# OSU-NLP-Group/saev

Hardware: AMD Instinct MI355X
Metric: activations/sec (train step), d_in=1024 x32 k=32 (higher is better)
Workload: dtype f32 (encoder: fp16 MFMA first pass with a rigorous error margin, survivors recomputed exactly in fp32; all else fp32)

## Files before the change

saev_amd/csrc/ctx.h:

```cpp
#pragma once
#include <hip/hip_runtime.h>

#include <algorithm>
#include <cmath>
#include <cstdio>
#include <cstdlib>
#include <cstring>
#include <string>
#include <vector>

#include "kernels.h"

constexpr int AUX_KSPLIT_MAX = 16;
constexpr int CAND_CAP = 4096;
constexpr int CAND_STRIDE = CAND_CAP + 256;
constexpr int TIMING_RING = 512;
constexpr int DEAD_LAG = 4;
constexpr int DEAD_RING = 16;
enum { AUX_NONE = 0, AUX_SMALL_DEVICE = 1, AUX_SMALL_HOST = 2, AUX_DENSE = 3 };

struct saev_ctx {
    saev_cfg cfg{};
    saev_debug_cfg dbg{};
    int device = 0;
    std::string err;
    float* params = nullptr;
    float* grads = nullptr;
    float* adam_m = nullptr;
    float* adam_v = nullptr;
    long n_params = 0;
    long off_W_dec = 0, off_b_dec = 0, off_W_enc = 0, off_b_enc = 0;
    int shard_world = 1;
    long chunk_a = 0, chunk_b = 0;
    double* sumsq_bound = nullptr;
    hipEvent_t wdec_ready = nullptr;
    hipEvent_t wenc_ready = nullptr;
    std::vector<void*> allocs;
    size_t scratch_bytes = 0, aux_bytes = 0;
    uint8_t* muon_ws = nullptr;
    size_t muon_bytes = 0;
    int cuts_last[MAX_PREFIXES] = {0};
    int32_t *cand_cnt = nullptr, *gmax = nullptr, *cand_idx = nullptr;
    int gmax_stride = 0;
    float* cand_val = nullptr;
    float* h_dense = nullptr;
    int32_t *idx = nullptr, *aux_idx = nullptr;
    float *val = nullptr, *aux_val = nullptr;
    float *x_hat = nullptr, *g = nullptr, *g_aux = nullptr;
    RowStats* rowstats = nullptr;
    uint32_t* bitmap = nullptr;
    int32_t* grp_prefix = nullptr;
    int32_t* scan_totals = nullptr;
    int32_t csc_epoch = 0;
    int bitmap_words = 0;
    int back_rows = 0;
    int bitmap_words_last = 0;
    bool bitmap_clean = false;
    int bitmap_clean_words = 0;
    int bitmap_prefill_words = 0, bitmap_prefill_rows = 0;
    bool last_backward_gathered = false;
    int32_t *counts = nullptr, *starts = nullptr;
    int2* pairs = nullptr;
    float* colsum_partials = nullptr;
    float* dval_pairs = nullptr;
    double *sumsq_partials = nullptr, *sumsq_total = nullptr;
    bool wenc_sq_valid = false;
    float2* row_proj = nullptr;
    float* enc_sq = nullptr;
    bool row_proj_valid = false, tail_proj_in_adam = false;
    bool wenc_t_pending = false;
    int64_t* toks = nullptr;
    int32_t *fired = nullptr, *dead = nullptr;
    int32_t* flags = nullptr;
    int32_t *chunk_starts = nullptr, *part_starts = nullptr, *work_latent = nullptr;
    float *dW_encT = nullptr, *partials = nullptr, *db_partials = nullptr;
    bool dws_ok = false;
    int dws_rows = 0;
    bool dws_pairs = false;
    float *gS = nullptr, *xS = nullptr, *dvp = nullptr;
    float* xS_ov = nullptr;
    float* xS_bwd = nullptr;
    float* dval_rows = nullptr;
    bool dval_fwd = false;
    float* wn2 = nullptr;
    float* sq_wave = nullptr;
    int sq_wave_n = 0;
    bool wn2_fresh = false;
    bool dval_pairs_ready = false;
    bool fused_forward = false;
    bool g_rows_valid = true;
    bool fwd_slices = false;
    bool fwd_step = false;
    float* rs_part = nullptr;
    float* xS_c = nullptr;
    int2 *pv = nullptr, *pv2 = nullptr;
    int32_t *plat = nullptr, *cut_lat = nullptr, *cut_list = nullptr;
    int32_t* lat_unused = nullptr;
    bool fused_step = false;
    bool unused_valid = false;
    int P = 1;
    int32_t cuts[MAX_PREFIXES] = {0};
    float* G = nullptr;
    float* GS = nullptr;
    int P_cap = 0;
    int n_dead_host = 0, k_use_host = 0;
    int64_t tokens_seen = 0;
    bool tracker_dirty = false;
    int nd_cap = 0;
    DeadRecord* rec_host = nullptr;
    DeadRecord* rec_dev = nullptr;
    hipEvent_t dead_ev[DEAD_RING];
    bool dead_ev_created = false;
    int64_t dead_steps = 0;
    int64_t rec_valid_from = 1;
    int aux_route = AUX_NONE;
    int64_t n_readbacks = 0;
    std::vector<void*> aux_allocs;
    int32_t* dead_list = nullptr;
    float *Wenc_dead = nullptr, *Wdec_dead = nullptr, *H_dead = nullptr, *A_dead = nullptr, *dWd = nullptr, *dWe = nullptr,
          *dbe = nullptr, *aux_partials = nullptr, *WencT_dead = nullptr, *aux_small_part = nullptr, *aux_small_part2 = nullptr, *aux_small_partbe = nullptr;
    bool aux_dev_count = false;
    bool aux_small = false;
    int aux_mfma_bound = 0;
    int aux_ndp = AUX_SMALL_MAX;
    int aux_mfma_cap = AUX_SMALL_MAX;
    bool aux_mfma = false;
    bool aux_fused = false;
    bool aux_all = false;
    uint8_t* A_mask = nullptr;
    _Float16 *aux_ws1 = nullptr, *aux_ws2 = nullptr, *aux_xsA = nullptr, *aux_xsg = nullptr, *aux_kA = nullptr, *aux_kD = nullptr, *aux_kX = nullptr;
    bool aux_both = false;
    float* aux_parts = nullptr;
    int aux_kpad = 0;
    float *bias_dead = nullptr, *zero_bias = nullptr, *aux_scales = nullptr;
    float* aux_sync = nullptr;
    int aux_Dp2 = 0;
    float *row_margin = nullptr, *wnorm_scratch = nullptr, *surv_val = nullptr;
    int32_t *surv_idx = nullptr, *surv_cnt = nullptr, *surv_rng = nullptr;
    int rs_lat_range = 0, rs_n_ranges = 0;
    int32_t* tau_max = nullptr;
    float* heur_state = nullptr;
    float *f16r_scales = nullptr, *mu = nullptr, *xnorm = nullptr, *b_shift = nullptr, *dot_part = nullptr, *xabs_part = nullptr,
          *sq_part = nullptr, *wmax_prev = nullptr;
    bool wmax_known = false;
    bool mu_ready = false;
    bool stream_ok = false;
    float *WeS = nullptr;
    float *xn_part = nullptr, *amax_part = nullptr, *cmax_part = nullptr;
    float* b_seen = nullptr;
    int32_t *stale_host = nullptr, *stale_dev = nullptr;
    uint32_t* wchk = nullptr;
    float *mu_keep = nullptr, *xside_keep = nullptr;
    bool fwd_streamed = false;
    bool fwd_moves_mu = false;
    int64_t fwd_mu_serial = -1;
    bool borrow_streamed = false;
    bool follow_stream = false;
    bool wchk_valid = false;
    bool fwd_reused_wimg = false;
    uint32_t stale_salt = 0;
    int scale_par = 0;
    bool prep_valid = false;
    bool wimg_fresh = false;
    int64_t mu_serial = 0, wimg_mu_serial = -1;
    bool wimg_bf16_fresh = false;
    bool stream_step = false;
    bool stats_pending = false, stats_lists = false;
    bool aux_stats_pending = false;
    bool dead_list_ready = false;
    bool train_fused = false;
    const float* gather_pool = nullptr;
    const int64_t* gather_rows = nullptr;
    float *upper_c = nullptr, *mu_c = nullptr, *xnorm_c = nullptr, *xabs_c = nullptr;
    _Float16* xs_c = nullptr;
    saev_ctx* leader = nullptr;
    void* comm = nullptr;
    int comm_rank = 0, comm_world = 0;
    std::vector<saev_ctx*> followers;
    const float* xprep_x = nullptr;
    int xprep_n = 0;
    int64_t xprep_serial = 0;
    int64_t leader_serial_seen = 0;
    _Float16 *xs = nullptr, *ws = nullptr;
    int Dp = 0, S_pad = 0, MB_pad = 0;
    int max_work = 0, max_part = 0;
    float* upper = nullptr;
    saev_step_stats* stats = nullptr;
    double* stats_scratch = nullptr;
    int* tickets = nullptr;
    const float *ov_x = nullptr, *ov_g = nullptr, *ov_val = nullptr;
    const int32_t* ov_idx = nullptr;
    int ov_n = 0;
    float* db_aux = nullptr;
    bool trust_grads = false;
    bool btk = false;
    int btk_k = 0, btk_list_cap = 0;
    double btk_momentum = 0.1;
    float *threshold = nullptr, *threshold_own = nullptr;
    uint32_t* btk_ws = nullptr;
    int32_t *row_nnz = nullptr, *btk_over = nullptr;
    int btk_need = 0;
    bool relu_train = false;
    bool rt_fwd_live = false;
    double rt_l1 = 0.0;
    float* rt_dA = nullptr;
    float *rt_parts = nullptr, *rt_colpart = nullptr;
    float* rt_scales = nullptr;
    int rt_Sp = 0, rt_kpad = 0;
    _Float16 *rt_xsF = nullptr, *rt_xsG = nullptr;
    _Float16 *rt_wsR = nullptr, *rt_wsK = nullptr;
    _Float16 *rt_kF = nullptr, *rt_kG = nullptr, *rt_kX = nullptr;
    float* rt_wparts = nullptr;
    const float* x_last = nullptr;
// ... 96 lines not shown
```

saev_amd/csrc/ctx.hip:

```cpp
#include "ctx.h"

int muon_cfg_check(const saev_muon_cfg& m, std::string* why) {
    if (m.ns_steps < 0 || m.ns_steps >= 100) { *why = "ns_steps must be in [0, 100)"; return SAEV_INVALID_ARG; }
    if (m.adjust_lr < 0 || m.adjust_lr > 2) { *why = "adjust_lr must be 0 (original), 1 (match_rms_adamw) or 2 (none)"; return SAEV_INVALID_ARG; }
    if (!(m.momentum >= 0.f) || !(m.weight_decay >= 0.f)) { *why = "momentum and weight_decay must be >= 0"; return SAEV_INVALID_ARG; }
    return SAEV_OK;
}

extern "C" {

int saev_abi_version(void) { return SAEV_AMD_ABI_VERSION; }

int saev_layout(const saev_cfg* cfg, saev_layout_t* out) {
    if (!cfg || !out || cfg->d_model <= 0 || cfg->d_sae <= 0) return SAEV_INVALID_ARG;
    const int64_t S = cfg->d_sae, D = cfg->d_model, N = std::max(1, cfg->shard_world);
    out->chunk_a = (S + 1 + N - 1) / N * D;
    out->chunk_b = ((D * S + S + N - 1) / N + 3) / 4 * 4;
    out->off_W_dec = 0;
    out->off_b_dec = S * D;
    out->off_W_enc = N * out->chunk_a;
    out->off_b_enc = out->off_W_enc + D * S;
    out->n_total = N * out->chunk_a + N * out->chunk_b;
    return SAEV_OK;
}

const char* saev_last_error(const saev_ctx* ctx) { return ctx ? ctx->err.c_str() : free_error(); }

int saev_create(const saev_cfg* cfg, int device, saev_ctx** out) { return saev_create_ex(cfg, nullptr, device, out); }

int saev_create_ex(const saev_cfg* cfg, const saev_debug_cfg* dbg, int device, saev_ctx** out) {
    return saev_create_batch_topk(cfg, dbg, nullptr, device, out);
}

int saev_create_batch_topk(const saev_cfg* cfg, const saev_debug_cfg* dbg, const saev_batch_topk_cfg* bt_in, int device, saev_ctx** out) {
    return create_context(cfg, dbg, bt_in, nullptr, device, out);
}

int saev_create_relu_train(const saev_cfg* cfg, const saev_debug_cfg* dbg, const saev_relu_train_cfg* rt, int device, saev_ctx** out) {
    if (!cfg || !out) return SAEV_INVALID_ARG;
    *out = nullptr;
    if (cfg->activation != SAEV_ACT_RELU || cfg->k_aux != 0) return SAEV_INVALID_ARG;
    saev_relu_train_cfg r{};
    if (rt != nullptr && rt->struct_size > 0) std::memcpy(&r, rt, std::min((size_t)rt->struct_size, sizeof(r)));
    if (!(r.l1_coeff >= 0.0) || !std::isfinite(r.l1_coeff)) return SAEV_INVALID_ARG;
    if (cfg->encoder_mode == SAEV_ENCODER_BF16 || cfg->shard_world > 1 || cfg->max_backward_rows > cfg->max_batch) return SAEV_UNSUPPORTED;
    r.struct_size = (int32_t)sizeof(r);
    return create_context(cfg, dbg, nullptr, &r, device, out);
}

}

int create_context(const saev_cfg* cfg, const saev_debug_cfg* dbg, const saev_batch_topk_cfg* bt_in, const saev_relu_train_cfg* rt, int device,
                   saev_ctx** out) {
    if (!cfg || !out) return SAEV_INVALID_ARG;
    *out = nullptr;
    if (cfg->activation != SAEV_ACT_TOPK && cfg->activation != SAEV_ACT_RELU && cfg->activation != SAEV_ACT_BATCHTOPK) return SAEV_INVALID_ARG;
    const bool btk = cfg->activation == SAEV_ACT_BATCHTOPK;
    if (bt_in != nullptr && !btk) return SAEV_INVALID_ARG;
    saev_batch_topk_cfg bt{};
    if (bt_in != nullptr && bt_in->struct_size > 0) std::memcpy(&bt, bt_in, std::min((size_t)bt_in->struct_size, sizeof(bt)));
    else bt.batch_momentum = 0.1;
    saev_cfg btk_cfg;
    int btk_k = 0;
    if (btk) {
        if (cfg->top_k <= 0 || cfg->d_sae <= 0 || bt.row_cap < 0 || bt.list_cap < 0 || !(bt.batch_momentum >= 0.0 && bt.batch_momentum <= 1.0))
            return SAEV_INVALID_ARG;
        if (cfg->encoder_mode == SAEV_ENCODER_BF16 || cfg->shard_world > 1 || cfg->max_backward_rows > cfg->max_batch) return SAEV_UNSUPPORTED;
        if ((uint64_t)cfg->max_batch * (uint64_t)cfg->d_sae >= (1ull << 31)) return SAEV_UNSUPPORTED;
        btk_k = std::min(cfg->top_k, cfg->d_sae);
        const long want = bt.row_cap > 0 ? bt.row_cap : std::max(64L, 4L * btk_k);
        btk_cfg = *cfg;
        btk_cfg.top_k = (int32_t)std::min<long>(cfg->d_sae, (want + 63) / 64 * 64);
        cfg = &btk_cfg;
    }
    saev_cfg relu_cfg;
    if (cfg->activation == SAEV_ACT_RELU) {
        if (cfg->k_aux != 0) return SAEV_UNSUPPORTED;
        relu_cfg = *cfg;
        relu_cfg.top_k = 1;
        cfg = &relu_cfg;
    }
    if (cfg->d_model <= 0 || cfg->d_sae <= 0 || cfg->top_k <= 0 || cfg->max_batch <= 0) return SAEV_INVALID_ARG;
    if ((uint64_t)cfg->max_batch * CAND_STRIDE * 4ull >= (1ull << 32)) return SAEV_INVALID_ARG;
    if (cfg->d_model % 4 != 0 || cfg->d_sae % 4 != 0 || cfg->d_model > 4096) return SAEV_UNSUPPORTED;
    if (cfg->k_aux < 0 || cfg->k_aux > 1024) return SAEV_UNSUPPORTED;
    if (cfg->encoder_mode != SAEV_ENCODER_F32 && cfg->encoder_mode != SAEV_ENCODER_F16X3 && cfg->encoder_mode != SAEV_ENCODER_BF16 &&
        cfg->encoder_mode != SAEV_ENCODER_F16R)
        return SAEV_INVALID_ARG;
    saev_ctx* c = new saev_ctx();
    c->cfg = *cfg;
    c->cfg.top_k = std::min(cfg->top_k, cfg->d_sae);
    if (dbg != nullptr && dbg->struct_size > 0)
        std::memcpy(&c->dbg, dbg, std::min((size_t)dbg->struct_size, sizeof(saev_debug_cfg)));
    c->device = device;
    c->btk = btk; c->btk_k = btk_k; c->btk_momentum = bt.batch_momentum; c->btk_list_cap = bt.list_cap;
    c->relu_train = rt != nullptr;
    c->rt_l1 = rt != nullptr ? rt->l1_coeff : 0.0;
    if (hipSetDevice(device) != hipSuccess) {
        delete c;
        return SAEV_HIP_ERROR;
    }
    const long S = cfg->d_sae, D = cfg->d_model, MB = cfg->max_batch, K = c->cfg.top_k, KA = cfg->k_aux;
    const long MBB = std::max<long>(MB, cfg->max_backward_rows);
    c->back_rows = (int)MBB;
    if ((uint64_t)MBB * K >= (1ull << 31)) { delete c; return SAEV_INVALID_ARG; }
    {
        saev_layout_t lay;
        saev_layout(cfg, &lay);
        c->shard_world = std::max(1, cfg->shard_world);
        c->chunk_a = lay.chunk_a; c->chunk_b = lay.chunk_b;
        c->off_W_dec = lay.off_W_dec; c->off_b_dec = lay.off_b_dec; c->off_W_enc = lay.off_W_enc; c->off_b_enc = lay.off_b_enc;
        c->n_params = lay.n_total;
    }
    int rc = SAEV_OK;
#define A(p, n) if (rc == SAEV_OK) rc = alloc(c, &c->p, (size_t)(n))
    c->gmax_stride = (int)((MB + 255) / 256 * 256);
    A(cand_cnt, MB); A(gmax, (size_t)64 * c->gmax_stride); A(cand_idx, MB * CAND_STRIDE); A(cand_val, MB * CAND_STRIDE);
    A(h_dense, MB * S);
    A(idx, MB * K); A(val, MB * K);
    if (KA > 0) { A(aux_idx, MB * KA); A(aux_val, MB * KA); A(g_aux, MB * D); A(dead_list, S); }
    A(x_hat, MB * D); A(g, MB * D);
    A(rowstats, MB);
    c->bitmap_words = (int)(((MBB + 31) / 32 + 7) / 8 * 8);
    A(bitmap, S * c->bitmap_words);
    A(grp_prefix, S * (c->bitmap_words / 8));
    A(scan_totals, ((S + 1023) / 1024) * 4);
    A(counts, S); A(starts, S + 1); A(pairs, MBB * K); A(dval_pairs, MBB * (size_t)cfg->top_k);
    {
        const long max_pairs = MBB * K;
        c->max_work = (int)(S + (max_pairs + DW_CHUNK - 1) / DW_CHUNK);
        c->max_part = (int)(2 * ((max_pairs + DW_CHUNK - 1) / DW_CHUNK) + 2);
    }
    A(chunk_starts, S + 1); A(part_starts, S); A(work_latent, c->max_work);
    A(dW_encT, S * D); A(partials, (size_t)c->max_part * 2 * D); A(db_partials, c->max_part); A(row_proj, S); A(enc_sq, S);
    {
        const bool rows_only = c->dbg.dw_route == 1;
        c->dws_ok = !rows_only && !btk && D % DWS_SLICE == 0 && (uint64_t)S * D * 4ull < (1ull << 32) && MBB < (1l << 24) &&
                    (uint64_t)MBB * K < (1ull << 31);
    }
    c->fwd_slices = !btk && c->cfg.encoder_mode == SAEV_ENCODER_F16R && c->dbg.fwd_route == 0 && D % RS_SLICE == 0 &&
                    (uint64_t)S * 128ull < (1ull << 32) - 256ull && fused_supported(c->cfg);
    if (c->fwd_slices) {
        A(rs_part, (size_t)(D / RS_SLICE) * MB * REFINE_CAP); A(surv_rng, MB * RS_MAX_RANGES);
        c->rs_lat_range = (int)std::max<long>(RS_LAT_RANGE, ((S + RS_MAX_RANGES - 1) / RS_MAX_RANGES + 255) / 256 * 256);
        c->rs_n_ranges = (int)((S + c->rs_lat_range - 1) / c->rs_lat_range);
    }
    if (c->fwd_slices && !c->dws_ok) A(xS, MBB * D);
    if (c->dws_ok) {
        A(gS, MBB * D); A(xS, MBB * D); A(dvp, (size_t)(D / DWS_SLICE) * MBB * K);
        if (c->dbg.dw_route != 2 && decode_forms_dval((int)D, (int)K)) A(dval_rows, MB * K);
        A(pv, MBB * K); A(pv2, MBB * K); A(plat, MBB * K); A(cut_lat, (MBB * K + DWS_RUN - 1) / DWS_RUN); A(cut_list, 4 * (1 + (MBB * K + DWS_RUN - 1) / DWS_RUN)); A(lat_unused, S);
        if (c->dval_rows != nullptr && c->dbg.fin_route == 0) { A(wn2, S); A(sq_wave, (size_t)2 * dw_slices_waves((int)D, (int)(MBB * K))); }
    }
    A(colsum_partials, ((MBB + 63) / 64) * D);
    A(sumsq_partials, 2 * 1024 + (S + 3) / 4 + 8 + transpose_blocks((int)S, (int)D)); A(sumsq_total, 1);
    if (c->cfg.encoder_mode != SAEV_ENCODER_F32 || KA > 0 || c->relu_train) {
        c->Dp = (int)((D + 31) / 32 * 32);
        c->S_pad = (int)((S + 255) / 256 * 256);
        c->MB_pad = (int)((MB + 255) / 256 * 256);
        A(zero_bias, std::max(S, D)); A(aux_scales, 16); A(aux_sync, absmax_parts_max((int)MB));
    }
    if (c->cfg.encoder_mode != SAEV_ENCODER_F32) {
        A(xs, (size_t)c->MB_pad * 2 * c->Dp);
        A(ws, (size_t)c->S_pad * 2 * c->Dp);
        A(row_margin, MB); A(wnorm_scratch, std::max((S + 3) / 4, 3 * ((S + 255) / 256))); A(f16r_scales, 16); A(mu, D); A(xnorm, 2 * MB); A(b_shift, S);
        A(xabs_part, (MB + 3) / 4);
        if (c->cfg.encoder_mode == SAEV_ENCODER_F16R) { A(dot_part, (size_t)2 * (c->Dp / 32) * c->S_pad); A(sq_part, (size_t)2 * (c->Dp / 32) * c->S_pad); A(wmax_prev, 1); }
        if (c->cfg.encoder_mode == SAEV_ENCODER_F16R) { A(surv_idx, MB * REFINE_CAP); A(surv_val, MB * REFINE_CAP); A(surv_cnt, MB); }
    }
    c->stream_ok = c->fwd_slices && c->cfg.bound_mode == 0 && c->dbg.prep_route == 0 && D % 32 == 0 && c->Dp == (int)D;
    if (c->stream_ok) {
        A(WeS, S * D); A(xn_part, (size_t)(D / 32) * c->MB_pad * 2);
        A(amax_part, (size_t)(c->MB_pad / 256) * (D / 32)); A(cmax_part, (size_t)(c->MB_pad / 256) * (D / 32)); A(b_seen, S);
        A(mu_keep, D); A(xside_keep, 4);
    }
    if (c->stream_ok || c->cfg.encoder_mode == SAEV_ENCODER_BF16) A(wchk, (size_t)2 * ((S + 255) / 256) * ((D + 31) / 32));
    A(toks, S); A(fired, S); A(dead, S); A(flags, 16); A(upper, 1); A(stats, 1);
    A(tau_max, MB); A(heur_state, 8); A(stats_scratch, STATS_SCRATCH_DOUBLES); A(tickets, 8); A(db_aux, D);
    if (btk) { A(btk_ws, btk_workspace_words((int)MB)); A(row_nnz, MB); A(btk_over, 1); A(threshold_own, 1); }
#undef A
    if (rc == SAEV_OK && c->relu_train) rc = relu_train_alloc(c);
    if (rc != SAEV_OK) {
        for (void* p : c->allocs) hipFree(p);
        delete c;
        return rc;
    }
    hipMemset(c->toks, 0, S * sizeof(int64_t));
    hipMemset(c->fired, 0, S * sizeof(int32_t));
    hipMemset(c->dead, 0, S * sizeof(int32_t));
    hipMemset(c->flags, 0, 16 * sizeof(int32_t));
    if (btk) {
        hipMemset(c->threshold_own, 0, sizeof(float));
        hipMemset(c->btk_ws, 0, BTK_ST_WORDS * sizeof(uint32_t));
        hipMemset(c->btk_over, 0, sizeof(int32_t));
        c->threshold = c->threshold_own;
    }
    if (c->stream_ok || c->cfg.encoder_mode == SAEV_ENCODER_BF16) {
        void* hp = nullptr;
        if (hipHostMalloc(&hp, 64, hipHostMallocMapped) == hipSuccess &&
            hipHostGetDevicePointer(reinterpret_cast<void**>(&c->stale_dev), hp, 0) == hipSuccess) {
            c->stale_host = static_cast<int32_t*>(hp);
            c->stale_host[0] = 0; c->stale_host[1] = 0;
        } else {
            if (hp) hipHostFree(hp);
            c->stale_host = nullptr; c->stale_dev = nullptr;
        }
    }
    hipMemset(c->scan_totals, 0, ((S + 1023) / 1024) * 4 * sizeof(int32_t));
    hipMemset(c->stats, 0, sizeof(saev_step_stats));
    hipMemset(c->stats_scratch, 0, STATS_SCRATCH_DOUBLES * sizeof(double));
    hipMemset(c->tickets, 0, 8 * sizeof(int));
    {
        const float init[8] = {2.6f, 0.f, 0.f, 0.f, 0.f, 0.f, 0.f, 0.f};
        hipMemcpy(c->heur_state, init, sizeof(init), hipMemcpyHostToDevice);
    }
    hipMemset(c->rowstats, 0, MB * sizeof(RowStats));
    if (c->xs) hipMemset(c->xs, 0, (size_t)c->MB_pad * 2 * c->Dp * sizeof(_Float16));
    if (c->zero_bias) hipMemset(c->zero_bias, 0, std::max(S, D) * sizeof(float));
    if (c->f16r_scales) hipMemset(c->f16r_scales, 0, 16 * sizeof(float));
    if (KA > 0) {
        const int s4 = (int)((S + 3) / 4 * 4);
        const int want = cfg->aux_dead_cap > 0 ? cfg->aux_dead_cap : std::max(4096, 8 * (int)KA);
        const int cap = std::min((want + 3) / 4 * 4, s4);
        rc = alloc_aux_buffers(c, cap);
        if (rc == SAEV_OK) {
            void* h = nullptr;
            if (hipHostMalloc(&h, DEAD_RING * sizeof(DeadRecord), hipHostMallocMapped) != hipSuccess ||
                hipHostGetDevicePointer(reinterpret_cast<void**>(&c->rec_dev), h, 0) != hipSuccess) {
                rc = SAEV_HIP_ERROR;
            } else {
                c->rec_host = static_cast<DeadRecord*>(h);
                std::memset(h, 0, DEAD_RING * sizeof(DeadRecord));
                for (int i = 0; i < DEAD_RING && rc == SAEV_OK; ++i)
                    if (hipEventCreateWithFlags(&c->dead_ev[i], hipEventDisableTiming) != hipSuccess) rc = SAEV_HIP_ERROR;
                c->dead_ev_created = rc == SAEV_OK;
            }
        }
        if (rc != SAEV_OK) {
            for (void* q : c->allocs) hipFree(q);
            for (void* q : c->aux_allocs) hipFree(q);
            if (c->rec_host) hipHostFree(c->rec_host);
            delete c;
            return rc;
        }
    }
    hipDeviceSynchronize();
    *out = c;
    return SAEV_OK;
}

extern "C" {

static void detach_follower(saev_ctx* c) {
    c->leader = nullptr;
    centre_owner_changed(c);
    c->borrow_streamed = false;
    c->follow_stream = false;
}

static void unlink_from_leader(saev_ctx* c) {
    if (c->leader != nullptr) {
        auto& f = c->leader->followers;
        f.erase(std::remove(f.begin(), f.end(), c), f.end());
        detach_follower(c);
    }
}

void saev_destroy(saev_ctx* c) {
    if (!c) return;
    for (saev_ctx* f : c->followers) detach_follower(f);
    c->followers.clear();
    unlink_from_leader(c);
    hipSetDevice(c->device);
    hipDeviceSynchronize();
    saev_comm_destroy(c);
    for (void* p : c->allocs) hipFree(p);
    for (void* p : c->aux_allocs) hipFree(p);
    if (c->G) hipFree(c->G);
// ... 293 lines not shown
```

saev_amd/csrc/ctx_backward.hip:

```cpp
#include "ctx.h"

extern "C" {


int saev_backward_begin(saev_ctx* c, void* stream) {
    if (!c) return SAEV_INVALID_ARG;
    REQUIRE(c, !c->relu_train, SAEV_UNSUPPORTED, "saev_backward_begin: a ReLU training context runs its dense backward in one piece (saev_step_backward)");
    REQUIRE(c, c->x_last && c->training_last, SAEV_INVALID_ARG, "saev_backward_begin: no training forward in flight");
    REQUIRE(c, c->grads, SAEV_NOT_BOUND, "gradient buffer not bound");
    hipStream_t s = (hipStream_t)stream;
    const int S = c->cfg.d_sae, D = c->cfg.d_model, K = c->cfg.top_k;
    const bool ov = c->ov_x != nullptr;
    const int n = ov ? c->ov_n : c->n_last;
    const int words = ((n + 31) / 32 + 7) / 8 * 8;
    c->row_proj_valid = false;
    CscArgs a{};
    a.idx = ov ? c->ov_idx : c->idx; a.code_stride = K; a.k = K; a.k_dev = nullptr; a.n_rows = n; a.S = S;
    a.bitmap = c->bitmap; a.words = words; a.grp_prefix = c->grp_prefix; a.scan_totals = c->scan_totals;
    a.counts = c->counts; a.starts = c->starts; a.pairs = c->pairs;
    a.chunk_starts = c->chunk_starts; a.part_starts = c->part_starts; a.work_latent = c->work_latent;
    const bool ov_slices = ov && c->dws_ok && c->P_last == 1 && n <= c->back_rows;
    c->dws_pairs = ov ? ov_slices : c->dws_rows == n;
    if (ov_slices) {
        c->xS_bwd = c->xS;
        if (!c->followers.empty()) {
            if (c->xS_ov == nullptr) {
                int rca = alloc(c, &c->xS_ov, (size_t)c->back_rows * D);
                if (rca != SAEV_OK) return rca;
            }
            c->xS_bwd = c->xS_ov;
        }
        HIPCHK(c, launch_slice_major_copy(c->ov_g, c->ov_x, n, D, c->gS, c->xS_bwd, s));
        c->dws_rows = 0;
    }
    c->csc_epoch = c->csc_epoch == 0x7fffffff ? 1 : c->csc_epoch + 1;
    a.epoch = c->dbg.csc_route == 2 ? 0 : c->csc_epoch;
    if (c->dws_pairs) {
        a.zero_word = c->cut_list;
        a.pv = c->pv; a.plat = c->plat; a.val = ov ? c->ov_val : c->val;
        a.P = c->P_last;
        for (int p = 0; p < c->P_last; ++p) a.cuts[p] = c->cuts_last[p];
        if (!ov && c->dval_fwd) { a.pv2 = c->pv2; a.dval = c->dval_rows; }
    }
    c->dval_pairs_ready = c->dws_pairs && a.pv2 != nullptr;
    if (c->fused_step && c->dws_pairs) { a.pairs = nullptr; a.chunk_starts = nullptr; a.part_starts = nullptr; a.work_latent = nullptr; }
    const float* gmat = ov ? c->ov_g : (c->P_last > 1 ? c->G : c->g);
    const bool g_slices = !ov && c->P_last == 1 && !c->g_rows_valid;
    if (g_slices) {
        REQUIRE(c, c->dws_rows == n, SAEV_INVALID_ARG, "saev_backward_begin: the forward in flight left no gradient rows");
        gmat = c->gS;
    }
    const bool prefilled = !ov && c->bitmap_prefill_words == words && c->bitmap_prefill_rows == n;
    HIPCHK(c, launch_csc_build(a, s, c->bitmap_clean && words <= c->bitmap_clean_words, gmat, D, (long)c->P_last * D,
                               c->colsum_partials, c->grads + c->off_b_dec, prefilled, g_slices));
    c->bitmap_prefill_words = 0;
    c->last_backward_gathered = ov;
    c->bitmap_clean = false;
    c->bitmap_words_last = words;
    if (c->aux_route != AUX_NONE) {
        int rc = auxk_backward(c, s);
        if (rc != SAEV_OK) return rc;
    }
    return SAEV_OK;
}

int saev_backward_rows(saev_ctx* c, int32_t lat_lo, int32_t lat_hi, void* stream) {
    return saev_backward_rows_part(c, lat_lo, lat_hi, 0, stream);
}

int saev_backward_rows_part(saev_ctx* c, int32_t lat_lo, int32_t lat_hi, int32_t part, void* stream) {
    if (!c) return SAEV_INVALID_ARG;
    REQUIRE(c, !c->relu_train, SAEV_UNSUPPORTED, "saev_backward_rows: a ReLU training context runs its dense backward in one piece, over all latents (saev_step_backward)");
    REQUIRE(c, part >= 0 && part <= 2, SAEV_INVALID_ARG, "saev_backward_rows_part: part must be 0 (both), 1 (decoder) or 2 (encoder)");
    REQUIRE(c, c->x_last && c->training_last && c->grads, SAEV_INVALID_ARG, "saev_backward_rows: call saev_backward_begin first");
    const int S = c->cfg.d_sae, D = c->cfg.d_model, K = c->cfg.top_k;
    const bool ov = c->ov_x != nullptr;
    const int n = ov ? c->ov_n : c->n_last;
    REQUIRE(c, 0 <= lat_lo && lat_lo < lat_hi && lat_hi <= S, SAEV_INVALID_ARG, "saev_backward_rows: bad latent range");
    REQUIRE(c, !c->btk || (part == 0 && lat_lo == 0 && lat_hi == S), SAEV_UNSUPPORTED,
            "saev_backward_rows: a BatchTopK context runs the backward over all latents in one part");
    hipStream_t s = (hipStream_t)stream;
    DwRowsArgs a{};
    a.starts = c->starts; a.chunk_starts = c->chunk_starts; a.work_latent = c->work_latent;
    a.part_starts = c->part_starts; a.pairs = c->pairs; a.val = ov ? c->ov_val : c->val; a.W_dec = c->params + c->off_W_dec;
    a.g = ov ? c->ov_g : (c->P_last > 1 ? c->G : c->g);
    const bool slices_all = lat_lo == 0 && lat_hi == S && c->dws_pairs && (ov || c->dws_rows == n);
    REQUIRE(c, ov || c->P_last > 1 || c->g_rows_valid || slices_all, SAEV_INVALID_ARG,
            "saev_backward_rows: the fused step's forward keeps no row-major gradient (a latent range needs the phase forward)");
    a.x = ov ? c->ov_x : c->x_last;
    a.D = D; a.S = S; a.k_dev = nullptr; a.accumulate = 0;
    a.P = c->P_last;
    for (int p = 0; p < c->P_last; ++p) a.cuts[p] = c->cuts_last[p];
    a.dW_dec = c->grads + c->off_W_dec; a.dW_encT = c->dW_encT; a.db_enc = c->grads + c->off_b_enc;
    a.partials = c->partials; a.db_partials = c->db_partials;
    a.lat_lo = lat_lo; a.lat_hi = lat_hi;
    a.part = part; a.dval = c->dval_pairs;
    const bool all_rows = part == 0 && lat_lo == 0 && lat_hi == S;
    const bool clears = part != 2 && lat_lo == 0 && lat_hi == S && c->bitmap_words_last > 0;
    if (clears) { a.clear_bitmap = c->bitmap; a.clear_words = c->bitmap_words_last; }
    a.row_proj = all_rows ? c->row_proj : nullptr; a.project = c->cfg.remove_parallel_grads ? 1 : 0;
    a.enc_sq = all_rows ? c->enc_sq : nullptr;
    const int max_work = (lat_hi - lat_lo) + (int)(((long)n * K + DW_CHUNK - 1) / DW_CHUNK);
    if (slices_all) {
        DwSlicesArgs w{};
        w.starts = c->starts; w.pv = c->pv; w.pv2 = c->pv2; w.plat = c->plat; w.gS = c->P_last > 1 ? c->GS : c->gS; w.W_dec = a.W_dec; w.P = c->P_last;
        w.xS = ov ? c->xS_bwd : (c->fwd_step ? c->xS_c : c->xS);
        w.n_rows = n; w.D = D; w.S = S; w.pair_cap = (int)((long)c->back_rows * K);
        w.dvp = c->dvp; w.dW_dec = a.dW_dec; w.dW_encT = a.dW_encT; w.db_enc = a.db_enc;
        const size_t runs_cap = ((size_t)w.pair_cap + DWS_RUN - 1) / DWS_RUN;
        w.part_dec = c->partials; w.part_enc = c->partials + 2 * runs_cap * D;
        w.cut_lat = c->cut_lat; w.cut_list = c->cut_list;
        w.lat_unused = (all_rows && c->fused_step) ? c->lat_unused : nullptr;
        c->unused_valid = w.lat_unused != nullptr;
        w.row_proj = a.row_proj; w.project = a.project; w.enc_sq = a.enc_sq;
        w.clear_bitmap = a.clear_bitmap; w.clear_words = a.clear_words;
        w.have_dval = c->dval_pairs_ready ? 1 : 0;
        c->sq_wave_n = 0;
        if (c->dval_pairs_ready && c->wn2_fresh && part == 0) {
            w.wn2 = c->wn2;
            if (c->fused_step && all_rows && c->sq_wave != nullptr && c->dbg.fin_route != 2) {
                c->sq_wave_n = dw_slices_waves(D, (int)((long)n * K));
                w.sq_wave_dec = c->sq_wave; w.sq_wave_enc = c->sq_wave + c->sq_wave_n;
            }
        }
        HIPCHK(c, launch_dw_slices(w, (int)((long)n * K), part, s));
    } else {
        c->unused_valid = false;
        HIPCHK(c, launch_dw_rows(a, max_work, s));
    }
    if (c->aux_route == AUX_DENSE)
        HIPCHK(c, launch_scatter_add_dead(c->dead_list, c->n_dead_host, D, c->dWd, c->dWe, c->dbe, c->grads + c->off_W_dec,
                                          c->dW_encT, c->grads + c->off_b_enc, lat_lo, lat_hi, s,
                                          c->aux_dev_count ? c->flags + 4 : nullptr, part, a.row_proj, a.W_dec, a.project, a.enc_sq,
                                          c->unused_valid ? c->lat_unused : nullptr, c->sq_wave_n > 0 ? c->starts : nullptr));
    else if (c->aux_route != AUX_NONE)
        HIPCHK(c, launch_scatter_add_dead(c->dead_list, c->aux_mfma ? c->aux_ndp : AUX_SMALL_MAX, D, c->dWd, c->dWe, c->dbe, c->grads + c->off_W_dec,
                                          c->dW_encT, c->grads + c->off_b_enc, lat_lo, lat_hi, s, c->flags + 4, part,
                                          a.row_proj, a.W_dec, a.project, a.enc_sq, c->unused_valid ? c->lat_unused : nullptr,
                                          c->sq_wave_n > 0 ? c->starts : nullptr));
    if (ov && c->aux_route != AUX_NONE && part != 2 && lat_lo == 0)
        HIPCHK(c, launch_colsum(c->db_aux, 1, D, c->colsum_partials, c->grads + c->off_b_dec, 1, nullptr, s));
    c->row_proj_valid = all_rows;
    if (clears) { c->bitmap_clean = true; c->bitmap_clean_words = c->bitmap_words_last; }
    return SAEV_OK;
}

float* saev_grad_w_enc_t(saev_ctx* c) { return c ? c->dW_encT : nullptr; }

int saev_bind_w_enc_t(saev_ctx* c, float* scratch) {
    if (!c || !scratch) return SAEV_INVALID_ARG;
    c->dW_encT = scratch;
    return SAEV_OK;
}

int saev_copy_step_state(saev_ctx* c, int32_t n_rows, float* g_out, int32_t* idx_out, float* val_out, void* stream) {
    if (!c) return SAEV_INVALID_ARG;
    REQUIRE(c, !c->btk, SAEV_UNSUPPORTED, "saev_copy_step_state: not for a BatchTopK context (no sparse-state exchange)");
    REQUIRE(c, !c->relu_train, SAEV_UNSUPPORTED, "saev_copy_step_state: not for a ReLU training context (its step state is dense: no sparse-state exchange)");
    REQUIRE(c, c->n_last > 0 && c->training_last && n_rows == c->n_last, SAEV_INVALID_ARG,
            "saev_copy_step_state: n_rows must be the row count of the training forward in flight");
    hipStream_t s = (hipStream_t)stream;
    const size_t nk = (size_t)n_rows * c->cfg.top_k, nd = (size_t)n_rows * c->cfg.d_model * (size_t)c->P_last;
    REQUIRE(c, !g_out || c->P_last > 1 || c->g_rows_valid, SAEV_INVALID_ARG,
            "saev_copy_step_state: the fused step's forward keeps no row-major gradient (use saev_step_forward)");
    if (g_out) HIPCHK(c, hipMemcpyAsync(g_out, c->P_last > 1 ? c->G : c->g, nd * sizeof(float), hipMemcpyDeviceToDevice, s));
    if (idx_out) HIPCHK(c, hipMemcpyAsync(idx_out, c->idx, nk * sizeof(int32_t), hipMemcpyDeviceToDevice, s));
    if (val_out) HIPCHK(c, hipMemcpyAsync(val_out, c->val, nk * sizeof(float), hipMemcpyDeviceToDevice, s));
    return SAEV_OK;
}

int saev_backward_override(saev_ctx* c, const float* x_all, const float* g_all, const int32_t* idx_all, const float* val_all,
                           int32_t n_all) {
    if (!c) return SAEV_INVALID_ARG;
    if (x_all == nullptr) { c->ov_x = nullptr; c->ov_n = 0; return SAEV_OK; }
    REQUIRE(c, !c->btk, SAEV_UNSUPPORTED, "saev_backward_override: not for a BatchTopK context (a batch-wide top-k over ranks needs a distributed select)");
    REQUIRE(c, !c->relu_train, SAEV_UNSUPPORTED, "saev_backward_override: not for a ReLU training context (one GPU: the dense backward runs over its own rows)");
    REQUIRE(c, g_all && idx_all && val_all && n_all > 0, SAEV_INVALID_ARG, "saev_backward_override: NULL buffer");
    REQUIRE(c, n_all <= c->back_rows, SAEV_INVALID_ARG,
            "saev_backward_override: the gathered row count exceeds saev_cfg.max_backward_rows (set it to the GLOBAL batch)");
    REQUIRE(c, c->x_last && c->training_last, SAEV_INVALID_ARG, "saev_backward_override: no training forward in flight");
    REQUIRE(c, ((uintptr_t)x_all % 16) == 0 && ((uintptr_t)g_all % 16) == 0, SAEV_INVALID_ARG, "x_all / g_all must be 16-byte aligned");
    c->ov_x = x_all; c->ov_g = g_all; c->ov_idx = idx_all; c->ov_val = val_all; c->ov_n = n_all;
    return SAEV_OK;
}

int32_t saev_aux_compact_rows(const saev_ctx* c) {
    if (!c || c->aux_route == AUX_NONE) return 0;
    return c->aux_route == AUX_DENSE ? (c->n_dead_host + 3) / 4 * 4 : (c->aux_mfma ? c->aux_ndp : AUX_SMALL_MAX);
}

static int aux_compact_copy(saev_ctx* c, float* buf, bool out, hipStream_t s) {
    const size_t rows = (size_t)saev_aux_compact_rows(c), D = c->cfg.d_model;
    if (rows == 0) return SAEV_OK;
    REQUIRE(c, buf != nullptr, SAEV_INVALID_ARG, "saev_aux_compact_*: NULL buffer");
    float* seg[4] = {c->dWd, c->dWe, c->dbe, c->db_aux};
    const size_t len[4] = {rows * D, rows * D, rows, D};
    size_t off = 0;
    for (int i = 0; i < 4; ++i) {
        if (out) HIPCHK(c, hipMemcpyAsync(buf + off, seg[i], len[i] * sizeof(float), hipMemcpyDeviceToDevice, s));
        else HIPCHK(c, hipMemcpyAsync(seg[i], buf + off, len[i] * sizeof(float), hipMemcpyDeviceToDevice, s));
        off += len[i];
    }
    return SAEV_OK;
}
int saev_aux_compact_export(saev_ctx* c, float* buf, void* stream) {
    if (!c) return SAEV_INVALID_ARG;
    return aux_compact_copy(c, buf, true, (hipStream_t)stream);
}
int saev_aux_compact_import(saev_ctx* c, const float* buf, void* stream) {
    if (!c) return SAEV_INVALID_ARG;
    return aux_compact_copy(c, const_cast<float*>(buf), false, (hipStream_t)stream);
}

int saev_trust_gradients(saev_ctx* c, int32_t on) {
    if (!c) return SAEV_INVALID_ARG;
    c->trust_grads = on != 0;
    return SAEV_OK;
}

int saev_backward_end(saev_ctx* c, void* stream) {
    if (!c) return SAEV_INVALID_ARG;
    REQUIRE(c, !c->relu_train, SAEV_UNSUPPORTED, "saev_backward_end: a ReLU training context runs its dense backward in one piece (saev_step_backward)");
    REQUIRE(c, c->grads, SAEV_NOT_BOUND, "gradient buffer not bound");
    double* sq = c->sumsq_partials + 2 * sumsq_blocks() + (c->cfg.d_sae + 3) / 4;
    HIPCHK(c, launch_transpose(c->dW_encT, c->grads + c->off_W_enc, c->cfg.d_sae, c->cfg.d_model, (hipStream_t)stream, sq));
    c->wenc_sq_valid = true;
    return SAEV_OK;
}

int saev_step_backward(saev_ctx* c, void* stream) {
    if (c && c->relu_train) return relu_train_backward(c, (hipStream_t)stream);
    int rc = saev_backward_begin(c, stream);
    if (rc != SAEV_OK) return rc;
    rc = saev_backward_rows(c, 0, c->cfg.d_sae, stream);
    if (rc != SAEV_OK) return rc;
    return saev_backward_end(c, stream);
}

}
```

saev_amd/csrc/ctx_forward.hip:

```cpp
#include "ctx.h"

extern "C" {


int saev_normalize_w_dec(saev_ctx* c, void* stream) {
    if (!c) return SAEV_INVALID_ARG;
    REQUIRE(c, c->params, SAEV_NOT_BOUND, "parameters not bound");
    if (!c->cfg.normalize_w_dec) return SAEV_OK;
    HIPCHK(c, launch_normalize_rows(c->params + c->off_W_dec, c->cfg.d_sae, c->cfg.d_model, (hipStream_t)stream));
    return SAEV_OK;
}

static bool bind_x_sources(saev_ctx* c, const float* x, int n, bool allow_borrow) {
    saev_ctx* l = c->leader;
    const bool borrow = allow_borrow && l != nullptr && l->xprep_x == x && l->xprep_n == n && l->xprep_serial != c->leader_serial_seen;
    saev_ctx* src = borrow ? l : c;
    c->upper_c = src->upper; c->mu_c = src->mu; c->xnorm_c = src->xnorm; c->xabs_c = src->xabs_part; c->xs_c = src->xs;
    c->borrow_streamed = borrow && l->fwd_streamed && l->mu_keep != nullptr;
    if (c->borrow_streamed) c->mu_c = l->mu_keep;
    c->fwd_step = c->fwd_slices && (src == c || src->fwd_slices);
    c->xS_c = c->fwd_step ? src->xS : nullptr;
    if (borrow) c->leader_serial_seen = l->xprep_serial;
    return borrow;
}
// ... 416 lines not shown
    int64_t single = S;
    if (!prefixes_host) { prefixes_host = &single; n_prefixes = 1; }
    REQUIRE(c, n_prefixes >= 1 && n_prefixes <= 16, SAEV_INVALID_ARG, "saev_decode_rows: 1 to 16 prefixes");
    REQUIRE(c, prefixes_host[n_prefixes - 1] == S && prefixes_host[0] >= 1, SAEV_INVALID_ARG,
            "prefixes must end at d_sae and start at >= 1");
    for (int p = 1; p < n_prefixes; ++p)
        REQUIRE(c, prefixes_host[p] > prefixes_host[p - 1], SAEV_INVALID_ARG, "prefixes must be strictly increasing");
    ReluDecodeArgs a{};
    a.idx = idx; a.val = val; a.row_nnz = row_nnz; a.row_cap = row_cap; a.n_rows = n; a.D = c->cfg.d_model;
    a.W_dec = c->params + c->off_W_dec; a.b_dec = c->params + c->off_b_dec;
    a.n_prefixes = n_prefixes;
    for (int p = 0; p < n_prefixes; ++p) a.prefixes[p] = prefixes_host[p];
    a.x_hats = x_hats_out;
    HIPCHK(c, launch_relu_decode(a, (hipStream_t)stream));
    return SAEV_OK;
}

int saev_scatter_rows(saev_ctx* c, const int32_t* idx, const float* val, const int32_t* row_nnz, int32_t row_cap, int32_t n,
                      float* f_out, void* stream) {
    if (!c) return SAEV_INVALID_ARG;
    REQUIRE(c, idx && val && row_nnz && f_out && n > 0 && row_cap > 0, SAEV_INVALID_ARG, "saev_scatter_rows: bad arguments");
    HIPCHK(c, launch_relu_scatter(idx, val, row_nnz, row_cap, n, c->cfg.d_sae, f_out, (hipStream_t)stream));
    return SAEV_OK;
}

int saev_remove_parallel_grads(saev_ctx* c, void* stream) {
    if (!c) return SAEV_INVALID_ARG;
    REQUIRE(c, c->params && c->grads, SAEV_NOT_BOUND, "parameters/grads not bound");
    if (!c->cfg.remove_parallel_grads) return SAEV_OK;
    HIPCHK(c, launch_rpg(c->grads + c->off_W_dec, c->params + c->off_W_dec, c->cfg.d_sae, c->cfg.d_model,
                         (hipStream_t)stream));
    return SAEV_OK;
}

int saev_gather_rows(saev_ctx* c, const float* pool, const int64_t* rows, int32_t n, float* out, void* stream) {
    if (!c) return SAEV_INVALID_ARG;
    REQUIRE(c, pool && rows && out && n > 0, SAEV_INVALID_ARG, "saev_gather_rows: bad arguments");
    HIPCHK(c, launch_gather_rows(pool, rows, n, c->cfg.d_model, out, (hipStream_t)stream));
    return SAEV_OK;
}


int saev_step_forward(saev_ctx* c, const float* x, int32_t n, int64_t n_rows_global, int32_t training,
                      void* stream) {
    if (!c) return SAEV_INVALID_ARG;
    if (c->relu_train) return relu_train_forward(c, x, n, n_rows_global, training, (hipStream_t)stream);
    REQUIRE(c, c->cfg.activation != SAEV_ACT_RELU, SAEV_UNSUPPORTED, "saev_step_forward: a ReLU context runs the forward entries only");
    REQUIRE(c, c->params, SAEV_NOT_BOUND, "parameters not bound");
    REQUIRE(c, x && n > 0 && n <= c->cfg.max_batch, SAEV_INVALID_ARG,
            "saev_step_forward: n_rows must be in 1..max_batch");
    REQUIRE(c, ((uintptr_t)x % 16) == 0, SAEV_INVALID_ARG, "x must be 16-byte aligned");
    REQUIRE(c, n_rows_global >= n, SAEV_INVALID_ARG, "n_rows_global < n_rows");
    hipStream_t s = (hipStream_t)stream;
    const int S = c->cfg.d_sae, D = c->cfg.d_model, K = c->cfg.top_k;
    c->x_last = x;
    c->n_last = n;
    c->training_last = training;
    c->ov_x = nullptr; c->ov_n = 0;
    c->unused_valid = false;
    hipEvent_t wdec_ev = c->wdec_ready;
    c->wdec_ready = nullptr;
    const bool btk = c->btk;
    const bool borrowed = bind_x_sources(c, x, n, !btk);
    if (c->stale_host != nullptr && reinterpret_cast<volatile int32_t*>(c->stale_host)[1] != 0) {
        const int n_tiles = reinterpret_cast<volatile int32_t*>(c->stale_host)[1];
        reinterpret_cast<volatile int32_t*>(c->stale_host)[1] = 0;
        c->wimg_fresh = false; c->wimg_bf16_fresh = false; c->wn2_fresh = false;
        c->err = "W_enc was written outside the library without saev_params_touched (" + std::to_string(n_tiles) +
                 " 32 x 256 tiles changed between two optimizer steps): a recent step encoded with operand images of the OLD values. "
                 "Announce such writes (saev_params_touched / SaeEngine.params_touched) or make them through torch in-place "
                 "operations on the parameter tensors; the context prepares from scratch from here on";
        return SAEV_STALE_PARAMS;
    }
    if (c->stale_host != nullptr && *reinterpret_cast<volatile int32_t*>(c->stale_host) != 0) {
        *reinterpret_cast<volatile int32_t*>(c->stale_host) = 0;
        c->wimg_fresh = false;
        c->wn2_fresh = false;
    }
    c->stream_step = c->stream_ok && c->prep_valid && c->wimg_fresh && c->wimg_mu_serial == c->mu_serial && c->leader == nullptr &&
                     c->wenc_ready == nullptr && c->fwd_step && (c->followers.empty() || c->dbg.group_route == 0);
    if (!borrowed) {
        c->fwd_streamed = c->stream_step;
        c->fwd_moves_mu = c->stream_step && c->train_fused;
        c->fwd_mu_serial = c->mu_serial;
    }
    c->follow_stream = borrowed && c->borrow_streamed && c->stream_ok && c->wimg_fresh && c->wimg_mu_serial == c->leader->fwd_mu_serial &&
                       c->wenc_ready == nullptr && c->fwd_step && c->cfg.encoder_mode == SAEV_ENCODER_F16R;
    c->fwd_reused_wimg = c->stream_step || c->follow_stream;
    if (c->gather_pool != nullptr && !c->stream_step)
        HIPCHK(c, launch_gather_rows(c->gather_pool, c->gather_rows, n, D, const_cast<float*>(x), s));
    if (c->stream_step) {
        c->xprep_x = nullptr;
    } else if (!borrowed && !btk && c->cfg.encoder_mode == SAEV_ENCODER_F16R) {
        c->xprep_x = nullptr;
        HIPCHK(c, launch_colsum_absmax(x, n, D, c->colsum_partials, c->mu, c->xabs_part, c->upper, s, 1.0f / (float)n, c->stats, c->flags));
        c->mu_ready = true;
        c->mu_serial++;
    } else {
        HIPCHK(c, launch_step_zero(c->stats, c->upper, c->flags, s));
        if (!borrowed) {
            c->xprep_x = nullptr;
            HIPCHK(c, launch_absmax(x, (long)n * D, c->upper, s));
        }
    }
    (void)n_rows_global;
    int rc;
    if (btk) {
        rc = encode_dense_h(c, x, n, s);
        if (rc == SAEV_OK) rc = btk_codes(c, c->h_dense, n, training, c->row_nnz, c->idx, c->val, c->btk_over, s);
        if (rc == SAEV_OK) {
            int32_t need = 0;
            HIPCHK(c, hipMemcpyAsync(&need, c->btk_over, sizeof(int32_t), hipMemcpyDeviceToHost, s));
            HIPCHK(c, hipStreamSynchronize(s));
            if (need > 0) {
                c->btk_need = need;
                c->x_last = nullptr; c->n_last = 0; c->training_last = 0;
                c->err = "BatchTopK: a row holds " + std::to_string(need) + " codes, the context's row_cap is " + std::to_string(K) +
                         " (create a context with a larger saev_batch_topk_cfg.row_cap and repeat the forward; the threshold has not moved)";
                return SAEV_ROW_OVERFLOW;
            }
        }
    } else {
        rc = encode_topk_impl(c, x, n, c->idx, c->val, c->flags, s, c->upper_c, borrowed);
    }
    if (rc != SAEV_OK) return rc;
    if (!borrowed) { c->xprep_x = x; c->xprep_n = n; c->xprep_serial++; }
    if (!borrowed && c->stream_ok && !c->stream_step && c->fwd_step) {
        HIPCHK(c, hipMemcpyAsync(scl(c) + 4, c->upper, sizeof(float), hipMemcpyDeviceToDevice, s));
        c->prep_valid = true;
    }
    if (wdec_ev != nullptr) HIPCHK(c, hipStreamWaitEvent(s, wdec_ev, 0));
    if (training) {
        c->wn2_fresh = false;
        if (c->cfg.normalize_w_dec) {
            HIPCHK(c, launch_normalize_rows(c->params + c->off_W_dec, S, D, s, c->wn2));
            c->wn2_fresh = c->wn2 != nullptr;
        }
    }

    DecodeArgs a{};
    a.x = x; a.idx = c->idx; a.val = c->val; a.code_stride = K; a.k = K;
    a.W_dec = c->params + c->off_W_dec; a.b_dec = c->params + c->off_b_dec;
    a.n_rows = n; a.D = D; a.S = S; a.idx_limit = S;
    a.upper = c->upper_c;
    a.gscale = 2.0f / ((float)n * (float)D * (float)c->P);
    a.training = training ? 1 : 0;
    a.g = c->g; a.x_hat = c->x_hat; a.fired = c->fired; a.rowstats = c->rowstats;
    c->dws_rows = 0;
    c->dval_fwd = false;
    if (training && c->dws_ok && (c->P == 1 || c->GS != nullptr)) { a.gS = c->P == 1 ? c->gS : c->GS; a.xS = c->fwd_step ? nullptr : c->xS; c->dws_rows = n; }
    if (c->dws_rows == n && c->dval_rows != nullptr && (c->P == 1 || decode_matry_forms_dval(D, K))) { a.dval_out = c->dval_rows; c->dval_fwd = true; }
    c->g_rows_valid = !(c->train_fused && training && c->P == 1 && c->dws_rows == n);
    if (!c->g_rows_valid) a.g = nullptr;
    c->bitmap_prefill_words = 0;
    if (training && c->dbg.csc_route == 0 && c->bitmap != nullptr && c->bitmap_clean && !c->last_backward_gathered) {
        const int words = ((n + 31) / 32 + 7) / 8 * 8;
        if (words <= c->bitmap_clean_words) {
            a.csc_bitmap = c->bitmap; a.csc_words = words;
            c->bitmap_prefill_words = words; c->bitmap_prefill_rows = n;
            c->bitmap_clean = false;
        }
    }
    if (c->P > 1) {
        MatryArgs m{};
        m.P = c->P;
        for (int p = 0; p < c->P; ++p) m.cuts[p] = c->cuts[p];
        m.G = c->G;
        m.g_rows_all = c->fused_forward ? 0 : 1;
        HIPCHK(c, launch_decode_matry(a, m, s));
    } else {
        HIPCHK(c, launch_decode(a, s));
    }
    c->P_last = c->P;
    for (int p = 0; p < c->P; ++p) c->cuts_last[p] = c->cuts[p];
    const bool lists = !btk && fused_supported(c->cfg) && !(c->cfg.bound_mode != 0 && c->cfg.encoder_mode != SAEV_ENCODER_F32 && f16_ngroups(c) == 32);
    c->stats_pending = false;
    if (c->train_fused && training) {
        c->stats_pending = true;
        c->stats_lists = lists;
        return SAEV_OK;
    }
    HIPCHK(c, launch_stats_reduce(c->rowstats, n, D, c->P, c->cfg.alpha, 0, c->upper_c, c->flags + 2, c->stats, s, nullptr, c->stats_scratch,
                                  lists ? c->cand_cnt : nullptr, CAND_CAP));
    return SAEV_OK;
}

}
```

saev_amd/csrc/kernels.h:

```cpp
#pragma once
#include <hip/hip_runtime.h>
#include <stdint.h>

#include <string>

#include "../../include/saev_amd.h"

enum { EPI_DENSE = 0, EPI_TOPK = 1 };

struct EncodeArgs {
    const float* x;
    const float* W_enc;
    const float* b_enc;
    int n_rows, D, S;
    int s_splits;
    float* h_out;
    int ngroups;
    int32_t* gmax;
    int gmax_stride;
    int32_t* cand_cnt;
    float* cand_val;
    int32_t* cand_idx;
    int cand_cap;
    int cand_stride;
    const int32_t* enable_flag;
    int enable_when;
};

size_t encode_gemm_smem_bytes();
hipError_t launch_encode_gemm(const EncodeArgs& a, int epi, hipStream_t stream);
int encode_gemm_tile_rows();
int encode_gemm_tile_latents();

struct SelectDenseArgs {
    const float* h;
    int n_rows, S;
    int k;
    const int32_t* k_dev;
    const int32_t* mask;
    int32_t* idx_out;
    float* val_out;
    int out_stride;
    const int32_t* enable_flag;
    int enable_when;
    int walk_grid;
};
hipError_t launch_select_dense(const SelectDenseArgs& a, hipStream_t stream);

struct SelectCandArgs {
    const int32_t* cand_cnt;
    const float* cand_val;
    const int32_t* cand_idx;
    int cand_cap, cand_stride, n_rows, k;
    int32_t* idx_out;
    float* val_out;
    int out_stride;
    const int32_t* enable_flag;
    int enable_when;
    const float* row_margin;
    const float* x;
    const float* W_encT;
    const float* b_enc;
    int D;
    int32_t* surv_idx;
    float* surv_val;
    int32_t* surv_cnt;
    int32_t* refine_overflow;
    const int32_t* tau_max;
    int32_t* invalid;
    int32_t* ovf;
    int32_t* surv_rng;
    int lat_range, n_ranges;
    const float* sum_part;
    const float* sum_bias;
    int sum_n;
    size_t sum_plane;
};
hipError_t launch_refine_exact(const SelectCandArgs& a, hipStream_t stream);
constexpr int REFINE_CAP = 512;
constexpr int RS_SLICE = 32;
constexpr int RS_ROWS_MAX = 8;
constexpr int RS_LAT_RANGE = 32768;
constexpr int RS_MAX_RANGES = 8;
struct RefineSlicesArgs {
    const int32_t* surv_idx; const int32_t* surv_cnt; float* surv_val; const int32_t* surv_rng;
    const float* xS; const float* WeS; const float* b_enc; float* part;
    int n_rows, S, D, lat_range, n_ranges;
    const int32_t* enable_flag; int enable_when;
};
hipError_t launch_refine_slices(const RefineSlicesArgs& a, hipStream_t stream);
hipError_t launch_select_cand(const SelectCandArgs& a, hipStream_t stream);
hipError_t launch_init_i32(int32_t* p, int32_t v, int n, hipStream_t stream);
hipError_t launch_encoder_init(int32_t* cand_cnt, int n_rows, int32_t* gmax, int n_gmax, hipStream_t stream,
                               int32_t* tau_max = nullptr, const int32_t* enable_flag = nullptr, int enable_when = 0);
hipError_t launch_pre_encode(int32_t* cand_cnt, int n_rows, int32_t* gmax, int n_gmax, const float* xnorm, int D,
                             const float* wg_part, int n_part, const float* scales, int32_t* pre_flag, float* wmax_prev,
                             float* margin, int32_t* flags1, hipStream_t stream);
hipError_t launch_heur_gate(float* state, const int32_t* pre_flag, int32_t* gate, hipStream_t stream);
hipError_t launch_heur_update(float* state, const int32_t* bad, const float* cand_mean, int k, const int32_t* gate,
                              hipStream_t stream);
hipError_t launch_step_zero(saev_step_stats* stats, float* upper, int32_t* flag0, hipStream_t stream);
hipError_t launch_wnorm_max(const float* W_encT, int S, int D, float* wg_scratch, float* wmax, hipStream_t stream);
hipError_t launch_f16r_scales(const float* xmax_part, int n_part, const float* wmax, float* scales, hipStream_t stream);
hipError_t launch_pow2_scale(const float* absmax, float* pair, hipStream_t stream);
hipError_t launch_center_stats(const float* x, const float* mu, int n, int D, float* xnorm, float* wg_absmax,
                               hipStream_t stream, const float* xmax = nullptr);
hipError_t launch_row_margins(const float* xnorm, int n, int D, const float* wg_part, int n_part, const float* scales,
                              int32_t* pre_flag, float* wmax_prev, float* margin, hipStream_t stream);
hipError_t launch_overflow_check(const int32_t* cand_cnt, int n_rows, int cap, const int32_t* pre_flag,
                                 int32_t* need_dense, int32_t* n_overflow, int32_t* cand_max, hipStream_t stream,
                                 int32_t* dense_out = nullptr, int32_t* run_out = nullptr, float* cand_mean = nullptr,
                                 const int32_t* enable_flag = nullptr, const int32_t* dense_src = nullptr);

struct __attribute__((aligned(8))) RowStats {
    float sse_scaled;
    float l0;
    float l1;
    float aux_sse;
    double sse64;
    double sumsq64;
};

struct DecodeArgs {
    const float* x;
    const int32_t* idx;
    const float* val;
    int code_stride, k;
    const float* W_dec;
    const float* b_dec;
    int n_rows, D, S;
    int idx_limit;
    const float* upper;
    float gscale;
    int training;
    float* g;
    float* x_hat;
    int32_t* fired;
    RowStats* rowstats;
    float* gS;
    float* xS;
    float* dval_out;
    uint32_t* csc_bitmap;
    int csc_words;
};
hipError_t launch_decode(const DecodeArgs& a, hipStream_t stream);
bool decode_forms_dval(int D, int k);
bool decode_matry_forms_dval(int D, int k);

constexpr int MAX_PREFIXES = 16;
struct MatryArgs {
    int P;
    int32_t cuts[MAX_PREFIXES];
    float* G;
    int g_rows_all;
};
hipError_t launch_decode_matry(const DecodeArgs& a, const MatryArgs& m, hipStream_t stream);

struct CscArgs {
    const int32_t* idx;
    int code_stride, k;
    const int32_t* k_dev;
    int n_rows, S;
    uint32_t* bitmap;
    int words;
    int32_t* grp_prefix;
    int32_t* counts;
    int32_t* scan_totals;
    int32_t* starts;
    int2* pairs;
    int32_t* chunk_starts;
    int32_t* part_starts;
    int32_t* work_latent;
    int2* pv;
    int32_t* plat;
    const float* val;
    int2* pv2;
    const float* dval;
    int P;
    int32_t cuts[16];
    int32_t* zero_word;
    int32_t epoch;
};
hipError_t launch_csc_build(const CscArgs& a, hipStream_t stream, bool bitmap_clean = false, const float* colsum_m = nullptr,
                            int colsum_D = 0, long colsum_row_stride = 0, float* colsum_partials = nullptr,
                            float* colsum_out = nullptr, bool prefilled = false,
                            bool colsum_slice_major = false);

constexpr int DW_CHUNK = 64;

struct DwRowsArgs {
    const int32_t* starts;
    const int32_t* chunk_starts;
    const int32_t* work_latent;
    const int32_t* part_starts;
    const int2* pairs;
    const float* val;
    const float* W_dec;
    const float* g;
    const float* x;
    int D, S;
    int P;
    int32_t cuts[MAX_PREFIXES];
    const int32_t* k_dev;
    int accumulate;
    float* dW_dec;
    float* dW_encT;
    float* db_enc;
    float* partials;
    float* db_partials;
    int lat_lo, lat_hi;
    int part;
    float* dval;
    float2* row_proj;
    int project;
    float* enc_sq;
    uint32_t* clear_bitmap;
    int clear_words;
};
hipError_t launch_dw_rows(const DwRowsArgs& a, int max_work, hipStream_t stream);

constexpr int DWS_RUN = 64, DWS_SLICE = 32;
constexpr int DWS_FIRST = 1, DWS_LAST = 2, DWS_END = 4;
struct DwSlicesArgs {
    const int32_t* starts;
    const int2* pv;
    int2* pv2;
    const int32_t* plat;
    const float* gS;
    const float* xS;
    const float* W_dec;
    int n_rows, D, S, pair_cap;
    int P;
    float* dvp;
    float* dW_dec;
    float* dW_encT;
    float* db_enc;
    float* part_dec;
    float* part_enc;
    int32_t* cut_lat;
    int32_t* cut_list;
    float2* row_proj;
    int project;
    float* enc_sq;
    uint32_t* clear_bitmap;
    int clear_words;
    int32_t* lat_unused;
    int have_dval;
    const float* wn2;
    float* sq_wave_dec;
    float* sq_wave_enc;
};
hipError_t launch_dw_slices(const DwSlicesArgs& a, int max_pairs, int part, hipStream_t stream);
int dw_slices_waves(int D, int max_pairs);
hipError_t launch_slice_major_copy(const float* g, const float* x, int n, int D, float* gS, float* xS, hipStream_t stream);
hipError_t launch_transpose(const float* in, float* out, int S, int D, hipStream_t stream, double* sq_part = nullptr);
int transpose_blocks(int S, int D);

hipError_t launch_colsum(const float* m, int n_rows, int D, float* partials, float* out, int accumulate,
                         const int32_t* k_dev, hipStream_t stream, long row_stride = 0, float out_scale = 1.0f,
                         int col_mult = 0);
hipError_t launch_colsum_absmax(const float* m, int n_rows, int D, float* partials, float* out, float* wg_scratch,
                                float* absmax_out, hipStream_t stream, float out_scale = 1.0f,
                                saev_step_stats* zero_stats = nullptr, int32_t* zero_flag = nullptr);

hipError_t launch_normalize_rows(float* W, int S, int D, hipStream_t stream, float* wn2 = nullptr);
hipError_t launch_rpg(float* gW, const float* W, int S, int D, hipStream_t stream, double* sq_partials = nullptr,
                      int project = 1);
int sumsq_blocks();
hipError_t launch_sumsq_partials(const float* g, long n, double* partials, hipStream_t stream);
hipError_t launch_sumsq_final(const double* partials, int nb, double* total, hipStream_t stream);
hipError_t launch_sumsq(const float* g, long n, double* partials, double* total, hipStream_t stream);
struct AdamArgs {
    float* p; const float* g; float* m; float* v;
    long n;
    float lr, beta1, beta2, eps, bc1, bc2_sqrt;
    float omb1, omb2;
    float grad_scale;
    float max_norm;
    const double* sumsq;
    saev_step_stats* stats;
};
hipError_t launch_adam(const AdamArgs& a, hipStream_t stream);
hipError_t launch_adam_rows(const AdamArgs& a, const float2* row_proj, int S, int D, hipStream_t stream);
hipError_t launch_sumsq_final_ex(const double* partials, int nb, const float2* row_proj, int n_rows, const float* e1, long n1,
                                 const float* e2, long n2, double* total, double* blk_part, int* ticket, hipStream_t stream,
                                 const float* enc_sq = nullptr,
                                 const float* plain = nullptr, long n_plain = 0);
struct AdamImageArgs {
    _Float16* ws; float* WeS; double* dot_part; float* sq_part;
    const float* mu; const float* wmax_prev; float* scales_next;
    int nks, S_pad;
    int mode;
    uint32_t* chk; int32_t* late; int verify;
    const int32_t* early;
};
hipError_t launch_adam_fused(const AdamArgs& a, const float2* row_proj, const float* gT, int S, int D, long off_b_dec, long n_b_dec,
                             long off_W_enc, long off_b_enc, long n_b_enc, hipStream_t stream, const int32_t* lat_unused = nullptr,
                             const AdamImageArgs* img = nullptr);
constexpr int SUMSQ_EX_BLOCKS = 32;

struct DeadRecord {
    int64_t step;
    int64_t cum_tokens;
    int64_t horizon_tokens;
    int32_t n_dead;
    int32_t n_near;
};

struct DeadArgs {
    int64_t* toks;
    int32_t* fired;
    int32_t* dead;
    int S;
    int64_t add_tokens, threshold;
    int k_aux;
    int32_t* n_dead;
    int32_t* k_use;
    saev_step_stats* stats;
    int32_t* scratch;
    int64_t horizon_tokens;
    int64_t step, cum_tokens;
    DeadRecord* rec;
    int32_t* dead_list;
};
hipError_t launch_dead_update(const DeadArgs& a, hipStream_t stream);
hipError_t launch_stats_dead(const RowStats* rs, int n_rows, int D, int P, float alpha, const float* upper, const int32_t* n_overflow,
                             saev_step_stats* stats, double* scratch, const int32_t* cand_cnt, int cand_cap, const DeadArgs& d,
                             hipStream_t stream);
hipError_t launch_absmax(const float* x, long n, float* out_zeroed, hipStream_t stream);
hipError_t launch_gather_rows(const float* pool, const int64_t* rows, int n_rows, int D, float* out, hipStream_t stream);
hipError_t launch_scatter_dense(const int32_t* idx, const float* val, int n_rows, int k, int stride, int S, float* f,
                                hipStream_t stream);
hipError_t launch_stats_reduce(const RowStats* rs, int n_rows, int D, int P, float alpha, int with_aux, const float* upper,
                               const int32_t* n_overflow_and_max, saev_step_stats* stats, hipStream_t stream,
                               const int32_t* n_dead_dev, double* scratch,
                               const int32_t* cand_cnt = nullptr, int cand_cap = 0);
constexpr int STATS_SCRATCH_DOUBLES = 16 * 8 + 1;

struct EncodeF16Args {
    const _Float16* xs;
    const _Float16* ws;
    const float* b_enc;
    int n_rows, Dp, S;
    float w_scale;
    int arith;
    const float* row_margin;
    const float* scale_dev;
    const float* scale_dev_b;
    int s_splits;
    float* h_out;
    int ngroups;
    int top_k;
    int32_t* gmax;
    int gmax_stride;
    int32_t* cand_cnt;
    float* cand_val;
    int32_t* cand_idx;
    int cand_cap, cand_stride;
    const int32_t* enable_flag;
    int enable_when;
    const float* heur_z;
    int32_t* tau_max;
    int refresh_first, refresh_every;
    int n_batches;
    int blk_imgs;
    long out_bstride;
};
hipError_t launch_encode_f16x3(const EncodeF16Args& a, int epi, hipStream_t stream);
int encode_f16x3_tile_rows();
int encode_f16x3_tile_latents();
hipError_t launch_split_rows(const float* x, int n, int D, int Dp, void* xs, int mode, hipStream_t stream, float scale = 1.0f,
                             const float* scale_dev = nullptr,
                             const float* mu = nullptr,
                             float* xS = nullptr);
hipError_t launch_split_wT(const float* W, int D, int S, int S_pad, int Dp, float scale, void* ws, int mode,
                           hipStream_t stream, const float* scale_dev = nullptr,
                           const float* mu = nullptr, double* dot_part = nullptr, float* sq_part = nullptr,
                           float* W_T = nullptr,
                           int wt_slices = 0);
struct XprepArgs {
    const float* x;
    const int64_t* rows;
    float* x_out;
    int n, D, nks, n_pad;
    const float* scales;
    const float* mu;
    _Float16* xs;
    float* xS;
    float* xn_part;
    float* col_part;
    float* amax_part;
    float* cmax_part;
    const float* W_enc; const float* WeS; const float* b_enc; const float* b_seen;
    int S; uint32_t salt; int32_t* stale;
    float* mu_keep; float* xside_keep;
};
hipError_t launch_xprep(const XprepArgs& a, hipStream_t stream);
struct PreEncode2Args {
// ... 257 lines not shown
```

saev_amd/csrc/sparse.hip:

```cpp
#include "common.h"
#include "kernels.h"

namespace {

template <int NV>
__device__ __forceinline__ void gather_rows_accum(f32x4 (&acc)[NV], const float* __restrict__ W, int D, int D4,
                                                  const int32_t* idx_row, const float* val_row, int k, int limit,
                                                  int lane) {
    for (int j0 = 0; j0 < k; j0 += 64) {
        const int cnt = min(64, k - j0);
        int32_t my_i = -1;
        float my_v = 0.f;
        if (lane < cnt) { my_i = idx_row[j0 + lane]; my_v = val_row[j0 + lane]; }
#pragma unroll 4
        for (int jj = 0; jj < cnt; ++jj) {
            const int32_t i = __shfl(my_i, jj, 64);
            const float v = __shfl(my_v, jj, 64);
            if (i < 0 || i >= limit) continue;
            const f32x4* wr = reinterpret_cast<const f32x4*>(W + (size_t)i * D);
#pragma unroll
            for (int n = 0; n < NV; ++n) {
                const int q = lane + 64 * n;
                if (q < D4) {
                    const f32x4 w = wr[q];
                    acc[n] += v * w;
                }
            }
        }
    }
}

template <int KC>
__device__ __forceinline__ float wave_reduce_scatter(float (&p)[KC], int lane) {
    int bit = 32;
#pragma unroll
    for (int h = KC / 2; h >= 1; h >>= 1, bit >>= 1) {
        const bool up = (lane & bit) != 0;
#pragma unroll
        for (int i = 0; i < h; ++i) {
            const float keep = up ? p[i + h] : p[i];
            const float send = up ? p[i] : p[i + h];
            p[i] = keep + __shfl_xor(send, bit, 64);
        }
    }
    float r = p[0];
    for (; bit >= 1; bit >>= 1) r += __shfl_xor(r, bit, 64);
    return r;
}

template <int H, int BIT>
__device__ __forceinline__ void wave_rs_step(float* p, int lane) {
    if constexpr (H >= 1) {
        const bool up = (lane & BIT) != 0;
#pragma unroll
        for (int i = 0; i < H; ++i) {
            const float keep = up ? p[i + H] : p[i];
            const float send = up ? p[i] : p[i + H];
            p[i] = keep + __shfl_xor(send, BIT, 64);
        }
        wave_rs_step<H / 2, BIT / 2>(p, lane);
    }
}
__device__ __forceinline__ float wave_reduce_scatter32(float (&p)[32], int lane) {
    wave_rs_step<16, 32>(p, lane);
    return p[0] + __shfl_xor(p[0], 1, 64);
}

__device__ __forceinline__ void csc_mark(const DecodeArgs& a, int32_t i, int row) {
    if (a.csc_bitmap != nullptr && i >= 0 && i < a.S) atomicOr(&a.csc_bitmap[(size_t)i * a.csc_words + (row >> 5)], 1u << (row & 31));
}
template <int NV>
__global__ __launch_bounds__(256) void decode_kernel(DecodeArgs a) {
    const int lane = threadIdx.x & 63;
    const int row = blockIdx.x * 4 + (threadIdx.x >> 6);
    if (row >= a.n_rows) return;
    const int D = a.D, D4 = D >> 2;
    const int32_t* idx_row = a.idx + (size_t)row * a.code_stride;
    const float* val_row = a.val + (size_t)row * a.code_stride;

    f32x4 acc[NV];
#pragma unroll
    for (int n = 0; n < NV; ++n) {
        const int q = lane + 64 * n;
        acc[n] = (q < D4) ? reinterpret_cast<const f32x4*>(a.b_dec)[q] : f32x4{0.f, 0.f, 0.f, 0.f};
    }
    gather_rows_accum<NV>(acc, a.W_dec, D, D4, idx_row, val_row, a.k, a.idx_limit, lane);

    if (a.x == nullptr) {
#pragma unroll
        for (int n = 0; n < NV; ++n) {
            const int q = lane + 64 * n;
            if (q < D4) reinterpret_cast<f32x4*>(a.x_hat + (size_t)row * D)[q] = acc[n];
        }
        return;
    }
    const float u = a.upper ? fmaxf(*a.upper, 1e-12f) : 1.0f;
    float sse_scaled = 0.f;
    double sse64 = 0.0, sumsq64 = 0.0;
    f32x4 g[NV];
    const f32x4* xr = reinterpret_cast<const f32x4*>(a.x + (size_t)row * D);
#pragma unroll
    for (int n = 0; n < NV; ++n) {
        const int q = lane + 64 * n;
        g[n] = f32x4{0.f, 0.f, 0.f, 0.f};
        if (q < D4) {
            const f32x4 xv = xr[q];
            if (a.x_hat) reinterpret_cast<f32x4*>(a.x_hat + (size_t)row * D)[q] = acc[n];
#pragma unroll
            for (int e = 0; e < 4; ++e) {
                const float t = acc[n][e] / u - xv[e] / u;
                sse_scaled += t * t * u * u;
                g[n][e] = a.gscale * t * u;
                const float r = xv[e] - acc[n][e];
                sse64 += (double)r * (double)r;
                sumsq64 += (double)xv[e] * (double)xv[e];
            }
            if (a.training && a.g != nullptr) reinterpret_cast<f32x4*>(a.g + (size_t)row * D)[q] = g[n];
            if (a.training && a.gS != nullptr) {
                const size_t o = ((size_t)(q >> 3) * a.n_rows + row) * 8 + (q & 7);
                reinterpret_cast<f32x4*>(a.gS)[o] = g[n];
                if (a.xS != nullptr) reinterpret_cast<f32x4*>(a.xS)[o] = xv;
            }
        }
    }
    float l0 = 0.f, l1 = 0.f;
    for (int j = lane; j < a.k; j += 64) {
        const int32_t i = idx_row[j];
        const float v = val_row[j];
        if (i >= 0 && v != 0.f) {
            l0 += 1.f;
            l1 += fabsf(v);
            if (a.training && a.fired) a.fired[i] = 1;
        }
        csc_mark(a, i, row);
    }
    if (a.rowstats) {
        sse_scaled = wave_sum(sse_scaled);
        l0 = wave_sum(l0);
        l1 = wave_sum(l1);
        sse64 = wave_sum_d(sse64);
        sumsq64 = wave_sum_d(sumsq64);
        if (lane == 0) {
            RowStats rs;
            rs.sse_scaled = sse_scaled; rs.l0 = l0; rs.l1 = l1; rs.aux_sse = 0.f;
            rs.sse64 = sse64; rs.sumsq64 = sumsq64;
            a.rowstats[row] = rs;
        }
    }
}

template <int NW, int KH>
__global__ __launch_bounds__(64 * NW) void decode_q_kernel(DecodeArgs a) {
    __shared__ float sh_dv[NW][32 * KH];
    __shared__ float sh_f[NW];
    __shared__ double sh_d[NW][2];
    const int lane = threadIdx.x & 63;
    const int w = __builtin_amdgcn_readfirstlane(threadIdx.x >> 6);
    const int row = blockIdx.x;
    constexpr int D4 = 64 * NW;
    const int q = w * 64 + lane;
    const int32_t* idx_row = a.idx + (size_t)row * a.code_stride;
    const float* val_row = a.val + (size_t)row * a.code_stride;
    int32_t raw_i = -1;
    float raw_v = 0.f;
    if (lane < a.k) { raw_i = idx_row[lane]; raw_v = val_row[lane]; }
    const int32_t my_i = (raw_i < 0 || raw_i >= a.idx_limit) ? -1 : raw_i;
    f32x4 acc = reinterpret_cast<const f32x4*>(a.b_dec)[q];
    const f32x4 xv = reinterpret_cast<const f32x4*>(a.x + (size_t)row * a.D)[q];
    __builtin_amdgcn_sched_barrier(0);
    typedef int i32x4_ __attribute__((ext_vector_type(4)));
    const __amdgpu_buffer_rsrc_t wres = __builtin_amdgcn_make_buffer_rsrc(const_cast<float*>(a.W_dec), 0, (uint32_t)a.S * (uint32_t)(D4 * 16), 0x00020000);
    const uint32_t voff = (uint32_t)q * 16u;
    f32x4 wv[32];
#pragma unroll
    for (int h = 0; h < KH; ++h) {
#pragma unroll
        for (int j = 0; j < 32; ++j) {
            const int i = __builtin_amdgcn_readlane(my_i, 32 * h + j);
            const i32x4_ t = __builtin_amdgcn_raw_buffer_load_b128(wres, voff, (uint32_t)max(i, 0) * (uint32_t)(D4 * 16), 0);
            wv[j] = f32x4{__int_as_float(t[0]), __int_as_float(t[1]), __int_as_float(t[2]), __int_as_float(t[3])};
        }
        __builtin_amdgcn_sched_barrier(0);
#pragma unroll
        for (int j = 0; j < 32; ++j) {
            const int i = __builtin_amdgcn_readlane(my_i, 32 * h + j);
            const float v = __builtin_bit_cast(float, __builtin_amdgcn_readlane(__builtin_bit_cast(int, raw_v), 32 * h + j));
            if (i >= 0) acc += v * wv[j];
        }
        __builtin_amdgcn_sched_barrier(0);
    }
    if (a.x_hat) reinterpret_cast<f32x4*>(a.x_hat + (size_t)row * a.D)[q] = acc;
    const float u = a.upper ? fmaxf(*a.upper, 1e-12f) : 1.0f;
    float sse_scaled = 0.f;
    double sse64 = 0.0, sumsq64 = 0.0;
    f32x4 g;
#pragma unroll
    for (int e = 0; e < 4; ++e) {
        const float t = acc[e] / u - xv[e] / u;
        sse_scaled += t * t * u * u;
        g[e] = a.gscale * t * u;
        const float r = xv[e] - acc[e];
        sse64 += (double)r * (double)r;
        sumsq64 += (double)xv[e] * (double)xv[e];
    }
    if (a.training) {
        if (a.g != nullptr) reinterpret_cast<f32x4*>(a.g + (size_t)row * a.D)[q] = g;
        if (a.gS != nullptr) {
            const size_t o = ((size_t)(q >> 3) * a.n_rows + row) * 8 + (q & 7);
            reinterpret_cast<f32x4*>(a.gS)[o] = g;
            if (a.xS != nullptr) reinterpret_cast<f32x4*>(a.xS)[o] = xv;
        }
    }
#pragma unroll
    for (int hh = 0; hh < KH; ++hh) {
        const int h = KH - 1 - hh;
        if (hh > 0) {
#pragma unroll
            for (int j = 0; j < 32; ++j) {
                const int i = __builtin_amdgcn_readlane(my_i, 32 * h + j);
                const i32x4_ t = __builtin_amdgcn_raw_buffer_load_b128(wres, voff, (uint32_t)max(i, 0) * (uint32_t)(D4 * 16), 0);
                wv[j] = f32x4{__int_as_float(t[0]), __int_as_float(t[1]), __int_as_float(t[2]), __int_as_float(t[3])};
            }
            __builtin_amdgcn_sched_barrier(0);
        }
        float pd[32];
#pragma unroll
        for (int j = 0; j < 32; ++j) pd[j] = (g[0] * wv[j][0] + g[1] * wv[j][1]) + (g[2] * wv[j][2] + g[3] * wv[j][3]);
        const float r = wave_reduce_scatter32(pd, lane);
        if ((lane & 1) == 0) sh_dv[w][32 * h + (lane >> 1)] = r;
    }
    sse_scaled = wave_sum(sse_scaled);
    sse64 = wave_sum_d(sse64);
    sumsq64 = wave_sum_d(sumsq64);
    if (lane == 0) { sh_f[w] = sse_scaled; sh_d[w][0] = sse64; sh_d[w][1] = sumsq64; }
    __syncthreads();
    if (w != 0) return;
    if (lane < 32 * KH) {
        float s = sh_dv[0][lane];
#pragma unroll
        for (int v = 1; v < NW; ++v) s += sh_dv[v][lane];
        if (lane < a.k) a.dval_out[(size_t)row * a.code_stride + lane] = s;
    }
    float l0 = 0.f, l1 = 0.f;
    if (raw_i >= 0 && raw_v != 0.f) {
        l0 = 1.f;
        l1 = fabsf(raw_v);
        if (a.training && a.fired) a.fired[raw_i] = 1;
    }
    csc_mark(a, raw_i, row);
    if (a.rowstats) {
        l0 = wave_sum(l0);
        l1 = wave_sum(l1);
        if (lane == 0) {
            RowStats rs;
            float f = sh_f[0];
            double d0 = sh_d[0][0], d1 = sh_d[0][1];
#pragma unroll
            for (int v = 1; v < NW; ++v) { f += sh_f[v]; d0 += sh_d[v][0]; d1 += sh_d[v][1]; }
            rs.sse_scaled = f; rs.l0 = l0; rs.l1 = l1; rs.aux_sse = 0.f;
            rs.sse64 = d0; rs.sumsq64 = d1;
            a.rowstats[row] = rs;
        }
    }
}

template <int NV>
__global__ __launch_bounds__(256) void decode_matry_kernel(DecodeArgs a, MatryArgs m) {
    const int lane = threadIdx.x & 63;
    const int row = blockIdx.x * 4 + (threadIdx.x >> 6);
    if (row >= a.n_rows) return;
    const int D = a.D, D4 = D >> 2, P = m.P;
    const int32_t* idx_row = a.idx + (size_t)row * a.code_stride;
    const float* val_row = a.val + (size_t)row * a.code_stride;
    f32x4 acc[NV], xv[NV];
    const f32x4* xr = reinterpret_cast<const f32x4*>(a.x + (size_t)row * D);
#pragma unroll
    for (int n = 0; n < NV; ++n) {
        const int q = lane + 64 * n;
        acc[n] = (q < D4) ? reinterpret_cast<const f32x4*>(a.b_dec)[q] : f32x4{0.f, 0.f, 0.f, 0.f};
        xv[n] = (q < D4) ? xr[q] : f32x4{0.f, 0.f, 0.f, 0.f};
    }
    const float u = a.upper ? fmaxf(*a.upper, 1e-12f) : 1.0f;
    float sse_scaled = 0.f;
    double sse64 = 0.0, sumsq64 = 0.0;
    f32x4* Grow = reinterpret_cast<f32x4*>(m.G + (size_t)row * P * D);
    auto emit = [&](int p) {
        const bool last = (p == P - 1);
#pragma unroll
        for (int n = 0; n < NV; ++n) {
            const int q = lane + 64 * n;
            if (q < D4) {
                f32x4 g;
#pragma unroll
                for (int e = 0; e < 4; ++e) {
                    const float t = acc[n][e] / u - xv[n][e] / u;
                    sse_scaled += t * t * u * u;
                    g[e] = a.gscale * t * u;
                    if (last) {
                        const float r = xv[n][e] - acc[n][e];
                        sse64 += (double)r * (double)r;
                        sumsq64 += (double)xv[n][e] * (double)xv[n][e];
                    }
                }
                if (a.training) Grow[(size_t)p * D4 + q] = g;
                if (last && a.x_hat) reinterpret_cast<f32x4*>(a.x_hat + (size_t)row * D)[q] = acc[n];
            }
        }
    };
    int p = 0;
    for (int j0 = 0; j0 < a.k; j0 += 64) {
        const int cnt = min(64, a.k - j0);
        int32_t my_i = -1;
        float my_v = 0.f;
        if (lane < cnt) { my_i = idx_row[j0 + lane]; my_v = val_row[j0 + lane]; }
        for (int jj = 0; jj < cnt; ++jj) {
            const int32_t i = __shfl(my_i, jj, 64);
            const float v = __shfl(my_v, jj, 64);
            if (i < 0) continue;
            while (p < P - 1 && i >= m.cuts[p]) { emit(p); ++p; }
            const f32x4* wr = reinterpret_cast<const f32x4*>(a.W_dec + (size_t)i * D);
#pragma unroll
            for (int n = 0; n < NV; ++n) {
                const int q = lane + 64 * n;
                if (q < D4) acc[n] += v * wr[q];
            }
        }
    }
    while (p < P) { emit(p); ++p; }

    if (a.training) {
        f32x4 c[NV];
#pragma unroll
        for (int n = 0; n < NV; ++n) c[n] = f32x4{0.f, 0.f, 0.f, 0.f};
        for (int pp = P - 1; pp >= 0; --pp) {
#pragma unroll
            for (int n = 0; n < NV; ++n) {
                const int q = lane + 64 * n;
                if (q < D4) {
                    c[n] += Grow[(size_t)pp * D4 + q];
                    Grow[(size_t)pp * D4 + q] = c[n];
                    if (a.gS != nullptr) {
                        reinterpret_cast<f32x4*>(a.gS)[(((size_t)(q >> 3) * P + pp) * a.n_rows + row) * 8 + (q & 7)] = c[n];
                        if (pp == 0 && a.xS != nullptr) reinterpret_cast<f32x4*>(a.xS)[((size_t)(q >> 3) * a.n_rows + row) * 8 + (q & 7)] = xv[n];
                    }
                }
            }
        }
    }
    float l0 = 0.f, l1 = 0.f;
    for (int j = lane; j < a.k; j += 64) {
        const int32_t i = idx_row[j];
        const float v = val_row[j];
        if (i >= 0 && v != 0.f) {
            l0 += 1.f;
            l1 += fabsf(v);
            if (a.training && a.fired) a.fired[i] = 1;
        }
        csc_mark(a, i, row);
    }
    if (a.rowstats) {
        sse_scaled = wave_sum(sse_scaled);
        l0 = wave_sum(l0);
        l1 = wave_sum(l1);
        sse64 = wave_sum_d(sse64);
        sumsq64 = wave_sum_d(sumsq64);
        if (lane == 0) {
            RowStats rs;
            rs.sse_scaled = sse_scaled; rs.l0 = l0; rs.l1 = l1; rs.aux_sse = 0.f;
            rs.sse64 = sse64; rs.sumsq64 = sumsq64;
            a.rowstats[row] = rs;
        }
    }
}

template <int NW>
__global__ __launch_bounds__(64 * NW) void decode_matry_q_kernel(DecodeArgs a, MatryArgs m) {
    extern __shared__ __attribute__((aligned(16))) char matry_smem[];
    f32x4* const shG = reinterpret_cast<f32x4*>(matry_smem);
    __shared__ float sh_dv[NW][32];
    __shared__ float sh_f[NW];
    __shared__ double sh_d[NW][2];
    const int lane = threadIdx.x & 63;
    const int w = __builtin_amdgcn_readfirstlane(threadIdx.x >> 6);
    const int row = blockIdx.x;
    constexpr int D4 = 64 * NW;
    const int q = w * 64 + lane;
    const int P = m.P;
    const int32_t* idx_row = a.idx + (size_t)row * a.code_stride;
    const float* val_row = a.val + (size_t)row * a.code_stride;
    int32_t raw_i = -1;
    float raw_v = 0.f;
    if (lane < a.k) { raw_i = idx_row[lane]; raw_v = val_row[lane]; }
    const int32_t my_i = raw_i < 0 ? -1 : raw_i;
    f32x4 acc = reinterpret_cast<const f32x4*>(a.b_dec)[q];
    const f32x4 xv = reinterpret_cast<const f32x4*>(a.x + (size_t)row * a.D)[q];
    __builtin_amdgcn_sched_barrier(0);
    typedef int i32x4_ __attribute__((ext_vector_type(4)));
    const __amdgpu_buffer_rsrc_t wres = __builtin_amdgcn_make_buffer_rsrc(const_cast<float*>(a.W_dec), 0, (uint32_t)a.S * (uint32_t)(D4 * 16), 0x00020000);
    const uint32_t voff = (uint32_t)q * 16u;
    f32x4 wv[32];
#pragma unroll
    for (int j = 0; j < 32; ++j) {
        const int i = __builtin_amdgcn_readlane(my_i, j);
        const i32x4_ t = __builtin_amdgcn_raw_buffer_load_b128(wres, voff, (uint32_t)max(i, 0) * (uint32_t)(D4 * 16), 0);
        wv[j] = f32x4{__int_as_float(t[0]), __int_as_float(t[1]), __int_as_float(t[2]), __int_as_float(t[3])};
    }
    __builtin_amdgcn_sched_barrier(0);
    const float u = a.upper ? fmaxf(*a.upper, 1e-12f) : 1.0f;
    float sse_scaled = 0.f;
    double sse64 = 0.0, sumsq64 = 0.0;
    auto emit = [&](int p) {
        f32x4 g;
#pragma unroll
        for (int e = 0; e < 4; ++e) {
            const float t = acc[e] / u - xv[e] / u;
            sse_scaled += t * t * u * u;
            g[e] = a.gscale * t * u;
        }
        shG[p * D4 + q] = g;
    };
    int p = 0;
#pragma unroll
    for (int j = 0; j < 32; ++j) {
        const int i = __builtin_amdgcn_readlane(my_i, j);
        const float v = __builtin_bit_cast(float, __builtin_amdgcn_readlane(__builtin_bit_cast(int, raw_v), j));
        if (i >= 0) {
            while (p < P - 1 && i >= m.cuts[p]) { emit(p); ++p; }
            acc += v * wv[j];
        }
    }
    while (p < P) { emit(p); ++p; }
#pragma unroll
    for (int e = 0; e < 4; ++e) {
        const float r = xv[e] - acc[e];
        sse64 += (double)r * (double)r;
        sumsq64 += (double)xv[e] * (double)xv[e];
    }
    if (a.x_hat) reinterpret_cast<f32x4*>(a.x_hat + (size_t)row * a.D)[q] = acc;
    if (a.training) {
        f32x4 c = {0.f, 0.f, 0.f, 0.f};
        f32x4* const Grow = reinterpret_cast<f32x4*>(m.G + (size_t)row * P * a.D);
        for (int pp = P - 1; pp >= 0; --pp) {
            c += shG[pp * D4 + q];
            shG[pp * D4 + q] = c;
            if (pp == 0 || m.g_rows_all) Grow[(size_t)pp * D4 + q] = c;
            if (a.gS != nullptr) reinterpret_cast<f32x4*>(a.gS)[(((size_t)(q >> 3) * P + pp) * a.n_rows + row) * 8 + (q & 7)] = c;
        }
        if (a.gS != nullptr && a.xS != nullptr) reinterpret_cast<f32x4*>(a.xS)[((size_t)(q >> 3) * a.n_rows + row) * 8 + (q & 7)] = xv;
        float pd[32];
        int pb = 0;
#pragma unroll
        for (int j = 0; j < 32; ++j) {
            const int i = __builtin_amdgcn_readlane(my_i, j);
            pd[j] = 0.f;
            if (i >= 0) {
                while (pb < P - 1 && i >= m.cuts[pb]) ++pb;
                const f32x4 cj = shG[pb * D4 + q];
                pd[j] = (cj[0] * wv[j][0] + cj[1] * wv[j][1]) + (cj[2] * wv[j][2] + cj[3] * wv[j][3]);
            }
        }
        const float r = wave_reduce_scatter32(pd, lane);
        if ((lane & 1) == 0) sh_dv[w][lane >> 1] = r;
    }
    sse_scaled = wave_sum(sse_scaled);
    sse64 = wave_sum_d(sse64);
    sumsq64 = wave_sum_d(sumsq64);
    if (lane == 0) { sh_f[w] = sse_scaled; sh_d[w][0] = sse64; sh_d[w][1] = sumsq64; }
    __syncthreads();
    if (w != 0) return;
    if (a.training && lane < 32) {
        float s = sh_dv[0][lane];
#pragma unroll
        for (int v = 1; v < NW; ++v) s += sh_dv[v][lane];
        if (lane < a.k) a.dval_out[(size_t)row * a.code_stride + lane] = s;
    }
    float l0 = 0.f, l1 = 0.f;
    if (raw_i >= 0 && raw_v != 0.f) {
        l0 = 1.f;
        l1 = fabsf(raw_v);
        if (a.training && a.fired) a.fired[raw_i] = 1;
    }
    csc_mark(a, raw_i, row);
    if (a.rowstats) {
        l0 = wave_sum(l0);
        l1 = wave_sum(l1);
        if (lane == 0) {
            RowStats rs;
            float f = sh_f[0];
            double d0 = sh_d[0][0], d1 = sh_d[0][1];
#pragma unroll
            for (int v = 1; v < NW; ++v) { f += sh_f[v]; d0 += sh_d[v][0]; d1 += sh_d[v][1]; }
            rs.sse_scaled = f; rs.l0 = l0; rs.l1 = l1; rs.aux_sse = 0.f;
            rs.sse64 = d0; rs.sumsq64 = d1;
            a.rowstats[row] = rs;
        }
    }
}


__global__ __launch_bounds__(256) void csc_clear_kernel(CscArgs a) {
    if (a.k_dev && *a.k_dev <= 0) return;
    const size_t n4 = ((size_t)a.S * a.words) >> 2;
    uint4* bm = reinterpret_cast<uint4*>(a.bitmap);
    for (size_t q = (size_t)blockIdx.x * 256 + threadIdx.x; q < n4; q += (size_t)gridDim.x * 256) bm[q] = uint4{0, 0, 0, 0};
}

__device__ __forceinline__ void csc_fill_body(const CscArgs& a, int bid, int nblk) {
    const int k = a.k_dev ? min(*a.k_dev, a.k) : a.k;
    if (k <= 0) return;
    const long n = (long)a.n_rows * k;
    for (long p = (long)bid * blockDim.x + threadIdx.x; p < n; p += (long)nblk * blockDim.x) {
        const int b = (int)(p / k), j = (int)(p % k);
        const int32_t i = a.idx[(size_t)b * a.code_stride + j];
        if (i >= 0 && i < a.S) atomicOr(&a.bitmap[(size_t)i * a.words + (b >> 5)], 1u << (b & 31));
    }
}
__global__ void csc_fill_kernel(CscArgs a) { csc_fill_body(a, blockIdx.x, gridDim.x); }

__device__ __forceinline__ void csc_count_body(const CscArgs& a, int bid) {
    if (a.k_dev && *a.k_dev <= 0) return;
    const int lane = threadIdx.x & 63;
    const int i = bid * 4 + (threadIdx.x >> 6);
    if (i >= a.S) return;
    const int groups = a.words >> 3;
    const uint4* bm = reinterpret_cast<const uint4*>(a.bitmap + (size_t)i * a.words);
    int base = 0;
    for (int g0 = 0; g0 < groups; g0 += 64) {
        const int g = g0 + lane;
        int c = 0;
        if (g < groups) {
            const uint4 lo = bm[2 * g], hi = bm[2 * g + 1];
            c = __popc(lo.x) + __popc(lo.y) + __popc(lo.z) + __popc(lo.w) + __popc(hi.x) + __popc(hi.y) + __popc(hi.z) + __popc(hi.w);
        }
        int incl = c;
#pragma unroll
        for (int o = 1; o < 64; o <<= 1) {
            const int n = __shfl_up(incl, o, 64);
            if (lane >= o) incl += n;
        }
        if (g < groups) a.grp_prefix[(size_t)i * groups + g] = base + incl - c;
        base += __shfl(incl, 63, 64);
    }
    if (lane == 0) a.counts[i] = base;
}
__global__ __launch_bounds__(256) void csc_count_kernel(CscArgs a) { csc_count_body(a, blockIdx.x); }

__global__ __launch_bounds__(1024) void csc_scan_block_kernel(CscArgs a) {
    if (a.k_dev && *a.k_dev <= 0) return;
    __shared__ int wave_tot[16][3];
    const int tid = threadIdx.x, lane = tid & 63, w = tid >> 6;
    const int i = blockIdx.x * 1024 + tid;
    int v[3] = {0, 0, 0};
    if (i < a.S) {
        const int c = a.counts[i];
        const int nch = (c + DW_CHUNK - 1) / DW_CHUNK;
        v[0] = c; v[1] = max(1, nch); v[2] = nch > 1 ? nch : 0;
    }
    int incl[3] = {v[0], v[1], v[2]};
#pragma unroll
    for (int o = 1; o < 64; o <<= 1) {
#pragma unroll
        for (int q = 0; q < 3; ++q) {
            const int n = __shfl_up(incl[q], o, 64);
            if (lane >= o) incl[q] += n;
        }
    }
    if (lane == 63)
        for (int q = 0; q < 3; ++q) wave_tot[w][q] = incl[q];
    __syncthreads();
    int off[3] = {0, 0, 0};
    for (int j = 0; j < w; ++j)
        for (int q = 0; q < 3; ++q) off[q] += wave_tot[j][q];
    if (i < a.S) {
        a.starts[i] = off[0] + incl[0] - v[0];
        if (a.chunk_starts) {
            a.chunk_starts[i] = off[1] + incl[1] - v[1];
            a.part_starts[i] = off[2] + incl[2] - v[2];
        }
    }
    if (tid == 1023)
        for (int q = 0; q < 3; ++q) a.scan_totals[blockIdx.x * 3 + q] = off[q] + incl[q];
}
__global__ __launch_bounds__(1024) void csc_scan_offset_kernel(CscArgs a) {
    if (a.k_dev && *a.k_dev <= 0) return;
    __shared__ int base[3];
    const int tid = threadIdx.x, lane = tid & 63;
    if (tid < 64) {
        int s3[3] = {0, 0, 0};
        for (int b = lane; b < (int)blockIdx.x; b += 64)
            for (int q = 0; q < 3; ++q) s3[q] += a.scan_totals[b * 3 + q];
        for (int q = 0; q < 3; ++q) s3[q] = wave_sum_i(s3[q]);
        if (lane == 0)
            for (int q = 0; q < 3; ++q) base[q] = s3[q];
    }
    __syncthreads();
    const int i = blockIdx.x * 1024 + tid;
    if (i < a.S) {
        a.starts[i] += base[0];
        if (a.chunk_starts) { a.chunk_starts[i] += base[1]; a.part_starts[i] += base[2]; }
    }
    if (blockIdx.x == gridDim.x - 1 && tid == 0) {
        if (a.zero_word != nullptr) *a.zero_word = 0;
        a.starts[a.S] = base[0] + a.scan_totals[blockIdx.x * 3 + 0];
        if (a.chunk_starts) a.chunk_starts[a.S] = base[1] + a.scan_totals[blockIdx.x * 3 + 1];
    }
}

__global__ void csc_place_kernel(CscArgs a) {
    const int k = a.k_dev ? min(*a.k_dev, a.k) : a.k;
    if (k <= 0) return;
    const long n = (long)a.n_rows * k;
    const int groups = a.words >> 3;
    for (long p = (long)blockIdx.x * blockDim.x + threadIdx.x; p < max(n, (long)a.S); p += (long)gridDim.x * blockDim.x) {
        if (p < a.S && a.chunk_starts) {
            const int c1 = a.chunk_starts[p + 1];
            for (int c = a.chunk_starts[p]; c < c1; ++c) a.work_latent[c] = (int)p;
        }
        if (p >= n) continue;
        const int b = (int)(p / k), j = (int)(p % k);
        const int32_t i = a.idx[(size_t)b * a.code_stride + j];
        if (i < 0 || i >= a.S) continue;
        const int g = b >> 8, wi = (b >> 5) & 7;
        const uint4* grp = reinterpret_cast<const uint4*>(a.bitmap + (size_t)i * a.words + 8 * g);
        const uint4 lo = grp[0], hi = grp[1];
        const uint32_t wd[8] = {lo.x, lo.y, lo.z, lo.w, hi.x, hi.y, hi.z, hi.w};
        int rank = a.grp_prefix[(size_t)i * groups + g];
#pragma unroll
        for (int e = 0; e < 8; ++e) {
            const uint32_t m = e < wi ? 0xffffffffu : (e == wi ? ((1u << (b & 31)) - 1u) : 0u);
            rank += __popc(wd[e] & m);
        }
        const int slot = a.starts[i] + rank;
        if (a.pairs != nullptr) a.pairs[slot] = int2{b, (int)((size_t)b * a.code_stride + j)};
        if (a.pv != nullptr) {
            const int fl = (rank == 0 ? DWS_FIRST : 0) | (rank == a.counts[i] - 1 ? DWS_LAST : 0);
            int pblk = 0;
            if (a.P > 1) while (pblk < a.P - 1 && i >= a.cuts[pblk]) ++pblk;
            a.pv[slot] = int2{((pblk * a.n_rows + b) << 7) | fl, __float_as_int(a.val[(size_t)b * a.code_stride + j])};
            a.plat[slot] = i;
            if (a.pv2 != nullptr) a.pv2[slot] = int2{(b << 7) | fl, __float_as_int(a.dval[(size_t)b * a.code_stride + j])};
        }
    }
}


template <int NV>
__device__ __forceinline__ void write_row_proj(float2* row_proj, int i, const f32x4 (&g)[NV], const f32x4 (&w)[NV], int project,
                                               int lane) {
    float sc;
    const float sq = rpg_row_stats<NV>(g, w, project, &sc);
    if (lane == 0) row_proj[i] = float2{sc, sq};
}

template <int NV>
__device__ __forceinline__ float row_sumsq(const f32x4 (&g)[NV]) {
    float sq = 0.f;
#pragma unroll
    for (int n = 0; n < NV; ++n)
#pragma unroll
        for (int e = 0; e < 4; ++e) sq = __builtin_fmaf(g[n][e], g[n][e], sq);
    return wave_sum(sq);
}

#ifndef DW_MIN_WAVES
#define DW_MIN_WAVES 1
#endif
#ifndef DW_GROUP
#define DW_GROUP 8
#endif
template <int NV>
__global__ __launch_bounds__(256, DW_MIN_WAVES) void dw_rows_kernel(DwRowsArgs a) {
    if (a.k_dev && *a.k_dev <= 0) return;
    const int lane = threadIdx.x & 63;
    const int wi = a.chunk_starts[a.lat_lo] + blockIdx.x * 4 + (threadIdx.x >> 6);
    const int n_work = a.chunk_starts[a.lat_hi];
    if (wi >= n_work) return;
    const int i = a.work_latent[wi];
    const int c = wi - a.chunk_starts[i];
    const int nch = a.chunk_starts[i + 1] - a.chunk_starts[i];
    const int D = a.D, D4 = D >> 2;
    const int seg_beg = a.starts[i], seg_end = a.starts[i + 1];
    int pblk = 0;
    if (a.P > 1) while (pblk < a.P - 1 && i >= a.cuts[pblk]) ++pblk;
    const size_t g_stride = (size_t)a.P * D;
    const float* gbase = a.g + (size_t)pblk * D;
    const int beg = seg_beg + c * DW_CHUNK;
    const int end = min(seg_end, beg + DW_CHUNK);
    f32x4 accd[NV], acce[NV], wv[NV];
    {
        const f32x4* wr = reinterpret_cast<const f32x4*>(a.W_dec + (size_t)i * D);
#pragma unroll
        for (int n = 0; n < NV; ++n) {
            accd[n] = f32x4{0.f, 0.f, 0.f, 0.f};
            acce[n] = f32x4{0.f, 0.f, 0.f, 0.f};
            wv[n] = (a.part != 2 && lane + 64 * n < D4) ? wr[lane + 64 * n] : f32x4{0.f, 0.f, 0.f, 0.f};
        }
    }
    int my_b = 0;
    float my_v = 0.f, my_dv = 0.f;
    const int cnt = end - beg;
    const int part = a.part;
    if (lane < cnt) {
        const int2 pr = a.pairs[beg + lane];
        my_b = pr.x;
        my_v = a.val[pr.y];
        if (part == 2) my_dv = a.dval[beg + lane];
        if (a.clear_bitmap != nullptr) a.clear_bitmap[(size_t)i * a.clear_words + (my_b >> 5)] = 0u;
    }
    float dbs = 0.f;
    constexpr int G = DW_GROUP, GS = (G == 8 ? 3 : 4);
    for (int j0 = 0; j0 < cnt; j0 += G) {
        float p[G];
        float r = 0.f;
        if (part != 2) {
#pragma unroll
        for (int t = 0; t < G; t += 2) {
            p[t] = 0.f; p[t + 1] = 0.f;
            if (j0 + t >= cnt) continue;
            const bool two = j0 + t + 1 < cnt;
            const int b0 = __shfl(my_b, j0 + t, 64), b1 = __shfl(my_b, min(j0 + t + 1, 63), 64);
            const float v0 = __shfl(my_v, j0 + t, 64), v1 = two ? __shfl(my_v, min(j0 + t + 1, 63), 64) : 0.f;
            const f32x4* g0 = reinterpret_cast<const f32x4*>(gbase + (size_t)b0 * g_stride);
            const f32x4* g1 = reinterpret_cast<const f32x4*>(gbase + (size_t)(two ? b1 : b0) * g_stride);
            f32x4 tg0[NV], tg1[NV];
#pragma unroll
            for (int n = 0; n < NV; ++n) {
                const int q = lane + 64 * n;
                const bool ok = q < D4;
                tg0[n] = ok ? g0[q] : f32x4{0.f, 0.f, 0.f, 0.f};
                tg1[n] = ok ? g1[q] : f32x4{0.f, 0.f, 0.f, 0.f};
            }
#pragma unroll
            for (int n = 0; n < NV; ++n) {
                accd[n] += v0 * tg0[n];
                accd[n] += v1 * tg1[n];
                p[t] += tg0[n][0] * wv[n][0] + tg0[n][1] * wv[n][1] + tg0[n][2] * wv[n][2] + tg0[n][3] * wv[n][3];
                p[t + 1] += tg1[n][0] * wv[n][0] + tg1[n][1] * wv[n][1] + tg1[n][2] * wv[n][2] + tg1[n][3] * wv[n][3];
            }
            if (!two) p[t + 1] = 0.f;
        }
        r = wave_reduce_scatter<G>(p, lane);
        if (part == 1) {
            if ((lane & ((1 << GS) - 1)) == 0 && j0 + (lane >> GS) < cnt) a.dval[beg + j0 + (lane >> GS)] = r;
            continue;
        }
        }
#pragma unroll
        for (int t = 0; t < G; t += 2) {
            if (j0 + t >= cnt) continue;
            const bool two = j0 + t + 1 < cnt;
            const float e0 = part == 2 ? __shfl(my_dv, j0 + t, 64) : __shfl(r, t << GS, 64);
            const float e1 = !two ? 0.f : part == 2 ? __shfl(my_dv, min(j0 + t + 1, 63), 64) : __shfl(r, (t + 1) << GS, 64);
            dbs += e0 + e1;
            const int b0 = __shfl(my_b, j0 + t, 64), b1 = __shfl(my_b, min(j0 + t + 1, 63), 64);
            const f32x4* x0 = reinterpret_cast<const f32x4*>(a.x + (size_t)b0 * D);
            const f32x4* x1 = reinterpret_cast<const f32x4*>(a.x + (size_t)(two ? b1 : b0) * D);
            f32x4 tx0[NV], tx1[NV];
#pragma unroll
            for (int n = 0; n < NV; ++n) {
                const int q = lane + 64 * n;
                const bool ok = q < D4;
                tx0[n] = ok ? x0[q] : f32x4{0.f, 0.f, 0.f, 0.f};
                tx1[n] = ok ? x1[q] : f32x4{0.f, 0.f, 0.f, 0.f};
            }
#pragma unroll
            for (int n = 0; n < NV; ++n) {
                acce[n] += e0 * tx0[n];
                acce[n] += e1 * tx1[n];
            }
        }
    }

    float *od, *oe;
    bool direct = (nch == 1);
    if (direct) {
        od = a.dW_dec + (size_t)i * D;
        oe = a.dW_encT + (size_t)i * D;
    } else {
        od = a.partials + (size_t)(a.part_starts[i] + c) * 2 * D;
        oe = od + D;
    }
#pragma unroll
    for (int n = 0; n < NV; ++n) {
        const int q = lane + 64 * n;
        if (q < D4) {
            f32x4* pd = reinterpret_cast<f32x4*>(od) + q;
            f32x4* pe = reinterpret_cast<f32x4*>(oe) + q;
            if (part != 2) { if (direct && a.accumulate) *pd = *pd + accd[n]; else *pd = accd[n]; }
            if (part != 1) { if (direct && a.accumulate) *pe = *pe + acce[n]; else *pe = acce[n]; }
        }
    }
    if (lane == 0 && part != 1) {
        if (direct) a.db_enc[i] = a.accumulate ? (a.db_enc[i] + dbs) : dbs;
        else a.db_partials[a.part_starts[i] + c] = dbs;
    }
    if (a.row_proj != nullptr && direct && part != 2 && !a.accumulate) write_row_proj<NV>(a.row_proj, i, accd, wv, a.project, lane);
    if (a.enc_sq != nullptr && direct && part != 1 && !a.accumulate) {
        const float sq = row_sumsq<NV>(acce);
        if (lane == 0) a.enc_sq[i] = sq;
    }
}

template <int NV>
__global__ __launch_bounds__(256) void dw_combine_kernel(DwRowsArgs a) {
    if (a.k_dev && *a.k_dev <= 0) return;
    const int lane = threadIdx.x & 63;
    const int i = a.lat_lo + blockIdx.x * 4 + (threadIdx.x >> 6);
    if (i >= a.lat_hi) return;
    const int enc = blockIdx.y;
    if ((enc == 0 && a.part == 2) || (enc == 1 && a.part == 1)) return;
    const int nch = a.chunk_starts[i + 1] - a.chunk_starts[i];
    if (nch <= 1) return;
    const int c0 = a.part_starts[i], c1 = c0 + nch;
    const int D = a.D, D4 = D >> 2;
    const float* base = a.partials + (enc ? D : 0);
    f32x4 acc[NV];
#pragma unroll
    for (int n = 0; n < NV; ++n) acc[n] = f32x4{0.f, 0.f, 0.f, 0.f};
    float dbs = 0.f;
    int c = c0;
    constexpr int TRIP = NV <= 4 ? 8 : (NV <= 8 ? 4 : 2);
    for (; c + TRIP <= c1; c += TRIP) {
        f32x4 t[TRIP][NV];
#pragma unroll
        for (int u = 0; u < TRIP; ++u) {
            const f32x4* p = reinterpret_cast<const f32x4*>(base + (size_t)(c + u) * 2 * D);
#pragma unroll
            for (int n = 0; n < NV; ++n) t[u][n] = (lane + 64 * n < D4) ? p[lane + 64 * n] : f32x4{0.f, 0.f, 0.f, 0.f};
        }
#pragma unroll
        for (int n = 0; n < NV; ++n) {
            if constexpr (TRIP == 8) acc[n] += ((t[0][n] + t[1][n]) + (t[2][n] + t[3][n])) + ((t[4][n] + t[5][n]) + (t[6][n] + t[7][n]));
            else if constexpr (TRIP == 4) acc[n] += (t[0][n] + t[1][n]) + (t[2][n] + t[3][n]);
            else acc[n] += t[0][n] + t[1][n];
        }
        if (enc) {
#pragma unroll
            for (int u = 0; u < TRIP; ++u) dbs += a.db_partials[c + u];
        }
    }
    for (; c < c1; ++c) {
        const f32x4* p = reinterpret_cast<const f32x4*>(base + (size_t)c * 2 * D);
#pragma unroll
        for (int n = 0; n < NV; ++n)
            if (lane + 64 * n < D4) acc[n] += p[lane + 64 * n];
        if (enc) dbs += a.db_partials[c];
    }
    f32x4* o = reinterpret_cast<f32x4*>((enc ? a.dW_encT : a.dW_dec) + (size_t)i * D);
#pragma unroll
    for (int n = 0; n < NV; ++n) {
        const int q = lane + 64 * n;
        if (q < D4) o[q] = a.accumulate ? o[q] + acc[n] : acc[n];
    }
    if (enc) {
        if (lane == 0) a.db_enc[i] = a.accumulate ? (a.db_enc[i] + dbs) : dbs;
        if (a.enc_sq != nullptr && !a.accumulate) {
            const float sq = row_sumsq<NV>(acc);
            if (lane == 0) a.enc_sq[i] = sq;
        }
    } else if (a.row_proj != nullptr && !a.accumulate) {
// ... 21 lines not shown
}

__global__ __launch_bounds__(256) void slice_major_copy_kernel(const float* __restrict__ g, const float* __restrict__ x, int n, int D,
                                                               float* __restrict__ gS, float* __restrict__ xS) {
    const int lane = threadIdx.x & 63;
    const int row = blockIdx.x * 4 + (threadIdx.x >> 6);
    if (row >= n) return;
    const f32x4* gr = reinterpret_cast<const f32x4*>(g + (size_t)row * D);
    const f32x4* xr = reinterpret_cast<const f32x4*>(x + (size_t)row * D);
    for (int q = lane; q < (D >> 2); q += 64) {
        const size_t o = ((size_t)(q >> 3) * n + row) * 8 + (q & 7);
        reinterpret_cast<f32x4*>(gS)[o] = gr[q];
        reinterpret_cast<f32x4*>(xS)[o] = xr[q];
    }
}

template <bool DEC, bool DVAL = true>
__global__ __launch_bounds__(256, (DEC && DVAL) ? 4 : 5) void dw_slices_kernel(DwSlicesArgs a, int wg_per_slice) {
    constexpr bool PASS_A = DEC && DVAL;
    constexpr int L = DWS_RUN;
    const int lane = threadIdx.x & 63, gi = lane >> 3, li = lane & 7;
    const int xcd = blockIdx.x & 7, q = blockIdx.x >> 3;
    const int slice = xcd + 8 * (q / wg_per_slice);
    const bool sq_on = (DEC ? a.sq_wave_dec : a.sq_wave_enc) != nullptr;
    auto sq_slot = [&]() -> float* {
        return (DEC ? a.sq_wave_dec : a.sq_wave_enc) + ((size_t)blockIdx.x * 4 + __builtin_amdgcn_readfirstlane((int)(threadIdx.x >> 6)));
    };
    if (slice * DWS_SLICE >= a.D) { if (sq_on && lane == 0) *sq_slot() = 0.f; return; }
    const int NP = a.starts[a.S];
    const int run0 = ((q % wg_per_slice) * 4 + (threadIdx.x >> 6)) * 8;
    if (run0 * L >= NP) { if (sq_on && lane == 0) *sq_slot() = 0.f; return; }
    const int run = run0 + gi;
    const int col = slice * DWS_SLICE + li * 4;
    const uint32_t colb = (uint32_t)col * 4u, rowb = (uint32_t)a.D * 4u, li16 = (uint32_t)li * 16u;
    auto bound = [&](int r) -> int {
        const long nb = (long)r * L;
        if (nb >= NP) return NP;
        const int lat = a.plat[nb];
        const int s = a.starts[lat];
        return (a.starts[lat + 1] - s < L) ? s : (int)nb;
    };
    const int p0 = bound(run), p1 = bound(run + 1);
    const bool live = p0 < p1;
    const int2* const pv = DEC ? a.pv : a.pv2;
    float* const out = DEC ? a.dW_dec : a.dW_encT;
    float* const part = DEC ? a.part_dec : a.part_enc;
    f32x4 acc = {0.f, 0.f, 0.f, 0.f};
    f32x4 w4 = {0.f, 0.f, 0.f, 0.f};
    float* const dvp = PASS_A ? a.dvp + (size_t)slice * a.pair_cap : nullptr;
    __shared__ float sh_sq[256];
    sh_sq[threadIdx.x] = 0.f;
    const int sel = (lane & 56) << 2;
    const __amdgpu_buffer_rsrc_t mres = __builtin_amdgcn_make_buffer_rsrc(
        const_cast<float*>(DEC ? a.gS : a.xS) + (size_t)slice * a.n_rows * DWS_SLICE * (DEC && a.P > 1 ? a.P : 1), 0,
        (uint32_t)a.n_rows * 128u * (uint32_t)(DEC && a.P > 1 ? a.P : 1), 0x00020000);
    const __amdgpu_buffer_rsrc_t wres = __builtin_amdgcn_make_buffer_rsrc(const_cast<float*>(a.W_dec), 0, (uint32_t)a.S * rowb, 0x00020000);

    auto load_info = [&](int t, int2& e, int& lat) {
        const int p = p0 + 8 * t + li;
        e = int2{0, 0};
        lat = 0;
        if (p < p1) {
            const i32x2 v = reinterpret_cast<const i32x2*>(pv)[p];
            e = int2{v[0], v[1]};
            lat = a.plat[p];
            if (p == p1 - 1) e.x |= DWS_END;
            if (p == p0) e.x &= ~DWS_FIRST;
        }
    };
    constexpr int PB = 4;
    auto issue = [&](const int2& e, int lat, int j0, int (&xj)[PB], int (&lj)[PB], f32x4 (&gt)[PB], f32x4 (&wt)[PB]) {
#pragma unroll
        for (int j = 0; j < PB; ++j) {
            xj[j] = __builtin_amdgcn_ds_bpermute(sel + 4 * (j0 + j), e.x);
            lj[j] = __builtin_amdgcn_ds_bpermute(sel + 4 * (j0 + j), lat);
            gt[j] = buf_load16(mres, ((uint32_t)xj[j] & ~127u) | li16);
            if (PASS_A && (xj[j] & DWS_FIRST)) wt[j] = buf_load16(wres, (uint32_t)lj[j] * rowb + colb);
        }
    };
    auto consume = [&](const int2& e, int j0, const int (&xc)[PB], const int (&lc)[PB], const f32x4 (&gc)[PB], const f32x4 (&wc)[PB],
                       const f32x4& wnext0, bool& head_open, float& dmine) {
        float vc[PB];
#pragma unroll
        for (int j = 0; j < PB; ++j) vc[j] = __int_as_float(__builtin_amdgcn_ds_bpermute(sel + 4 * (j0 + j), e.y));
#pragma unroll
        for (int j = 0; j < PB; ++j) {
            if (PASS_A) {
                float d = gc[j][0] * w4[0] + gc[j][1] * w4[1] + gc[j][2] * w4[2] + gc[j][3] * w4[3];
                d = group8_sum(d);
                dmine = li == j0 + j ? d : dmine;
            }
            acc += vc[j] * gc[j];
            if (xc[j] & (DWS_LAST | DWS_END)) {
                float* o;
                if (head_open) o = part + ((size_t)run * 2 + 0) * a.D + col;
                else if (!(xc[j] & DWS_LAST)) o = part + ((size_t)run * 2 + 1) * a.D + col;
                else {
                    o = out + (size_t)lc[j] * a.D + col;
                    if (sq_on)
                        sh_sq[threadIdx.x] += __builtin_fmaf(acc[3], acc[3], __builtin_fmaf(acc[2], acc[2], __builtin_fmaf(acc[1], acc[1], acc[0] * acc[0])));
                }
                *reinterpret_cast<f32x4*>(o) = acc;
                if (DEC && slice == 0 && li == 0 && (xc[j] & DWS_END)) {
                    const int cl = (!head_open && !(xc[j] & DWS_LAST)) ? lc[j] : -1;
                    a.cut_lat[run] = cl;
                    if (cl >= 0 && a.cut_list != nullptr)
                        reinterpret_cast<i32x4*>(a.cut_list)[1 + atomicAdd(&a.cut_list[0], 1)] = i32x4{run, cl, a.starts[cl], a.starts[cl + 1]};
                }
                head_open = false;
                acc = f32x4{0.f, 0.f, 0.f, 0.f};
                if (PASS_A) w4 = j + 1 < PB ? wc[j + 1 < PB ? j + 1 : 0] : wnext0;
            }
        }
    };
    int2 e_c, e_n;
    int lat_c, lat_n;
    int xa[PB], xb[PB], la[PB], lb[PB];
    f32x4 ga[PB], gb[PB], wa[PB], wb[PB];
    bool head_open = false;
    load_info(0, e_c, lat_c);
    if (live) {
        head_open = (pv[p0].x & DWS_FIRST) == 0;
        if (PASS_A) w4 = buf_load16(wres, (uint32_t)a.plat[p0] * rowb + colb);
    }
    issue(e_c, lat_c, 0, xa, la, ga, wa);
    load_info(1, e_n, lat_n);
#pragma unroll 1
    for (int t = 0; __any(p0 + 8 * t < p1); ++t) {
        float dmine = 0.f;
        issue(e_c, lat_c, PB, xb, lb, gb, wb);
        consume(e_c, 0, xa, la, ga, wa, wb[0], head_open, dmine);
        issue(e_n, lat_n, 0, xa, la, ga, wa);
        consume(e_c, PB, xb, lb, gb, wb, wa[0], head_open, dmine);
        if (PASS_A && p0 + 8 * t + li < p1) dvp[p0 + 8 * t + li] = dmine;
        e_c = e_n; lat_c = lat_n;
        load_info(t + 2, e_n, lat_n);
    }
    if (sq_on) {
        const float sq = wave_sum(sh_sq[threadIdx.x]);
        if (lane == 0) *sq_slot() = sq;
    }
}

__global__ __launch_bounds__(256) void dw_dval_sum_kernel(DwSlicesArgs a) {
    const int NP = a.starts[a.S];
    const int p = blockIdx.x * 256 + threadIdx.x;
    if (p >= NP) return;
    const int n_slices = a.D / DWS_SLICE;
    float s = 0.f;
    for (int c = 0; c < n_slices; ++c) s += a.dvp[(size_t)c * a.pair_cap + p];
    const int2 e = a.pv[p];
    const int b = a.P > 1 ? (e.x >> 7) % a.n_rows : (e.x >> 7);
    a.pv2[p] = int2{(b << 7) | (e.x & 127), __float_as_int(s)};
    if (a.clear_bitmap != nullptr) a.clear_bitmap[(size_t)a.plat[p] * a.clear_words + (b >> 5)] = 0u;
}

__global__ __launch_bounds__(256) void dw_clear_bitmap_kernel(DwSlicesArgs a) {
    const int NP = a.starts[a.S];
    const int p = blockIdx.x * 256 + threadIdx.x;
    if (p >= NP) return;
    a.clear_bitmap[(size_t)a.plat[p] * a.clear_words + (a.pv2[p].x >> 12)] = 0u;
}

template <int NV>
__global__ __launch_bounds__(256) void dw_finalize_cut_kernel(DwSlicesArgs a, int kind0) {
    constexpr int L = DWS_RUN;
    __shared__ f32x4 sh[3][NV * 64];
    __shared__ float shdb[4];
    const int lane = threadIdx.x & 63, w = threadIdx.x >> 6;
    const int NP = a.starts[a.S];
    const int r0 = blockIdx.x;
    if ((long)(r0 + 1) * L >= NP) return;
    const int i = a.cut_lat[r0];
    if (i < 0) return;
    const int s = a.starts[i], e = a.starts[i + 1];
    const int r1 = (e - 1) / L;
    const int enc = blockIdx.y + kind0;
    const int D = a.D, D4 = D >> 2;
    const float* const part = enc ? a.part_enc : a.part_dec;
    const int nh = r1 - r0, ch = (nh + 3) / 4;
    const int ra = r0 + 1 + w * ch, rb = min(r1 + 1, ra + ch);
    f32x4 acc[NV];
#pragma unroll
    for (int n = 0; n < NV; ++n) acc[n] = f32x4{0.f, 0.f, 0.f, 0.f};
    int r = ra;
    constexpr int TRIP = NV <= 4 ? 4 : 2;
    for (; r + TRIP <= rb; r += TRIP) {
        f32x4 t[TRIP][NV];
#pragma unroll
        for (int u = 0; u < TRIP; ++u) {
            const f32x4* p = reinterpret_cast<const f32x4*>(part + (size_t)(r + u) * 2 * D);
#pragma unroll
            for (int n = 0; n < NV; ++n) t[u][n] = (lane + 64 * n < D4) ? p[lane + 64 * n] : f32x4{0.f, 0.f, 0.f, 0.f};
        }
#pragma unroll
        for (int n = 0; n < NV; ++n) {
            if constexpr (TRIP == 4) acc[n] += (t[0][n] + t[1][n]) + (t[2][n] + t[3][n]);
            else acc[n] += t[0][n] + t[1][n];
        }
    }
    for (; r < rb; ++r) {
        const f32x4* p = reinterpret_cast<const f32x4*>(part + (size_t)r * 2 * D);
#pragma unroll
        for (int n = 0; n < NV; ++n)
            if (lane + 64 * n < D4) acc[n] += p[lane + 64 * n];
    }
    float dbs = 0.f;
    if (enc) {
        const int cnt = e - s, q4 = (cnt + 3) / 4;
        const int pend = min(e, s + (w + 1) * q4);
        for (int p0 = s + w * q4 + lane; p0 < pend; p0 += 64 * 8) {
            float t[8];
#pragma unroll
            for (int u = 0; u < 8; ++u) t[u] = (p0 + 64 * u < pend) ? __int_as_float(a.pv2[p0 + 64 * u].y) : 0.f;
#pragma unroll
            for (int u = 0; u < 8; ++u)
                if (p0 + 64 * u < pend) dbs += t[u];
        }
        dbs = wave_sum(dbs);
    }
    if (w != 0) {
#pragma unroll
        for (int n = 0; n < NV; ++n) sh[w - 1][lane + 64 * n] = acc[n];
    }
    if (lane == 0) shdb[w] = dbs;
    __syncthreads();
    if (w != 0) return;
    {
        const f32x4* p = reinterpret_cast<const f32x4*>(part + ((size_t)r0 * 2 + 1) * D);
#pragma unroll
        for (int n = 0; n < NV; ++n) {
            const f32x4 t = (lane + 64 * n < D4) ? p[lane + 64 * n] : f32x4{0.f, 0.f, 0.f, 0.f};
            acc[n] = (((t + acc[n]) + sh[0][lane + 64 * n]) + sh[1][lane + 64 * n]) + sh[2][lane + 64 * n];
        }
    }
    float* const row = (enc ? a.dW_encT : a.dW_dec) + (size_t)i * D;
#pragma unroll
    for (int n = 0; n < NV; ++n)
        if (lane + 64 * n < D4) reinterpret_cast<f32x4*>(row)[lane + 64 * n] = acc[n];
    if (enc) {
        if (lane == 0) a.db_enc[i] = ((shdb[0] + shdb[1]) + shdb[2]) + shdb[3];
        if (a.enc_sq != nullptr) {
            const float sq = row_sumsq<NV>(acc);
            if (lane == 0) a.enc_sq[i] = sq;
        }
    } else if (a.row_proj != nullptr) {
        f32x4 wv[NV];
        const f32x4* wr = reinterpret_cast<const f32x4*>(a.W_dec + (size_t)i * D);
#pragma unroll
        for (int n = 0; n < NV; ++n) wv[n] = (lane + 64 * n < D4) ? wr[lane + 64 * n] : f32x4{0.f, 0.f, 0.f, 0.f};
        write_row_proj<NV>(a.row_proj, i, acc, wv, a.project, lane);
    }
}

template <int NV>
__global__ __launch_bounds__(256) void dw_finalize_kernel(DwSlicesArgs a, int kind0) {
    constexpr int L = DWS_RUN;
    const int lane = threadIdx.x & 63;
    const int i = blockIdx.x * 4 + (threadIdx.x >> 6);
    if (i >= a.S) return;
    const int enc = blockIdx.y + kind0;
    const int D = a.D, D4 = D >> 2;
    const int s = a.starts[i], e = a.starts[i + 1];
    if (!enc && a.lat_unused != nullptr && lane == 0) a.lat_unused[i] = e == s ? 1 : 0;
    if (e - s >= L && s / L != (e - 1) / L) return;
    float* const row = (enc ? a.dW_encT : a.dW_dec) + (size_t)i * D;
    f32x4 acc[NV], wv[NV];
    const bool proj = !enc && a.row_proj != nullptr;
    const f32x4* wr = reinterpret_cast<const f32x4*>(a.W_dec + (size_t)i * D);
#pragma unroll
    for (int n = 0; n < NV; ++n) {
        acc[n] = f32x4{0.f, 0.f, 0.f, 0.f};
        wv[n] = f32x4{0.f, 0.f, 0.f, 0.f};
        if (lane + 64 * n < D4) {
            if (e > s) acc[n] = reinterpret_cast<const f32x4*>(row)[lane + 64 * n];
            else if (!(enc && a.lat_unused != nullptr)) reinterpret_cast<f32x4*>(row)[lane + 64 * n] = acc[n];
            if (proj) wv[n] = wr[lane + 64 * n];
        }
    }
    if (enc) {
        float dbs = 0.f;
        for (int p = s + lane; p < e; p += 64) dbs += __int_as_float(a.pv2[p].y);
        dbs = wave_sum(dbs);
        if (lane == 0) a.db_enc[i] = dbs;
        if (a.enc_sq != nullptr) {
            const float sq = row_sumsq<NV>(acc);
            if (lane == 0) a.enc_sq[i] = sq;
        }
    } else if (proj) {
        write_row_proj<NV>(a.row_proj, i, acc, wv, a.project, lane);
    }
}

template <int NV>
__global__ __launch_bounds__(256) void dw_finalize_light_kernel(DwSlicesArgs a, int n_cut_blocks) {
    constexpr int L = DWS_RUN;
    __shared__ f32x4 sh[3][NV * 64];
    __shared__ float shdb[4];
    const int lane = threadIdx.x & 63, w = threadIdx.x >> 6;
    const int D = a.D, D4 = D >> 2;
    if ((int)blockIdx.x < n_cut_blocks) {
      const i32x4 first = reinterpret_cast<const i32x4*>(a.cut_list)[1 + (blockIdx.x >> 1)];
      const int n_items = 2 * a.cut_list[0];
      for (int item = blockIdx.x; item < n_items; item += n_cut_blocks) {
        const i32x4 ent = item == (int)blockIdx.x ? first : reinterpret_cast<const i32x4*>(a.cut_list)[1 + (item >> 1)];
        const int r0 = ent[0], i = ent[1], s = ent[2], e = ent[3], enc = item & 1;
        const int r1 = (e - 1) / L;
        const float* const part = enc ? a.part_enc : a.part_dec;
        f32x4 tp[NV], wv[NV];
        if (w == 0) {
            const f32x4* p = reinterpret_cast<const f32x4*>(part + ((size_t)r0 * 2 + 1) * D);
            const f32x4* wr = reinterpret_cast<const f32x4*>(a.W_dec + (size_t)i * D);
            const bool need_w = !enc && a.row_proj != nullptr;
#pragma unroll
            for (int n = 0; n < NV; ++n) {
                const bool ok = lane + 64 * n < D4;
                tp[n] = ok ? p[lane + 64 * n] : f32x4{0.f, 0.f, 0.f, 0.f};
                wv[n] = (ok && need_w) ? wr[lane + 64 * n] : f32x4{0.f, 0.f, 0.f, 0.f};
            }
        }
        const int nh = r1 - r0, ch = (nh + 3) / 4;
        const int ra = r0 + 1 + w * ch, rb = min(r1 + 1, ra + ch);
        f32x4 acc[NV];
#pragma unroll
        for (int n = 0; n < NV; ++n) acc[n] = f32x4{0.f, 0.f, 0.f, 0.f};
        constexpr int TRIP = NV <= 4 ? 4 : 2;
        int r = ra;
        for (; r + 2 * TRIP <= rb; r += 2 * TRIP) {
            f32x4 t[2 * TRIP][NV];
#pragma unroll
            for (int u = 0; u < 2 * TRIP; ++u) {
                const f32x4* p = reinterpret_cast<const f32x4*>(part + (size_t)(r + u) * 2 * D);
#pragma unroll
                for (int n = 0; n < NV; ++n) t[u][n] = (lane + 64 * n < D4) ? p[lane + 64 * n] : f32x4{0.f, 0.f, 0.f, 0.f};
            }
#pragma unroll
            for (int n = 0; n < NV; ++n) {
                if constexpr (TRIP == 4) {
                    acc[n] += (t[0][n] + t[1][n]) + (t[2][n] + t[3][n]);
                    acc[n] += (t[4][n] + t[5][n]) + (t[6][n] + t[7][n]);
                } else {
                    acc[n] += t[0][n] + t[1][n];
                    acc[n] += t[2][n] + t[3][n];
                }
            }
        }
        for (; r + TRIP <= rb; r += TRIP) {
            f32x4 t[TRIP][NV];
#pragma unroll
            for (int u = 0; u < TRIP; ++u) {
                const f32x4* p = reinterpret_cast<const f32x4*>(part + (size_t)(r + u) * 2 * D);
#pragma unroll
                for (int n = 0; n < NV; ++n) t[u][n] = (lane + 64 * n < D4) ? p[lane + 64 * n] : f32x4{0.f, 0.f, 0.f, 0.f};
            }
#pragma unroll
            for (int n = 0; n < NV; ++n) {
                if constexpr (TRIP == 4) acc[n] += (t[0][n] + t[1][n]) + (t[2][n] + t[3][n]);
                else acc[n] += t[0][n] + t[1][n];
            }
        }
        for (; r < rb; ++r) {
            const f32x4* p = reinterpret_cast<const f32x4*>(part + (size_t)r * 2 * D);
#pragma unroll
            for (int n = 0; n < NV; ++n)
                if (lane + 64 * n < D4) acc[n] += p[lane + 64 * n];
        }
        float dbs = 0.f;
        if (enc) {
            const int cnt = e - s, q4 = (cnt + 3) / 4;
            const int pend = min(e, s + (w + 1) * q4);
            for (int p0 = s + w * q4 + lane; p0 < pend; p0 += 64 * 8) {
                int2 pe[8];
#pragma unroll
                for (int u = 0; u < 8; ++u) pe[u] = (p0 + 64 * u < pend) ? a.pv2[p0 + 64 * u] : int2{0, 0};
#pragma unroll
                for (int u = 0; u < 8; ++u) {
                    if (p0 + 64 * u < pend) {
                        dbs += __int_as_float(pe[u].y);
                        if (a.clear_bitmap != nullptr) a.clear_bitmap[(size_t)i * a.clear_words + (pe[u].x >> 12)] = 0u;
                    }
                }
            }
            dbs = wave_sum(dbs);
        }
        if (w != 0) {
#pragma unroll
            for (int n = 0; n < NV; ++n) sh[w - 1][lane + 64 * n] = acc[n];
        }
        if (lane == 0) shdb[w] = dbs;
        __syncthreads();
        if (w == 0) {
#pragma unroll
            for (int n = 0; n < NV; ++n) acc[n] = (((tp[n] + acc[n]) + sh[0][lane + 64 * n]) + sh[1][lane + 64 * n]) + sh[2][lane + 64 * n];
            float* const row = (enc ? a.dW_encT : a.dW_dec) + (size_t)i * D;
#pragma unroll
            for (int n = 0; n < NV; ++n)
                if (lane + 64 * n < D4) reinterpret_cast<f32x4*>(row)[lane + 64 * n] = acc[n];
            if (enc) {
                if (lane == 0) a.db_enc[i] = ((shdb[0] + shdb[1]) + shdb[2]) + shdb[3];
                if (a.enc_sq != nullptr) {
                    const float sq = row_sumsq<NV>(acc);
                    if (lane == 0) a.enc_sq[i] = sq;
                }
            } else if (a.row_proj != nullptr) {
                write_row_proj<NV>(a.row_proj, i, acc, wv, a.project, lane);
            }
        }
        __syncthreads();
      }
      return;
    }
    const int li = lane & 7;
    const int i = ((int)blockIdx.x - n_cut_blocks) * 32 + (int)(threadIdx.x >> 3);
    if (i >= a.S) return;
    const int s = a.starts[i], e = a.starts[i + 1];
    if (a.lat_unused != nullptr && li == 0) a.lat_unused[i] = e == s ? 1 : 0;
    if (e - s >= L && s / L != (e - 1) / L) return;
    if (e == s) {
        if (a.lat_unused == nullptr) {
            for (int q = li; q < D4; q += 8) {
                reinterpret_cast<f32x4*>(a.dW_dec + (size_t)i * D)[q] = f32x4{0.f, 0.f, 0.f, 0.f};
                reinterpret_cast<f32x4*>(a.dW_encT + (size_t)i * D)[q] = f32x4{0.f, 0.f, 0.f, 0.f};
            }
        }
        if (li == 0) {
            a.db_enc[i] = 0.f;
            if (a.enc_sq != nullptr) a.enc_sq[i] = 0.f;
            if (a.row_proj != nullptr) a.row_proj[i] = float2{0.f, 0.f};
        }
        return;
    }
    auto group_tree = [&](float (&v)[8]) -> float {
        float r = ((v[0] + v[4]) + (v[2] + v[6])) + ((v[1] + v[5]) + (v[3] + v[7]));
        r += __shfl_xor(r, 4, 64);
        r += __shfl_xor(r, 2, 64);
        r += __shfl_xor(r, 1, 64);
        return r;
    };
    float gsq = 0.f, esq = 0.f;
    const bool waves_hold_squares = a.sq_wave_dec != nullptr;
    if (!waves_hold_squares) {
        const f32x4* gd = reinterpret_cast<const f32x4*>(a.dW_dec + (size_t)i * D);
        const f32x4* ge = reinterpret_cast<const f32x4*>(a.dW_encT + (size_t)i * D);
#pragma unroll 4
        for (int q = li; q < D4; q += 8) {
            const f32x4 u = gd[q], v = ge[q];
            gsq = __builtin_fmaf(u[3], u[3], __builtin_fmaf(u[2], u[2], __builtin_fmaf(u[1], u[1], __builtin_fmaf(u[0], u[0], gsq))));
            esq = __builtin_fmaf(v[3], v[3], __builtin_fmaf(v[2], v[2], __builtin_fmaf(v[1], v[1], __builtin_fmaf(v[0], v[0], esq))));
        }
        gsq += __shfl_xor(gsq, 4, 64); gsq += __shfl_xor(gsq, 2, 64); gsq += __shfl_xor(gsq, 1, 64);
        esq += __shfl_xor(esq, 4, 64); esq += __shfl_xor(esq, 2, 64); esq += __shfl_xor(esq, 1, 64);
    }
    float dv8[8], dt8[8];
#pragma unroll
    for (int j = 0; j < 8; ++j) {
        float dbs = 0.f, dot = 0.f;
#pragma unroll
        for (int t = 0; t < 2; ++t) {
            const int p = s + li + 8 * j + 64 * t;
            if (p < e) {
                const int2 pd = a.pv2[p];
                const float dv = __int_as_float(pd.y);
                dbs += dv;
                dot = __builtin_fmaf(__int_as_float(a.pv[p].y), dv, dot);
                if (a.clear_bitmap != nullptr) a.clear_bitmap[(size_t)i * a.clear_words + (pd.x >> 12)] = 0u;
            }
        }
        dv8[j] = dbs; dt8[j] = dot;
    }
    const float dbs = group_tree(dv8), dot = group_tree(dt8);
    if (li == 0) {
        a.db_enc[i] = dbs;
        if (a.enc_sq != nullptr) a.enc_sq[i] = esq;
        if (a.row_proj != nullptr) {
            const float nsq = a.wn2[i];
            const float sc = (a.project && nsq > 0.f) ? dot / nsq : 0.f;
            a.row_proj[i] = float2{sc, waves_hold_squares ? -sc * dot : fmaxf(__builtin_fmaf(-sc, dot, gsq), 0.f)};
        }
    }
}

__global__ __launch_bounds__(256) void transpose_kernel(const float* __restrict__ in, float* __restrict__ out, int S,
                                                        int D, double* __restrict__ sq_part) {
    __shared__ float tile[64][65];
    __shared__ double sh[4];
    const int s0 = blockIdx.x * 64, d0 = blockIdx.y * 64;
    const int c4 = (threadIdx.x & 15) * 4, r0 = threadIdx.x >> 4;
    float q0 = 0.f, q1 = 0.f, q2 = 0.f, q3 = 0.f;
#pragma unroll
    for (int r = r0; r < 64; r += 16) {
        const int s = s0 + r, d = d0 + c4;
        f32x4 v = f32x4{0.f, 0.f, 0.f, 0.f};
        if (s < S && d < D) v = *reinterpret_cast<const f32x4*>(in + (size_t)s * D + d);
        tile[r][c4] = v[0]; tile[r][c4 + 1] = v[1]; tile[r][c4 + 2] = v[2]; tile[r][c4 + 3] = v[3];
        q0 += v[0] * v[0]; q1 += v[1] * v[1]; q2 += v[2] * v[2]; q3 += v[3] * v[3];
    }
    if (sq_part != nullptr) {
        const double q = wave_sum_d((double)q0 + (double)q1 + (double)q2 + (double)q3);
        if ((threadIdx.x & 63) == 0) sh[threadIdx.x >> 6] = q;
    }
    __syncthreads();
    if (sq_part != nullptr && threadIdx.x == 0) sq_part[(size_t)blockIdx.y * gridDim.x + blockIdx.x] = sh[0] + sh[1] + sh[2] + sh[3];
#pragma unroll
    for (int r = r0; r < 64; r += 16) {
        const int d = d0 + r, s = s0 + c4;
        if (d < D && s < S)
            *reinterpret_cast<f32x4*>(out + (size_t)d * S + s) = f32x4{tile[c4][r], tile[c4 + 1][r], tile[c4 + 2][r], tile[c4 + 3][r]};
    }
}


template <bool ABSMAX>
__global__ __launch_bounds__(256) void colsum_partial_kernel(const float* m, int n_rows, int D, float* partials,
                                                             const int32_t* k_dev, long row_stride, float* wg_absmax,
                                                             int col_mult) {
    if (k_dev && *k_dev <= 0) return;
    const int Dfull = D;
    if (k_dev && col_mult > 0) D = min(D, (*k_dev * col_mult + 3) & ~3);
    float amax = 0.f;
    const int r0 = blockIdx.x * 64;
    const int r1 = min(n_rows, r0 + 64);
    for (int q = threadIdx.x; q < (D >> 2); q += 256) {
        f32x4 s = {0.f, 0.f, 0.f, 0.f};
        int r = r0;
        for (; r + 8 <= r1; r += 8) {
            f32x4 v[8];
#pragma unroll
            for (int u = 0; u < 8; ++u) v[u] = reinterpret_cast<const f32x4*>(m + (size_t)(r + u) * row_stride)[q];
            s += ((v[0] + v[1]) + (v[2] + v[3])) + ((v[4] + v[5]) + (v[6] + v[7]));
            if constexpr (ABSMAX) {
#pragma unroll
                for (int u = 0; u < 8; ++u)
                    amax = fmaxf(fmaxf(fmaxf(amax, fabsf(v[u][0])), fabsf(v[u][1])), fmaxf(fabsf(v[u][2]), fabsf(v[u][3])));
            }
        }
        for (; r < r1; ++r) {
            const f32x4 v = reinterpret_cast<const f32x4*>(m + (size_t)r * row_stride)[q];
            s += v;
            if constexpr (ABSMAX) amax = fmaxf(fmaxf(fmaxf(amax, fabsf(v[0])), fabsf(v[1])), fmaxf(fabsf(v[2]), fabsf(v[3])));
        }
        reinterpret_cast<f32x4*>(partials + (size_t)blockIdx.x * Dfull)[q] = s;
    }
    if constexpr (ABSMAX) {
        __shared__ float sh[4];
        for (int o = 32; o > 0; o >>= 1) amax = fmaxf(amax, __shfl_xor(amax, o, 64));
        if ((threadIdx.x & 63) == 0) sh[threadIdx.x >> 6] = amax;
        __syncthreads();
        if (threadIdx.x == 0) wg_absmax[blockIdx.x] = fmaxf(fmaxf(sh[0], sh[1]), fmaxf(sh[2], sh[3]));
    }
}
__global__ __launch_bounds__(256) void colsum_final_kernel(const float* partials, int n_blocks, int D, float* out,
                                                           int accumulate, const int32_t* k_dev, float out_scale, int col_mult,
                                                           const float* wg_absmax, float* absmax_out,
                                                           saev_step_stats* zero_stats, int32_t* zero_flag) {
    if (k_dev && *k_dev <= 0) return;
    if (blockIdx.x == 0 && absmax_out != nullptr) {
        __shared__ float shm[4];
        float m = 0.f;
        for (int i = threadIdx.x; i < n_blocks; i += 256) m = fmaxf(m, wg_absmax[i]);
        m = wave_max(m);
        if ((threadIdx.x & 63) == 0) shm[threadIdx.x >> 6] = m;
        __syncthreads();
        if (threadIdx.x == 0) {
            *absmax_out = fmaxf(fmaxf(shm[0], shm[1]), fmaxf(shm[2], shm[3]));
            if (zero_stats != nullptr) *zero_stats = saev_step_stats{};
            if (zero_flag != nullptr) *zero_flag = 0;
        }
    }
    if (k_dev && col_mult > 0 && (int)blockIdx.x * 64 >= *k_dev * col_mult) return;
    __shared__ float part[4][64];
    const int col = threadIdx.x & 63, slice = threadIdx.x >> 6;
    const int d = blockIdx.x * 64 + col;
    float s0 = 0.f, s1 = 0.f, s2 = 0.f, s3 = 0.f;
    if (d < D) {
        int b = slice;
        for (; b + 12 < n_blocks; b += 16) {
            s0 += partials[(size_t)b * D + d];
            s1 += partials[(size_t)(b + 4) * D + d];
            s2 += partials[(size_t)(b + 8) * D + d];
            s3 += partials[(size_t)(b + 12) * D + d];
        }
        for (; b < n_blocks; b += 4) s0 += partials[(size_t)b * D + d];
    }
    part[slice][col] = (s0 + s1) + (s2 + s3);
    __syncthreads();
    if (slice == 0 && d < D) {
        const float s = (part[0][col] + part[1][col]) + (part[2][col] + part[3][col]);
        out[d] = accumulate ? out[d] + s * out_scale : s * out_scale;
    }
}

struct ColsumPlain { const float* m; int n_rows, D; float* partials; long row_stride; float* out; int n_blocks; int slice_major; };
__device__ __forceinline__ void colsum_partial_plain(const ColsumPlain& c, int bid) {
    const int r0 = bid * 64, r1 = min(c.n_rows, r0 + 64);
    for (int q = threadIdx.x; q < (c.D >> 2); q += 256) {
        const f32x4* const base = c.slice_major ? reinterpret_cast<const f32x4*>(c.m) + (size_t)(q >> 3) * c.n_rows * 8 + (q & 7)
                                                : reinterpret_cast<const f32x4*>(c.m) + q;
        const size_t pitch = c.slice_major ? (size_t)8 : (size_t)(c.row_stride >> 2);
        f32x4 s = {0.f, 0.f, 0.f, 0.f};
        int r = r0;
        for (; r + 8 <= r1; r += 8) {
            f32x4 v[8];
#pragma unroll
            for (int u = 0; u < 8; ++u) v[u] = base[(size_t)(r + u) * pitch];
            s += ((v[0] + v[1]) + (v[2] + v[3])) + ((v[4] + v[5]) + (v[6] + v[7]));
        }
        for (; r < r1; ++r) s += base[(size_t)r * pitch];
        reinterpret_cast<f32x4*>(c.partials + (size_t)bid * c.D)[q] = s;
    }
}
__device__ __forceinline__ void colsum_final_plain(const ColsumPlain& c, int bid, float (&part)[4][64]) {
    const int col = threadIdx.x & 63, slice = threadIdx.x >> 6;
    const int d = bid * 64 + col;
    float s0 = 0.f, s1 = 0.f, s2 = 0.f, s3 = 0.f;
    if (d < c.D && slice < 4) {
        int b = slice;
        for (; b + 12 < c.n_blocks; b += 16) {
            s0 += c.partials[(size_t)b * c.D + d];
            s1 += c.partials[(size_t)(b + 4) * c.D + d];
            s2 += c.partials[(size_t)(b + 8) * c.D + d];
            s3 += c.partials[(size_t)(b + 12) * c.D + d];
        }
        for (; b < c.n_blocks; b += 4) s0 += c.partials[(size_t)b * c.D + d];
    }
    if (slice < 4) part[slice][col] = (s0 + s1) + (s2 + s3);
    __syncthreads();
    if (slice == 0 && d < c.D) c.out[d] = ((part[0][col] + part[1][col]) + (part[2][col] + part[3][col])) * 1.0f;
}
__global__ __launch_bounds__(1024) void csc_scan_fused_kernel(CscArgs a, int n_scan, ColsumPlain c, int have_colsum) {
    __shared__ int wave_tot[16][3];
    __shared__ int base[3];
    __shared__ float part[4][64];
    const int tid = threadIdx.x, lane = tid & 63, w = tid >> 6;
    if ((int)blockIdx.x >= n_scan) {
        if (have_colsum) colsum_final_plain(c, (int)blockIdx.x - n_scan, part);
        return;
    }
    const int blk = blockIdx.x;
    const int i = blk * 1024 + tid;
    int v[3] = {0, 0, 0};
    if (i < a.S) {
        const int cn = a.counts[i];
        const int nch = (cn + DW_CHUNK - 1) / DW_CHUNK;
        v[0] = cn; v[1] = max(1, nch); v[2] = nch > 1 ? nch : 0;
    }
    int incl[3] = {v[0], v[1], v[2]};
#pragma unroll
    for (int o = 1; o < 64; o <<= 1) {
#pragma unroll
        for (int q = 0; q < 3; ++q) {
            const int n = __shfl_up(incl[q], o, 64);
            if (lane >= o) incl[q] += n;
        }
    }
    if (lane == 63)
        for (int q = 0; q < 3; ++q) wave_tot[w][q] = incl[q];
    __syncthreads();
    int off[3] = {0, 0, 0};
    for (int j = 0; j < w; ++j)
        for (int q = 0; q < 3; ++q) off[q] += wave_tot[j][q];
    int32_t* const agg = a.scan_totals;
    if (tid == 1023) {
        for (int q = 0; q < 3; ++q) __hip_atomic_store(&agg[blk * 4 + q], off[q] + incl[q], __ATOMIC_RELAXED, __HIP_MEMORY_SCOPE_AGENT);
        __hip_atomic_store(&agg[blk * 4 + 3], a.epoch, __ATOMIC_RELEASE, __HIP_MEMORY_SCOPE_AGENT);
    }
    if (tid < 64) {
        int s3[3] = {0, 0, 0};
        for (int b = lane; b < blk; b += 64) {
            while (__hip_atomic_load(&agg[b * 4 + 3], __ATOMIC_ACQUIRE, __HIP_MEMORY_SCOPE_AGENT) != a.epoch) __builtin_amdgcn_s_sleep(1);
            for (int q = 0; q < 3; ++q) s3[q] += __hip_atomic_load(&agg[b * 4 + q], __ATOMIC_RELAXED, __HIP_MEMORY_SCOPE_AGENT);
        }
        for (int q = 0; q < 3; ++q) s3[q] = wave_sum_i(s3[q]);
        if (lane == 0)
            for (int q = 0; q < 3; ++q) base[q] = s3[q];
    }
    __syncthreads();
    if (i < a.S) {
        a.starts[i] = base[0] + off[0] + incl[0] - v[0];
        if (a.chunk_starts) {
            a.chunk_starts[i] = base[1] + off[1] + incl[1] - v[1];
            a.part_starts[i] = base[2] + off[2] + incl[2] - v[2];
        }
    }
    if (blk == n_scan - 1 && tid == 1023) {
        if (a.zero_word != nullptr) *a.zero_word = 0;
        a.starts[a.S] = base[0] + off[0] + incl[0];
        if (a.chunk_starts) a.chunk_starts[a.S] = base[1] + off[1] + incl[1];
    }
}
__global__ __launch_bounds__(256) void csc_fill_colsum_kernel(CscArgs a, int n_fill, ColsumPlain c) {
    if ((int)blockIdx.x < n_fill) csc_fill_body(a, blockIdx.x, n_fill);
    else colsum_partial_plain(c, blockIdx.x - n_fill);
}
__global__ __launch_bounds__(256) void csc_count_colpart_kernel(CscArgs a, int n_count, ColsumPlain c) {
    if ((int)blockIdx.x < c.n_blocks) colsum_partial_plain(c, blockIdx.x);
    else csc_count_body(a, blockIdx.x - c.n_blocks);
}
__global__ __launch_bounds__(256) void csc_count_colsum_kernel(CscArgs a, int n_count, ColsumPlain c) {
    __shared__ float part[4][64];
    if ((int)blockIdx.x < n_count) csc_count_body(a, blockIdx.x);
    else colsum_final_plain(c, blockIdx.x - n_count, part);
}

template <typename F>
hipError_t dispatch_nv(int D, F&& f) {
    const int nv = (D / 4 + 63) / 64;
    switch (nv) {
        case 1: f(std::integral_constant<int, 1>()); break;
        case 2: f(std::integral_constant<int, 2>()); break;
        case 3: f(std::integral_constant<int, 3>()); break;
        case 4: f(std::integral_constant<int, 4>()); break;
        case 5: f(std::integral_constant<int, 5>()); break;
        case 6: f(std::integral_constant<int, 6>()); break;
        case 7: case 8: f(std::integral_constant<int, 8>()); break;
        case 9: case 10: case 11: case 12: f(std::integral_constant<int, 12>()); break;
        case 13: case 14: case 15: case 16: f(std::integral_constant<int, 16>()); break;
        default: return hipErrorInvalidValue;
    }
    return hipGetLastError();
}

}

bool decode_forms_dval(int D, int k) { return k <= 64 && D % 256 == 0 && D >= 256 && D <= 1280; }
bool decode_matry_forms_dval(int D, int k) { return k <= 32 && D % 256 == 0 && D >= 256 && D <= 1024; }
hipError_t launch_decode(const DecodeArgs& a, hipStream_t stream) {
    if (a.n_rows <= 0) return hipSuccess;
    if (a.dval_out != nullptr && a.x != nullptr && decode_forms_dval(a.D, a.k)) {
#define DQ(NW)                                                                                                             \
    if (a.k <= 32) hipLaunchKernelGGL((decode_q_kernel<NW, 1>), dim3(a.n_rows), dim3(64 * NW), 0, stream, a);              \
    else hipLaunchKernelGGL((decode_q_kernel<NW, 2>), dim3(a.n_rows), dim3(64 * NW), 0, stream, a)
        switch (a.D / 256) {
            case 1: DQ(1); break;
            case 2: DQ(2); break;
            case 3: DQ(3); break;
            case 4: DQ(4); break;
            default: DQ(5); break;
        }
#undef DQ
        return hipGetLastError();
    }
    return dispatch_nv(a.D, [&](auto nv) {
        hipLaunchKernelGGL(decode_kernel<decltype(nv)::value>, dim3((a.n_rows + 3) / 4), dim3(256), 0, stream, a);
    });
}
hipError_t launch_decode_matry(const DecodeArgs& a, const MatryArgs& m, hipStream_t stream) {
    if (a.n_rows <= 0) return hipSuccess;
    if (a.dval_out != nullptr && a.x != nullptr && a.training && decode_matry_forms_dval(a.D, a.k)) {
        const size_t smem = (size_t)m.P * a.D * sizeof(float);
        static bool attr_set = false;
        if (!attr_set) {
            const void* fns[4] = {reinterpret_cast<const void*>(&decode_matry_q_kernel<1>), reinterpret_cast<const void*>(&decode_matry_q_kernel<2>),
                                  reinterpret_cast<const void*>(&decode_matry_q_kernel<3>), reinterpret_cast<const void*>(&decode_matry_q_kernel<4>)};
            for (const void* f : fns) {
                hipError_t e = hipFuncSetAttribute(f, hipFuncAttributeMaxDynamicSharedMemorySize, MAX_PREFIXES * 1024 * (int)sizeof(float));
                if (e != hipSuccess) return e;
            }
            attr_set = true;
        }
        switch (a.D / 256) {
            case 1: hipLaunchKernelGGL(decode_matry_q_kernel<1>, dim3(a.n_rows), dim3(64), smem, stream, a, m); break;
            case 2: hipLaunchKernelGGL(decode_matry_q_kernel<2>, dim3(a.n_rows), dim3(128), smem, stream, a, m); break;
            case 3: hipLaunchKernelGGL(decode_matry_q_kernel<3>, dim3(a.n_rows), dim3(192), smem, stream, a, m); break;
            default: hipLaunchKernelGGL(decode_matry_q_kernel<4>, dim3(a.n_rows), dim3(256), smem, stream, a, m); break;
        }
        return hipGetLastError();
    }
    return dispatch_nv(a.D, [&](auto nv) {
        hipLaunchKernelGGL(decode_matry_kernel<decltype(nv)::value>, dim3((a.n_rows + 3) / 4), dim3(256), 0, stream, a, m);
    });
}
hipError_t launch_csc_build(const CscArgs& a, hipStream_t stream, bool bitmap_clean, const float* colsum_m, int colsum_D,
                            long colsum_row_stride, float* colsum_partials, float* colsum_out, bool prefilled, bool colsum_slice_major) {
    if (a.n_rows <= 0) return hipSuccess;
    const long n = (long)a.n_rows * a.k;
    const int blocks = prefilled ? 0 : (int)std::min<long>((n + 255) / 256, 4096);
    const int place_blocks = (int)std::min<long>((std::max<long>(n, a.S) + 255) / 256, 8192);
    if (!bitmap_clean && !prefilled) hipLaunchKernelGGL(csc_clear_kernel, dim3(2048), dim3(256), 0, stream, a);
    const int n_scan = (a.S + 1023) / 1024;
    ColsumPlain c{colsum_m, a.n_rows, colsum_D, colsum_partials, colsum_row_stride > 0 ? colsum_row_stride : (long)colsum_D,
                  colsum_out, (a.n_rows + 63) / 64, colsum_slice_major ? 1 : 0};
    int colsum_in_scan = 0;
    if (colsum_m != nullptr && prefilled && a.epoch != 0) {
        hipLaunchKernelGGL(csc_count_colpart_kernel, dim3((a.S + 3) / 4 + c.n_blocks), dim3(256), 0, stream, a, (a.S + 3) / 4, c);
        colsum_in_scan = 1;
    } else if (colsum_m != nullptr) {
        hipLaunchKernelGGL(csc_fill_colsum_kernel, dim3(blocks + c.n_blocks), dim3(256), 0, stream, a, blocks, c);
        hipLaunchKernelGGL(csc_count_colsum_kernel, dim3((a.S + 3) / 4 + (colsum_D + 63) / 64), dim3(256), 0, stream, a, (a.S + 3) / 4, c);
    } else {
        if (blocks > 0) hipLaunchKernelGGL(csc_fill_kernel, dim3(blocks), dim3(256), 0, stream, a);
        hipLaunchKernelGGL(csc_count_kernel, dim3((a.S + 3) / 4), dim3(256), 0, stream, a);
    }
    if (a.epoch != 0 && n_scan <= 128) {
        hipLaunchKernelGGL(csc_scan_fused_kernel, dim3(n_scan + (colsum_in_scan ? (colsum_D + 63) / 64 : 0)), dim3(1024), 0, stream, a, n_scan, c,
                           colsum_in_scan);
    } else {
        hipLaunchKernelGGL(csc_scan_block_kernel, dim3(n_scan), dim3(1024), 0, stream, a);
        hipLaunchKernelGGL(csc_scan_offset_kernel, dim3(n_scan), dim3(1024), 0, stream, a);
    }
    hipLaunchKernelGGL(csc_place_kernel, dim3(place_blocks), dim3(256), 0, stream, a);
    return hipGetLastError();
}
hipError_t launch_dw_rows(const DwRowsArgs& a, int max_work, hipStream_t stream) {
    return dispatch_nv(a.D, [&](auto nv) {
        hipLaunchKernelGGL(dw_rows_kernel<decltype(nv)::value>, dim3((max_work + 3) / 4), dim3(256), 0, stream, a);
        hipLaunchKernelGGL(dw_combine_kernel<decltype(nv)::value>, dim3((a.lat_hi - a.lat_lo + 3) / 4, 2), dim3(256), 0, stream, a);
    });
}
hipError_t launch_slice_major_copy(const float* g, const float* x, int n, int D, float* gS, float* xS, hipStream_t stream) {
    if (n <= 0) return hipSuccess;
    hipLaunchKernelGGL(slice_major_copy_kernel, dim3((n + 3) / 4), dim3(256), 0, stream, g, x, n, D, gS, xS);
    return hipGetLastError();
}
int dw_slices_waves(int D, int max_pairs) {
    const int n_runs = (max_pairs + DWS_RUN - 1) / DWS_RUN;
    return ((D / DWS_SLICE + 7) / 8) * 8 * ((n_runs + 31) / 32) * 4;
}
hipError_t launch_dw_slices(const DwSlicesArgs& a_in, int max_pairs, int part, hipStream_t stream) {
    DwSlicesArgs a = a_in;
    if (a.D % DWS_SLICE != 0 || max_pairs <= 0) return hipErrorInvalidValue;
    const int n_runs = (max_pairs + DWS_RUN - 1) / DWS_RUN;
    const int wg_per_slice = (n_runs + 31) / 32;
    const int grid = ((a.D / DWS_SLICE + 7) / 8) * 8 * wg_per_slice;
    const bool light = part == 0 && a.have_dval && a.wn2 != nullptr;
    if (!light) { a.sq_wave_dec = nullptr; a.sq_wave_enc = nullptr; }
    if (part != 2 && a.have_dval) {
        hipLaunchKernelGGL((dw_slices_kernel<true, false>), dim3(grid), dim3(256), 0, stream, a, wg_per_slice);
        if (a.clear_bitmap != nullptr && !light) hipLaunchKernelGGL(dw_clear_bitmap_kernel, dim3((max_pairs + 255) / 256), dim3(256), 0, stream, a);
    } else if (part != 2) {
        hipLaunchKernelGGL(dw_slices_kernel<true>, dim3(grid), dim3(256), 0, stream, a, wg_per_slice);
        hipLaunchKernelGGL(dw_dval_sum_kernel, dim3((max_pairs + 255) / 256), dim3(256), 0, stream, a);
    }
    if (part != 1) hipLaunchKernelGGL(dw_slices_kernel<false>, dim3(grid), dim3(256), 0, stream, a, wg_per_slice);
    const int kinds = part == 0 ? 2 : 1, kind0 = part == 2 ? 1 : 0;
    if (light) {
        const int n_cut = a.cut_list != nullptr ? std::min(2 * (n_runs - 1), 8192) : 0;
        if (a.cut_list == nullptr && n_runs > 1) return hipErrorInvalidValue;
        return dispatch_nv(a.D, [&](auto nv) {
            hipLaunchKernelGGL(dw_finalize_light_kernel<decltype(nv)::value>, dim3(n_cut + (a.S + 31) / 32), dim3(256), 0, stream, a, n_cut);
        });
    }
    return dispatch_nv(a.D, [&](auto nv) {
        if (n_runs > 1) hipLaunchKernelGGL(dw_finalize_cut_kernel<decltype(nv)::value>, dim3(n_runs - 1, kinds), dim3(256), 0, stream, a, kind0);
        hipLaunchKernelGGL(dw_finalize_kernel<decltype(nv)::value>, dim3((a.S + 3) / 4, kinds), dim3(256), 0, stream, a, kind0);
    });
}
hipError_t launch_transpose(const float* in, float* out, int S, int D, hipStream_t stream, double* sq_part) {
    hipLaunchKernelGGL(transpose_kernel, dim3((S + 63) / 64, (D + 63) / 64), dim3(256), 0, stream, in, out, S, D, sq_part);
    return hipGetLastError();
}
int transpose_blocks(int S, int D) { return ((S + 63) / 64) * ((D + 63) / 64); }
hipError_t launch_colsum(const float* m, int n_rows, int D, float* partials, float* out, int accumulate,
                         const int32_t* k_dev, hipStream_t stream, long row_stride, float out_scale, int col_mult) {
    const int nb = (n_rows + 63) / 64;
    if (nb <= 0) return hipSuccess;
    hipLaunchKernelGGL(colsum_partial_kernel<false>, dim3(nb), dim3(256), 0, stream, m, n_rows, D, partials, k_dev,
                       row_stride > 0 ? row_stride : (long)D, (float*)nullptr, col_mult);
    hipLaunchKernelGGL(colsum_final_kernel, dim3((D + 63) / 64), dim3(256), 0, stream, partials, nb, D, out,
                       accumulate, k_dev, out_scale, col_mult, (const float*)nullptr, (float*)nullptr, (saev_step_stats*)nullptr,
                       (int32_t*)nullptr);
    return hipGetLastError();
}
hipError_t launch_colsum_absmax(const float* m, int n_rows, int D, float* partials, float* out, float* wg_scratch,
                                float* absmax_out, hipStream_t stream, float out_scale, saev_step_stats* zero_stats,
                                int32_t* zero_flag) {
    const int nb = (n_rows + 63) / 64;
    if (nb <= 0) return hipSuccess;
    hipLaunchKernelGGL(colsum_partial_kernel<true>, dim3(nb), dim3(256), 0, stream, m, n_rows, D, partials,
                       (const int32_t*)nullptr, (long)D, wg_scratch, 0);
    hipLaunchKernelGGL(colsum_final_kernel, dim3((D + 63) / 64), dim3(256), 0, stream, partials, nb, D, out, 0,
                       (const int32_t*)nullptr, out_scale, 0, (const float*)wg_scratch, absmax_out, zero_stats, zero_flag);
    return hipGetLastError();
}
```

Baseline: 6.432 million.

## Replace bitmap CSC build with per-row-block histogram count, prefix and place

The default CSC (latent-major) construction no longer uses a per-latent row bitmap. Instead, each 64-row block builds an LDS histogram of latent counts, a column-wise prefix over blocks gives per-block offsets and totals, and a place kernel assigns slots by in-block rank. This removes the bitmap clearing, the prefill in decode and the clears inside the dW kernels, all of which wrote to a large S×words array. In exchange it adds a blocks×S count array and heavy LDS atomics. The old bitmap path stays only for the debug route and batch-topk.

```diff
diff --git a/saev_amd/csrc/ctx.h b/saev_amd/csrc/ctx.h
--- a/saev_amd/csrc/ctx.h
+++ b/saev_amd/csrc/ctx.h
@@ -48,17 +48,14 @@
     float *val = nullptr, *aux_val = nullptr;
     float *x_hat = nullptr, *g = nullptr, *g_aux = nullptr;
     RowStats* rowstats = nullptr;
+    uint16_t* csc_blk = nullptr;
+    bool csc_blk_wide = false;
+    bool csc_bitmap_build = false;
     uint32_t* bitmap = nullptr;
     int32_t* grp_prefix = nullptr;
     int32_t* scan_totals = nullptr;
     int32_t csc_epoch = 0;
-    int bitmap_words = 0;
     int back_rows = 0;
-    int bitmap_words_last = 0;
-    bool bitmap_clean = false;
-    int bitmap_clean_words = 0;
-    int bitmap_prefill_words = 0, bitmap_prefill_rows = 0;
-    bool last_backward_gathered = false;
     int32_t *counts = nullptr, *starts = nullptr;
     int2* pairs = nullptr;
     float* colsum_partials = nullptr;
diff --git a/saev_amd/csrc/ctx.hip b/saev_amd/csrc/ctx.hip
--- a/saev_amd/csrc/ctx.hip
+++ b/saev_amd/csrc/ctx.hip
@@ -121,9 +121,15 @@
     if (KA > 0) { A(aux_idx, MB * KA); A(aux_val, MB * KA); A(g_aux, MB * D); A(dead_list, S); }
     A(x_hat, MB * D); A(g, MB * D);
     A(rowstats, MB);
-    c->bitmap_words = (int)(((MBB + 31) / 32 + 7) / 8 * 8);
-    A(bitmap, S * c->bitmap_words);
-    A(grp_prefix, S * (c->bitmap_words / 8));
+    c->csc_bitmap_build = c->dbg.csc_route == 1 || btk;
+    if (c->csc_bitmap_build) {
+        const long words = ((MBB + 31) / 32 + 7) / 8 * 8;
+        A(bitmap, S * words);
+        A(grp_prefix, S * (words / 8));
+    } else {
+        c->csc_blk_wide = MBB > 65535;
+        A(csc_blk, ((MBB + CSC_BLK_ROWS - 1) / CSC_BLK_ROWS) * ((S + 3) / 4 * 4) * (c->csc_blk_wide ? 2 : 1));
+    }
     A(scan_totals, ((S + 1023) / 1024) * 4);
     A(counts, S); A(starts, S + 1); A(pairs, MBB * K); A(dval_pairs, MBB * (size_t)cfg->top_k);
     {
diff --git a/saev_amd/csrc/ctx_backward.hip b/saev_amd/csrc/ctx_backward.hip
--- a/saev_amd/csrc/ctx_backward.hip
+++ b/saev_amd/csrc/ctx_backward.hip
@@ -16,6 +16,7 @@
     c->row_proj_valid = false;
     CscArgs a{};
     a.idx = ov ? c->ov_idx : c->idx; a.code_stride = K; a.k = K; a.k_dev = nullptr; a.n_rows = n; a.S = S;
+    a.blk = c->csc_blk; a.blk_wide = c->csc_blk_wide ? 1 : 0;
     a.bitmap = c->bitmap; a.words = words; a.grp_prefix = c->grp_prefix; a.scan_totals = c->scan_totals;
     a.counts = c->counts; a.starts = c->starts; a.pairs = c->pairs;
     a.chunk_starts = c->chunk_starts; a.part_starts = c->part_starts; a.work_latent = c->work_latent;
@@ -50,13 +51,8 @@
         REQUIRE(c, c->dws_rows == n, SAEV_INVALID_ARG, "saev_backward_begin: the forward in flight left no gradient rows");
         gmat = c->gS;
     }
-    const bool prefilled = !ov && c->bitmap_prefill_words == words && c->bitmap_prefill_rows == n;
-    HIPCHK(c, launch_csc_build(a, s, c->bitmap_clean && words <= c->bitmap_clean_words, gmat, D, (long)c->P_last * D,
-                               c->colsum_partials, c->grads + c->off_b_dec, prefilled, g_slices));
-    c->bitmap_prefill_words = 0;
-    c->last_backward_gathered = ov;
-    c->bitmap_clean = false;
-    c->bitmap_words_last = words;
+    HIPCHK(c, launch_csc_build(a, s, c->csc_bitmap_build, gmat, D, (long)c->P_last * D, c->colsum_partials, c->grads + c->off_b_dec,
+                               g_slices));
     if (c->aux_route != AUX_NONE) {
         int rc = auxk_backward(c, s);
         if (rc != SAEV_OK) return rc;
@@ -96,8 +92,6 @@
     a.lat_lo = lat_lo; a.lat_hi = lat_hi;
     a.part = part; a.dval = c->dval_pairs;
     const bool all_rows = part == 0 && lat_lo == 0 && lat_hi == S;
-    const bool clears = part != 2 && lat_lo == 0 && lat_hi == S && c->bitmap_words_last > 0;
-    if (clears) { a.clear_bitmap = c->bitmap; a.clear_words = c->bitmap_words_last; }
     a.row_proj = all_rows ? c->row_proj : nullptr; a.project = c->cfg.remove_parallel_grads ? 1 : 0;
     a.enc_sq = all_rows ? c->enc_sq : nullptr;
     const int max_work = (lat_hi - lat_lo) + (int)(((long)n * K + DW_CHUNK - 1) / DW_CHUNK);
@@ -113,7 +107,6 @@
         w.lat_unused = (all_rows && c->fused_step) ? c->lat_unused : nullptr;
         c->unused_valid = w.lat_unused != nullptr;
         w.row_proj = a.row_proj; w.project = a.project; w.enc_sq = a.enc_sq;
-        w.clear_bitmap = a.clear_bitmap; w.clear_words = a.clear_words;
         w.have_dval = c->dval_pairs_ready ? 1 : 0;
         c->sq_wave_n = 0;
         if (c->dval_pairs_ready && c->wn2_fresh && part == 0) {
@@ -141,7 +134,6 @@
     if (ov && c->aux_route != AUX_NONE && part != 2 && lat_lo == 0)
         HIPCHK(c, launch_colsum(c->db_aux, 1, D, c->colsum_partials, c->grads + c->off_b_dec, 1, nullptr, s));
     c->row_proj_valid = all_rows;
-    if (clears) { c->bitmap_clean = true; c->bitmap_clean_words = c->bitmap_words_last; }
     return SAEV_OK;
 }
 
diff --git a/saev_amd/csrc/ctx_forward.hip b/saev_amd/csrc/ctx_forward.hip
--- a/saev_amd/csrc/ctx_forward.hip
+++ b/saev_amd/csrc/ctx_forward.hip
@@ -592,15 +592,6 @@
     if (c->dws_rows == n && c->dval_rows != nullptr && (c->P == 1 || decode_matry_forms_dval(D, K))) { a.dval_out = c->dval_rows; c->dval_fwd = true; }
     c->g_rows_valid = !(c->train_fused && training && c->P == 1 && c->dws_rows == n);
     if (!c->g_rows_valid) a.g = nullptr;
-    c->bitmap_prefill_words = 0;
-    if (training && c->dbg.csc_route == 0 && c->bitmap != nullptr && c->bitmap_clean && !c->last_backward_gathered) {
-        const int words = ((n + 31) / 32 + 7) / 8 * 8;
-        if (words <= c->bitmap_clean_words) {
-            a.csc_bitmap = c->bitmap; a.csc_words = words;
-            c->bitmap_prefill_words = words; c->bitmap_prefill_rows = n;
-            c->bitmap_clean = false;
-        }
-    }
     if (c->P > 1) {
         MatryArgs m{};
         m.P = c->P;
diff --git a/saev_amd/csrc/kernels.h b/saev_amd/csrc/kernels.h
--- a/saev_amd/csrc/kernels.h
+++ b/saev_amd/csrc/kernels.h
@@ -140,8 +140,6 @@
     float* gS;
     float* xS;
     float* dval_out;
-    uint32_t* csc_bitmap;
-    int csc_words;
 };
 hipError_t launch_decode(const DecodeArgs& a, hipStream_t stream);
 bool decode_forms_dval(int D, int k);
@@ -156,11 +154,15 @@
 };
 hipError_t launch_decode_matry(const DecodeArgs& a, const MatryArgs& m, hipStream_t stream);
 
+constexpr int CSC_BLK_ROWS = 64;
+constexpr int CSC_LDS_LATENTS = 131072;
 struct CscArgs {
     const int32_t* idx;
     int code_stride, k;
     const int32_t* k_dev;
     int n_rows, S;
+    void* blk;
+    int blk_wide;
     uint32_t* bitmap;
     int words;
     int32_t* grp_prefix;
@@ -181,9 +183,9 @@
     int32_t* zero_word;
     int32_t epoch;
 };
-hipError_t launch_csc_build(const CscArgs& a, hipStream_t stream, bool bitmap_clean = false, const float* colsum_m = nullptr,
+hipError_t launch_csc_build(const CscArgs& a, hipStream_t stream, bool via_bitmap = false, const float* colsum_m = nullptr,
                             int colsum_D = 0, long colsum_row_stride = 0, float* colsum_partials = nullptr,
-                            float* colsum_out = nullptr, bool prefilled = false,
+                            float* colsum_out = nullptr,
                             bool colsum_slice_major = false);
 
 constexpr int DW_CHUNK = 64;
@@ -214,8 +216,6 @@
     float2* row_proj;
     int project;
     float* enc_sq;
-    uint32_t* clear_bitmap;
-    int clear_words;
 };
 hipError_t launch_dw_rows(const DwRowsArgs& a, int max_work, hipStream_t stream);
 
@@ -242,8 +242,6 @@
     float2* row_proj;
     int project;
     float* enc_sq;
-    uint32_t* clear_bitmap;
-    int clear_words;
     int32_t* lat_unused;
     int have_dval;
     const float* wn2;
diff --git a/saev_amd/csrc/sparse.hip b/saev_amd/csrc/sparse.hip
--- a/saev_amd/csrc/sparse.hip
+++ b/saev_amd/csrc/sparse.hip
@@ -66,9 +66,6 @@
     return p[0] + __shfl_xor(p[0], 1, 64);
 }
 
-__device__ __forceinline__ void csc_mark(const DecodeArgs& a, int32_t i, int row) {
-    if (a.csc_bitmap != nullptr && i >= 0 && i < a.S) atomicOr(&a.csc_bitmap[(size_t)i * a.csc_words + (row >> 5)], 1u << (row & 31));
-}
 template <int NV>
 __global__ __launch_bounds__(256) void decode_kernel(DecodeArgs a) {
     const int lane = threadIdx.x & 63;
@@ -132,7 +129,6 @@
             l1 += fabsf(v);
             if (a.training && a.fired) a.fired[i] = 1;
         }
-        csc_mark(a, i, row);
     }
     if (a.rowstats) {
         sse_scaled = wave_sum(sse_scaled);
@@ -247,7 +243,6 @@
         l1 = fabsf(raw_v);
         if (a.training && a.fired) a.fired[raw_i] = 1;
     }
-    csc_mark(a, raw_i, row);
     if (a.rowstats) {
         l0 = wave_sum(l0);
         l1 = wave_sum(l1);
@@ -356,7 +351,6 @@
             l1 += fabsf(v);
             if (a.training && a.fired) a.fired[i] = 1;
         }
-        csc_mark(a, i, row);
     }
     if (a.rowstats) {
         sse_scaled = wave_sum(sse_scaled);
@@ -480,7 +474,6 @@
         l1 = fabsf(raw_v);
         if (a.training && a.fired) a.fired[raw_i] = 1;
     }
-    csc_mark(a, raw_i, row);
     if (a.rowstats) {
         l0 = wave_sum(l0);
         l1 = wave_sum(l1);
@@ -705,7 +698,6 @@
         my_b = pr.x;
         my_v = a.val[pr.y];
         if (part == 2) my_dv = a.dval[beg + lane];
-        if (a.clear_bitmap != nullptr) a.clear_bitmap[(size_t)i * a.clear_words + (my_b >> 5)] = 0u;
     }
     float dbs = 0.f;
     constexpr int G = DW_GROUP, GS = (G == 8 ? 3 : 4);
@@ -1033,14 +1025,6 @@
     const int2 e = a.pv[p];
     const int b = a.P > 1 ? (e.x >> 7) % a.n_rows : (e.x >> 7);
     a.pv2[p] = int2{(b << 7) | (e.x & 127), __float_as_int(s)};
-    if (a.clear_bitmap != nullptr) a.clear_bitmap[(size_t)a.plat[p] * a.clear_words + (b >> 5)] = 0u;
-}
-
-__global__ __launch_bounds__(256) void dw_clear_bitmap_kernel(DwSlicesArgs a) {
-    const int NP = a.starts[a.S];
-    const int p = blockIdx.x * 256 + threadIdx.x;
-    if (p >= NP) return;
-    a.clear_bitmap[(size_t)a.plat[p] * a.clear_words + (a.pv2[p].x >> 12)] = 0u;
 }
 
 template <int NV>
@@ -1258,7 +1242,6 @@
                 for (int u = 0; u < 8; ++u) {
                     if (p0 + 64 * u < pend) {
                         dbs += __int_as_float(pe[u].y);
-                        if (a.clear_bitmap != nullptr) a.clear_bitmap[(size_t)i * a.clear_words + (pe[u].x >> 12)] = 0u;
                     }
                 }
             }
@@ -1344,7 +1327,6 @@
                 const float dv = __int_as_float(pd.y);
                 dbs += dv;
                 dot = __builtin_fmaf(__int_as_float(a.pv[p].y), dv, dot);
-                if (a.clear_bitmap != nullptr) a.clear_bitmap[(size_t)i * a.clear_words + (pd.x >> 12)] = 0u;
             }
         }
         dv8[j] = dbs; dt8[j] = dot;
@@ -1508,15 +1490,10 @@
     __syncthreads();
     if (slice == 0 && d < c.D) c.out[d] = ((part[0][col] + part[1][col]) + (part[2][col] + part[3][col])) * 1.0f;
 }
-__global__ __launch_bounds__(1024) void csc_scan_fused_kernel(CscArgs a, int n_scan, ColsumPlain c, int have_colsum) {
+__global__ __launch_bounds__(1024) void csc_scan_fused_kernel(CscArgs a, int n_scan) {
     __shared__ int wave_tot[16][3];
     __shared__ int base[3];
-    __shared__ float part[4][64];
     const int tid = threadIdx.x, lane = tid & 63, w = tid >> 6;
-    if ((int)blockIdx.x >= n_scan) {
-        if (have_colsum) colsum_final_plain(c, (int)blockIdx.x - n_scan, part);
-        return;
-    }
     const int blk = blockIdx.x;
     const int i = blk * 1024 + tid;
     int v[3] = {0, 0, 0};
@@ -1573,14 +1550,213 @@
     if ((int)blockIdx.x < n_fill) csc_fill_body(a, blockIdx.x, n_fill);
     else colsum_partial_plain(c, blockIdx.x - n_fill);
 }
-__global__ __launch_bounds__(256) void csc_count_colpart_kernel(CscArgs a, int n_count, ColsumPlain c) {
-    if ((int)blockIdx.x < c.n_blocks) colsum_partial_plain(c, blockIdx.x);
-    else csc_count_body(a, blockIdx.x - c.n_blocks);
-}
 __global__ __launch_bounds__(256) void csc_count_colsum_kernel(CscArgs a, int n_count, ColsumPlain c) {
     __shared__ float part[4][64];
     if ((int)blockIdx.x < n_count) csc_count_body(a, blockIdx.x);
     else colsum_final_plain(c, blockIdx.x - n_count, part);
+}
+
+template <typename T> struct CscCell4;
+template <> struct CscCell4<uint16_t> { using V = ushort4; };
+template <> struct CscCell4<uint32_t> { using V = uint4; };
+
+template <typename T>
+__global__ __launch_bounds__(256) void csc_blk_count_kernel(CscArgs a, ColsumPlain c, int n_colsum, int tile) {
+    extern __shared__ uint32_t csc_hist[];
+    if ((int)blockIdx.x < n_colsum) { colsum_partial_plain(c, blockIdx.x); return; }
+    const int k = a.k_dev ? min(*a.k_dev, a.k) : a.k;
+    if (k <= 0) return;
+    using V = typename CscCell4<T>::V;
+    const int rb = (int)blockIdx.x - n_colsum, r0 = rb * CSC_BLK_ROWS, nr = min(CSC_BLK_ROWS, a.n_rows - r0);
+    const int S4 = (a.S + 3) >> 2;
+    V* const out = reinterpret_cast<V*>(a.blk) + (size_t)rb * S4;
+    for (int t0 = 0; t0 < a.S; t0 += tile) {
+        const int t1 = min(a.S, t0 + tile), tw = (t1 - t0 + 3) >> 2;
+        for (int w = threadIdx.x; w < tw; w += 256) csc_hist[w] = 0u;
+        __syncthreads();
+        for (int p = threadIdx.x; p < nr * k; p += 256) {
+            const int r = p / k, j = p - r * k;
+            const int32_t i = a.idx[(size_t)(r0 + r) * a.code_stride + j];
+            if (i >= t0 && i < t1) atomicAdd(&csc_hist[(i - t0) >> 2], 1u << (8 * ((i - t0) & 3)));
+        }
+        __syncthreads();
+        for (int w = threadIdx.x; w < tw; w += 256) {
+            const uint32_t h = csc_hist[w];
+            V v;
+            v.x = (T)(h & 255u); v.y = (T)((h >> 8) & 255u); v.z = (T)((h >> 16) & 255u); v.w = (T)(h >> 24);
+            out[(t0 >> 2) + w] = v;
+        }
+        __syncthreads();
+    }
+}
+
+template <typename T>
+__global__ __launch_bounds__(256) void csc_blk_prefix_kernel(CscArgs a, int n_blk, int n_prefix, ColsumPlain c, int have_colsum) {
+    __shared__ float part[4][64];
+    __shared__ int tot[16][64];
+    if ((int)blockIdx.x >= n_prefix) {
+        if (have_colsum) colsum_final_plain(c, (int)blockIdx.x - n_prefix, part);
+        return;
+    }
+    if (a.k_dev && *a.k_dev <= 0) return;
+    using V = typename CscCell4<T>::V;
+    const int q = threadIdx.x & 15, seg = threadIdx.x >> 4;
+    const int S4 = (a.S + 3) >> 2, quad = (int)blockIdx.x * 16 + q;
+    const int per = (n_blk + 15) >> 4, rb0 = min(n_blk, seg * per), rb1 = min(n_blk, rb0 + per);
+    V* const col = reinterpret_cast<V*>(a.blk) + quad;
+    int s[4] = {0, 0, 0, 0};
+    if (quad < S4) {
+        int rb = rb0;
+        for (; rb + 8 <= rb1; rb += 8) {
+            V v[8];
+#pragma unroll
+            for (int u = 0; u < 8; ++u) v[u] = col[(size_t)(rb + u) * S4];
+#pragma unroll
+            for (int u = 0; u < 8; ++u) { s[0] += v[u].x; s[1] += v[u].y; s[2] += v[u].z; s[3] += v[u].w; }
+        }
+        for (; rb < rb1; ++rb) {
+            const V v = col[(size_t)rb * S4];
+            s[0] += v.x; s[1] += v.y; s[2] += v.z; s[3] += v.w;
+        }
+    }
+#pragma unroll
+    for (int e = 0; e < 4; ++e) tot[seg][4 * q + e] = s[e];
+    __syncthreads();
+    if (quad >= S4) return;
+    int b[4] = {0, 0, 0, 0};
+    for (int j = 0; j < seg; ++j)
+#pragma unroll
+        for (int e = 0; e < 4; ++e) b[e] += tot[j][4 * q + e];
+    int rb = rb0;
+    for (; rb + 8 <= rb1; rb += 8) {
+        V v[8];
+#pragma unroll
+        for (int u = 0; u < 8; ++u) v[u] = col[(size_t)(rb + u) * S4];
+#pragma unroll
+        for (int u = 0; u < 8; ++u) {
+            V o;
+            o.x = (T)b[0]; o.y = (T)b[1]; o.z = (T)b[2]; o.w = (T)b[3];
+            col[(size_t)(rb + u) * S4] = o;
+            b[0] += v[u].x; b[1] += v[u].y; b[2] += v[u].z; b[3] += v[u].w;
+        }
+    }
+    for (; rb < rb1; ++rb) {
+        const V v = col[(size_t)rb * S4];
+        V o;
+        o.x = (T)b[0]; o.y = (T)b[1]; o.z = (T)b[2]; o.w = (T)b[3];
+        col[(size_t)rb * S4] = o;
+        b[0] += v.x; b[1] += v.y; b[2] += v.z; b[3] += v.w;
+    }
+    if (seg == 15)
+#pragma unroll
+        for (int e = 0; e < 4; ++e)
+            if (4 * quad + e < a.S) a.counts[4 * quad + e] = b[e];
+}
+
+constexpr int CSC_STAGE = 4096;
+template <typename T>
+__global__ __launch_bounds__(1024) void csc_blk_place_kernel(CscArgs a, int tile) {
+    extern __shared__ uint32_t csc_hist[];
+    __shared__ int32_t stage[CSC_STAGE];
+    __shared__ uint8_t rnk[CSC_STAGE];
+    const int k = a.k_dev ? min(*a.k_dev, a.k) : a.k;
+    if (k <= 0) return;
+    const int tid = threadIdx.x, nt = blockDim.x;
+    if (a.chunk_starts)
+        for (int p = (int)blockIdx.x * nt + tid; p < a.S; p += (int)gridDim.x * nt) {
+            const int c1 = a.chunk_starts[p + 1];
+            for (int c = a.chunk_starts[p]; c < c1; ++c) a.work_latent[c] = p;
+        }
+    const int rb = blockIdx.x, r0 = rb * CSC_BLK_ROWS, nr = min(CSC_BLK_ROWS, a.n_rows - r0);
+    const int S4 = (a.S + 3) >> 2;
+    const T* const pre = reinterpret_cast<const T*>(a.blk) + (size_t)rb * S4 * 4;
+    const int KC = min(k, CSC_STAGE), RS = CSC_STAGE / KC;
+    for (int t0 = 0; t0 < a.S; t0 += tile) {
+        const int t1 = min(a.S, t0 + tile), tw = (t1 - t0 + 3) >> 2;
+        for (int w = tid; w < tw; w += nt) csc_hist[w] = 0u;
+        for (int rr = 0; rr < nr; rr += RS) {
+            const int rs = min(RS, nr - rr);
+            for (int c0 = 0; c0 < k; c0 += KC) {
+                const int kc = min(KC, k - c0);
+                constexpr int CPT = CSC_STAGE / 1024;
+                int32_t ci[CPT];
+                int cst[CPT], ccn[CPT], cpre[CPT];
+                float cv[CPT], cdv[CPT];
+#pragma unroll
+                for (int u = 0; u < CPT; ++u) {
+                    const int q = tid + u * 1024;
+                    ci[u] = -1;
+                    if (q < rs * kc) {
+                        const int r = q / kc, j = c0 + q - r * kc;
+                        const int32_t i = a.idx[(size_t)(r0 + rr + r) * a.code_stride + j];
+                        ci[u] = (i >= t0 && i < t1) ? i : -1;
+                        stage[q] = ci[u];
+                    }
+                }
+                __syncthreads();
+                if (tid < 64) {
+                    const int cpr = (kc + 63) >> 6, n_adds = rs * cpr;
+                    for (int s0 = 0; s0 < n_adds; s0 += 8) {
+                        int32_t iv[8];
+                        int qv[8];
+                        uint32_t old[8];
+                        bool any = false;
+#pragma unroll
+                        for (int u = 0; u < 8; ++u) {
+                            const int r = (s0 + u) / cpr, jc = ((s0 + u) - r * cpr) * 64 + tid;
+                            qv[u] = r * kc + jc;
+                            iv[u] = (s0 + u < n_adds && jc < kc) ? stage[qv[u]] : -1;
+                            any = any || iv[u] >= 0;
+                        }
+                        if (__ballot(any) == 0) continue;
+#pragma unroll
+                        for (int u = 0; u < 8; ++u) {
+                            old[u] = 0u;
+                            if (iv[u] >= 0) old[u] = atomicAdd(&csc_hist[(iv[u] - t0) >> 2], 1u << (8 * ((iv[u] - t0) & 3)));
+                            __builtin_amdgcn_wave_barrier();
+                        }
+#pragma unroll
+                        for (int u = 0; u < 8; ++u)
+                            if (iv[u] >= 0) rnk[qv[u]] = (uint8_t)((old[u] >> (8 * ((iv[u] - t0) & 3))) & 255u);
+                    }
+                }
+#pragma unroll
+                for (int u = 0; u < CPT; ++u) {
+                    cst[u] = 0; ccn[u] = 0; cpre[u] = 0; cv[u] = 0.f; cdv[u] = 0.f;
+                    if (ci[u] >= 0) {
+                        const int q = tid + u * 1024, r = q / kc, j = c0 + q - r * kc;
+                        const size_t code = (size_t)(r0 + rr + r) * a.code_stride + j;
+                        cpre[u] = (int)pre[ci[u]];
+                        cst[u] = a.starts[ci[u]];
+                        if (a.pv != nullptr) {
+                            ccn[u] = a.counts[ci[u]];
+                            cv[u] = a.val[code];
+                            if (a.pv2 != nullptr) cdv[u] = a.dval[code];
+                        }
+                    }
+                }
+                __syncthreads();
+#pragma unroll
+                for (int u = 0; u < CPT; ++u) {
+                    const int32_t i = ci[u];
+                    if (i < 0) continue;
+                    const int q = tid + u * 1024, r = q / kc, j = c0 + q - r * kc, b = r0 + rr + r;
+                    const int rank = cpre[u] + (int)rnk[q];
+                    const int slot = cst[u] + rank;
+                    if (a.pairs != nullptr) a.pairs[slot] = int2{b, (int)((size_t)b * a.code_stride + j)};
+                    if (a.pv != nullptr) {
+                        const int fl = (rank == 0 ? DWS_FIRST : 0) | (rank == ccn[u] - 1 ? DWS_LAST : 0);
+                        int pblk = 0;
+                        if (a.P > 1) while (pblk < a.P - 1 && i >= a.cuts[pblk]) ++pblk;
+                        a.pv[slot] = int2{((pblk * a.n_rows + b) << 7) | fl, __float_as_int(cv[u])};
+                        a.plat[slot] = i;
+                        if (a.pv2 != nullptr) a.pv2[slot] = int2{(b << 7) | fl, __float_as_int(cdv[u])};
+                    }
+                }
+                __syncthreads();
+            }
+        }
+    }
 }
 
 template <typename F>
@@ -1651,35 +1827,62 @@
         hipLaunchKernelGGL(decode_matry_kernel<decltype(nv)::value>, dim3((a.n_rows + 3) / 4), dim3(256), 0, stream, a, m);
     });
 }
-hipError_t launch_csc_build(const CscArgs& a, hipStream_t stream, bool bitmap_clean, const float* colsum_m, int colsum_D,
-                            long colsum_row_stride, float* colsum_partials, float* colsum_out, bool prefilled, bool colsum_slice_major) {
+hipError_t launch_csc_build(const CscArgs& a, hipStream_t stream, bool via_bitmap, const float* colsum_m, int colsum_D,
+                            long colsum_row_stride, float* colsum_partials, float* colsum_out, bool colsum_slice_major) {
     if (a.n_rows <= 0) return hipSuccess;
     const long n = (long)a.n_rows * a.k;
-    const int blocks = prefilled ? 0 : (int)std::min<long>((n + 255) / 256, 4096);
-    const int place_blocks = (int)std::min<long>((std::max<long>(n, a.S) + 255) / 256, 8192);
-    if (!bitmap_clean && !prefilled) hipLaunchKernelGGL(csc_clear_kernel, dim3(2048), dim3(256), 0, stream, a);
     const int n_scan = (a.S + 1023) / 1024;
     ColsumPlain c{colsum_m, a.n_rows, colsum_D, colsum_partials, colsum_row_stride > 0 ? colsum_row_stride : (long)colsum_D,
                   colsum_out, (a.n_rows + 63) / 64, colsum_slice_major ? 1 : 0};
-    int colsum_in_scan = 0;
-    if (colsum_m != nullptr && prefilled && a.epoch != 0) {
-        hipLaunchKernelGGL(csc_count_colpart_kernel, dim3((a.S + 3) / 4 + c.n_blocks), dim3(256), 0, stream, a, (a.S + 3) / 4, c);
-        colsum_in_scan = 1;
-    } else if (colsum_m != nullptr) {
-        hipLaunchKernelGGL(csc_fill_colsum_kernel, dim3(blocks + c.n_blocks), dim3(256), 0, stream, a, blocks, c);
-        hipLaunchKernelGGL(csc_count_colsum_kernel, dim3((a.S + 3) / 4 + (colsum_D + 63) / 64), dim3(256), 0, stream, a, (a.S + 3) / 4, c);
+    const int n_colpart = colsum_m != nullptr ? c.n_blocks : 0, n_colfin = colsum_m != nullptr ? (colsum_D + 63) / 64 : 0;
+    const int n_blk = (a.n_rows + CSC_BLK_ROWS - 1) / CSC_BLK_ROWS;
+    const int tile = std::min((a.S + 3) / 4 * 4, CSC_LDS_LATENTS);
+    if (via_bitmap) {
+        if (a.bitmap == nullptr || a.grp_prefix == nullptr) return hipErrorInvalidValue;
+        const int blocks = (int)std::min<long>((n + 255) / 256, 4096);
+        hipLaunchKernelGGL(csc_clear_kernel, dim3(2048), dim3(256), 0, stream, a);
+        if (colsum_m != nullptr) {
+            hipLaunchKernelGGL(csc_fill_colsum_kernel, dim3(blocks + c.n_blocks), dim3(256), 0, stream, a, blocks, c);
+            hipLaunchKernelGGL(csc_count_colsum_kernel, dim3((a.S + 3) / 4 + n_colfin), dim3(256), 0, stream, a, (a.S + 3) / 4, c);
+        } else {
+            hipLaunchKernelGGL(csc_fill_kernel, dim3(blocks), dim3(256), 0, stream, a);
+            hipLaunchKernelGGL(csc_count_kernel, dim3((a.S + 3) / 4), dim3(256), 0, stream, a);
+        }
     } else {
-        if (blocks > 0) hipLaunchKernelGGL(csc_fill_kernel, dim3(blocks), dim3(256), 0, stream, a);
-        hipLaunchKernelGGL(csc_count_kernel, dim3((a.S + 3) / 4), dim3(256), 0, stream, a);
+        if (a.blk == nullptr) return hipErrorInvalidValue;
+        static bool attr_set = false;
+        if (!attr_set) {
+            const void* fns[4] = {reinterpret_cast<const void*>(&csc_blk_count_kernel<uint16_t>), reinterpret_cast<const void*>(&csc_blk_count_kernel<uint32_t>),
+                                  reinterpret_cast<const void*>(&csc_blk_place_kernel<uint16_t>), reinterpret_cast<const void*>(&csc_blk_place_kernel<uint32_t>)};
+            for (const void* f : fns) {
+                hipError_t e = hipFuncSetAttribute(f, hipFuncAttributeMaxDynamicSharedMemorySize, CSC_LDS_LATENTS);
+                if (e != hipSuccess) return e;
+            }
+            attr_set = true;
+        }
+        const int n_prefix = ((a.S + 3) / 4 + 15) / 16;
+        if (a.blk_wide) {
+            hipLaunchKernelGGL(csc_blk_count_kernel<uint32_t>, dim3(n_colpart + n_blk), dim3(256), tile, stream, a, c, n_colpart, tile);
+            hipLaunchKernelGGL(csc_blk_prefix_kernel<uint32_t>, dim3(n_prefix + n_colfin), dim3(256), 0, stream, a, n_blk, n_prefix, c, n_colfin > 0 ? 1 : 0);
+        } else {
+            hipLaunchKernelGGL(csc_blk_count_kernel<uint16_t>, dim3(n_colpart + n_blk), dim3(256), tile, stream, a, c, n_colpart, tile);
+            hipLaunchKernelGGL(csc_blk_prefix_kernel<uint16_t>, dim3(n_prefix + n_colfin), dim3(256), 0, stream, a, n_blk, n_prefix, c, n_colfin > 0 ? 1 : 0);
+        }
     }
     if (a.epoch != 0 && n_scan <= 128) {
-        hipLaunchKernelGGL(csc_scan_fused_kernel, dim3(n_scan + (colsum_in_scan ? (colsum_D + 63) / 64 : 0)), dim3(1024), 0, stream, a, n_scan, c,
-                           colsum_in_scan);
+        hipLaunchKernelGGL(csc_scan_fused_kernel, dim3(n_scan), dim3(1024), 0, stream, a, n_scan);
     } else {
         hipLaunchKernelGGL(csc_scan_block_kernel, dim3(n_scan), dim3(1024), 0, stream, a);
         hipLaunchKernelGGL(csc_scan_offset_kernel, dim3(n_scan), dim3(1024), 0, stream, a);
     }
-    hipLaunchKernelGGL(csc_place_kernel, dim3(place_blocks), dim3(256), 0, stream, a);
+    if (via_bitmap) {
+        const int place_blocks = (int)std::min<long>((std::max<long>(n, a.S) + 255) / 256, 8192);
+        hipLaunchKernelGGL(csc_place_kernel, dim3(place_blocks), dim3(256), 0, stream, a);
+    } else if (a.blk_wide) {
+        hipLaunchKernelGGL(csc_blk_place_kernel<uint32_t>, dim3(n_blk), dim3(1024), tile, stream, a, tile);
+    } else {
+        hipLaunchKernelGGL(csc_blk_place_kernel<uint16_t>, dim3(n_blk), dim3(1024), tile, stream, a, tile);
+    }
     return hipGetLastError();
 }
 hipError_t launch_dw_rows(const DwRowsArgs& a, int max_work, hipStream_t stream) {
@@ -1707,7 +1910,6 @@
     if (!light) { a.sq_wave_dec = nullptr; a.sq_wave_enc = nullptr; }
     if (part != 2 && a.have_dval) {
         hipLaunchKernelGGL((dw_slices_kernel<true, false>), dim3(grid), dim3(256), 0, stream, a, wg_per_slice);
-        if (a.clear_bitmap != nullptr && !light) hipLaunchKernelGGL(dw_clear_bitmap_kernel, dim3((max_pairs + 255) / 256), dim3(256), 0, stream, a);
     } else if (part != 2) {
         hipLaunchKernelGGL(dw_slices_kernel<true>, dim3(grid), dim3(256), 0, stream, a, wg_per_slice);
         hipLaunchKernelGGL(dw_dval_sum_kernel, dim3((max_pairs + 255) / 256), dim3(256), 0, stream, a);
```

Result: no change. 6.490 million (median of 6 runs) (+0.9%).
